# demox-labs/aleo

Measured on AMD Instinct MI355X. Metric: MSM G1 scalar-muls/sec (2^20 bases per GPU, BLS12-377, bit-exact), higher is better.
Workload: dtype u32

## Files before the change

### aleo_amd/_lib.py

```python
from __future__ import annotations
import ctypes, os

_HERE = os.path.dirname(os.path.abspath(__file__))
LIB_PATH = os.environ.get('ALEO_MI355X_LIB') or os.path.join(_HERE, 'lib', 'libaleo_mi355x.so')

EXPORTS = [
    'aleo_mi355x_init', 'aleo_mi355x_msm_g1', 'aleo_mi355x_bases_pin', 'aleo_mi355x_bases_unpin',
    'aleo_mi355x_bases_generate', 'aleo_mi355x_bases_from_scalars', 'aleo_mi355x_fr_lin_device', 'aleo_mi355x_msm_g1_device_sparse', 'aleo_mi355x_bases_precompute_range', 'aleo_mi355x_kzg_commit_segments_sparse_device', 'aleo_mi355x_fr_blind_rows_device', 'aleo_mi355x_ahp_sumcheck_operands_device', 'aleo_mi355x_varuna_prove', 'aleo_mi355x_varuna_index_build', 'aleo_mi355x_varuna_index_export', 'aleo_mi355x_varuna_index_vk', 'aleo_mi355x_varuna_index_free', 'aleo_mi355x_varuna_prove_indexed', 'aleo_mi355x_varuna_prove_batch_indexed', 'aleo_mi355x_varuna_last_timing', 'aleo_mi355x_fr_random_device', 'aleo_mi355x_fr_lincomb_device', 'aleo_mi355x_ahp_first_sumcheck_device', 'aleo_mi355x_ahp_matrix_sumcheck_device', 'aleo_mi355x_fr_powers_device', 'aleo_mi355x_fr_gather_mul_device', 'aleo_mi355x_fr_eval_batch_device', 'aleo_mi355x_bases_download', 'aleo_mi355x_bases_info', 'aleo_mi355x_bases_precompute',
    'aleo_mi355x_msm_g1_pinned', 'aleo_mi355x_msm_g1_device', 'aleo_mi355x_g1_sum', 'aleo_mi355x_msm_g2', 'aleo_mi355x_g2_sum', 'aleo_mi355x_bases_g2_pin', 'aleo_mi355x_bases_g2_unpin', 'aleo_mi355x_msm_g2_pinned', 'aleo_mi355x_ntt_fr',
    'aleo_mi355x_ntt_fr_device', 'aleo_mi355x_ntt_fr_batch_device', 'aleo_mi355x_ntt_fr_from_device', 'aleo_mi355x_fr_grid_scale_device', 'aleo_mi355x_kzg_commit', 'aleo_mi355x_kzg_commit_device', 'aleo_mi355x_kzg_commit_hiding',
    'aleo_mi355x_msm_g1_batch_device', 'aleo_mi355x_kzg_commit_batch_device', 'aleo_mi355x_kzg_commit_batch', 'aleo_mi355x_kzg_commit_segments', 'aleo_mi355x_kzg_commit_segments_device',
    'aleo_mi355x_fr_vec_op_device', 'aleo_mi355x_fr_batch_inverse_device', 'aleo_mi355x_fr_spmv_device', 'aleo_mi355x_fr_divide_by_linear_device', 'aleo_mi355x_kzg_open_device', 'aleo_mi355x_fq_mul',
    'aleo_mi355x_fr_mul', 'aleo_mi355x_selftest_madd28', 'aleo_mi355x_selftest_addquad', 'aleo_mi355x_selftest_f28_rows', 'aleo_mi355x_selftest_g2pair', 'aleo_mi355x_selftest_slice_order', 'aleo_mi355x_last_msm_timing', 'aleo_mi355x_strerror', 'aleo_mi355x_last_error',
    'aleo_mi355x_version',
    'aleo_mi355x_g1_compress', 'aleo_mi355x_g1_decompress', 'aleo_mi355x_fr_to_bytes', 'aleo_mi355x_fr_from_bytes',
    'aleo_mi355x_bech32m_encode', 'aleo_mi355x_bech32m_decode', 'aleo_mi355x_proof_to_bytes',
    'aleo_mi355x_poseidon_hash_fr', 'aleo_mi355x_fs_new', 'aleo_mi355x_fs_free', 'aleo_mi355x_fs_absorb_bytes', 'aleo_mi355x_fs_absorb_g1',
    'aleo_mi355x_fs_absorb_fr', 'aleo_mi355x_fs_squeeze_fr', 'aleo_mi355x_fr_random', 'aleo_mi355x_poseidon_parameters_fr',
    'aleo_mi355x_init_device', 'aleo_mi355x_device_count', 'aleo_mi355x_peer_info', 'aleo_mi355x_min_msm', 'aleo_mi355x_min_ntt', 'aleo_mi355x_kzg_commit_segments_sharded_device', 'aleo_mi355x_kzg_commit_batch_sharded_device', 'aleo_mi355x_bases_attach_shards', 'aleo_mi355x_bases_shard_transforms', 'aleo_mi355x_bases_pin_sharded', 'aleo_mi355x_bases_generate_sharded', 'aleo_mi355x_bases_unpin_sharded',
    'aleo_mi355x_bases_sharded_info', 'aleo_mi355x_msm_g1_sharded', 'aleo_mi355x_fr_transpose_device', 'aleo_mi355x_ntt_fr_sharded', 'aleo_mi355x_ntt_fr_sharded_device', 'aleo_mi355x_selftest_host_inverse', 'aleo_mi355x_varuna_prove_many',
    'aleo_mi355x_record_parse', 'aleo_mi355x_records_scan', 'aleo_mi355x_records_scan_host', 'aleo_mi355x_min_records',
    'aleo_mi355x_records_scan_many', 'aleo_mi355x_records_scan_many_host',
    'aleo_mi355x_records_parse_many', 'aleo_mi355x_records_parse_many_host', 'aleo_mi355x_records_scan_strings', 'aleo_mi355x_records_scan_strings_host',
    'aleo_mi355x_records_decrypt_fields', 'aleo_mi355x_records_decrypt_fields_host', 'aleo_mi355x_min_decrypt',
    'aleo_mi355x_record_fields', 'aleo_mi355x_record_plaintext', 'aleo_mi355x_record_decrypt',
    'aleo_mi355x_records_decrypt_strings', 'aleo_mi355x_records_decrypt_strings_host', 'aleo_mi355x_found_free', 'aleo_mi355x_found_count', 'aleo_mi355x_found_index',
    'aleo_mi355x_found_kind', 'aleo_mi355x_found_rvk', 'aleo_mi355x_found_offsets', 'aleo_mi355x_found_fields', 'aleo_mi355x_found_plain', 'aleo_mi355x_found_status',
    'aleo_mi355x_found_microcredits', 'aleo_mi355x_found_unparsed', 'aleo_mi355x_found_first_unparsed',
    'aleo_mi355x_records_decrypt_strings_many', 'aleo_mi355x_records_decrypt_strings_many_host',
    'aleo_mi355x_records_serial_numbers', 'aleo_mi355x_records_serial_numbers_host', 'aleo_mi355x_min_serials', 'aleo_mi355x_found_serial_numbers',
    'aleo_mi355x_record_commitment', 'aleo_mi355x_record_checksum', 'aleo_mi355x_account_from_private_key',
]


class AleoMi355xError(RuntimeError):
    status = None


class NotOwner(AleoMi355xError):
    status = 7


class UnsatisfiedAssignment(AleoMi355xError):
    status = 6


_LIB = None


def lib():
    global _LIB
    if _LIB is not None:
        return _LIB
    if not os.path.exists(LIB_PATH):
        raise AleoMi355xError(f'{LIB_PATH} not built: run `python -c "import __graft_entry__ as g; g.build()"` '
                              '(aleo_amd/csrc/build.sh).  There is no CPU fallback.')
    try:
        import torch
    except Exception:
        pass
    L = ctypes.CDLL(LIB_PATH)
    vp, sz, i32, u32, u64 = ctypes.c_void_p, ctypes.c_size_t, ctypes.c_int32, ctypes.c_uint32, ctypes.c_uint64
    sig = {
        'aleo_mi355x_init': ([i32], i32),
        'aleo_mi355x_init_device': ([i32], i32),
        'aleo_mi355x_device_count': ([ctypes.POINTER(i32), ctypes.POINTER(i32)], i32),
        'aleo_mi355x_peer_info': ([ctypes.POINTER(i32), ctypes.POINTER(i32)], i32),
        'aleo_mi355x_min_msm': ([], sz),
        'aleo_mi355x_min_ntt': ([], sz),
        'aleo_mi355x_kzg_commit_segments_sharded_device': ([vp, sz, u64, vp, sz, vp], i32),
        'aleo_mi355x_kzg_commit_batch_sharded_device': ([vp, u64, vp, vp, sz, vp], i32),
        'aleo_mi355x_bases_attach_shards': ([u64, u64, sz], i32),
        'aleo_mi355x_bases_shard_transforms': ([u64, sz], i32),
        'aleo_mi355x_bases_pin_sharded': ([vp, sz, sz, ctypes.POINTER(i32), sz, i32, ctypes.POINTER(u64)], i32),
        'aleo_mi355x_bases_generate_sharded': ([vp, u64, sz, ctypes.POINTER(i32), sz, i32, ctypes.POINTER(u64)], i32),
        'aleo_mi355x_bases_unpin_sharded': ([u64], i32),
        'aleo_mi355x_bases_sharded_info': ([u64, ctypes.POINTER(u64), i32], i32),
        'aleo_mi355x_msm_g1_sharded': ([vp, u64, vp, sz, vp], i32),
        'aleo_mi355x_fr_transpose_device': ([vp, vp, u64, u64, vp], i32),
        'aleo_mi355x_ntt_fr_sharded': ([vp, u32, i32, i32, ctypes.POINTER(i32), sz], i32),
        'aleo_mi355x_ntt_fr_sharded_device': ([vp, u32, i32, i32, ctypes.POINTER(i32), sz, vp], i32),
        'aleo_mi355x_selftest_host_inverse': ([u32, ctypes.c_uint64, ctypes.POINTER(u32), ctypes.POINTER(ctypes.c_double)], i32),
        'aleo_mi355x_msm_g1': ([vp, vp, sz, vp, sz], i32),
        'aleo_mi355x_bases_pin': ([vp, sz, sz, ctypes.POINTER(u64)], i32),
        'aleo_mi355x_bases_unpin': ([u64], i32),
        'aleo_mi355x_bases_generate': ([vp, u64, sz, ctypes.POINTER(u64)], i32),
        'aleo_mi355x_bases_from_scalars': ([vp, vp, sz, ctypes.POINTER(u64)], i32),
        'aleo_mi355x_fr_lin_device': ([vp, sz, vp, vp, vp, vp, vp, vp], i32),
        'aleo_mi355x_fr_powers_device': ([vp, sz, vp, vp, vp], i32),
        'aleo_mi355x_msm_g1_device_sparse': ([vp, u64, vp, sz, vp], i32),
        'aleo_mi355x_bases_precompute_range': ([u64, sz, sz, i32], i32),
        'aleo_mi355x_kzg_commit_segments_sparse_device': ([vp, sz, u64, vp, sz, vp], i32),
        'aleo_mi355x_fr_blind_rows_device': ([vp, vp, sz, sz, vp, vp], i32),
        'aleo_mi355x_ahp_sumcheck_operands_device': ([vp, vp, vp, sz, sz, sz, vp], i32),
        'aleo_mi355x_varuna_prove': ([vp, ctypes.POINTER(vp), sz, vp, vp, ctypes.POINTER(sz)], i32),
        'aleo_mi355x_varuna_index_build': ([ctypes.POINTER(u64), u64, u64, u64, u64, vp, sz, sz, sz, ctypes.c_uint32], i32),
        'aleo_mi355x_varuna_index_export': ([u64, vp], i32),
        'aleo_mi355x_varuna_index_vk': ([u64, vp, ctypes.POINTER(sz)], i32),
        'aleo_mi355x_varuna_index_free': ([u64], i32),
        'aleo_mi355x_varuna_prove_indexed': ([u64, ctypes.POINTER(vp), sz, vp, vp, ctypes.POINTER(sz)], i32),
        'aleo_mi355x_varuna_prove_batch_indexed': ([ctypes.POINTER(u64), sz, ctypes.POINTER(vp), ctypes.POINTER(sz), vp, vp, ctypes.POINTER(sz)], i32),
        'aleo_mi355x_varuna_last_timing': ([ctypes.POINTER(ctypes.c_double), i32], i32),
        'aleo_mi355x_varuna_prove_many': ([vp, sz], i32),
        'aleo_mi355x_fr_random_device': ([vp, sz, vp, u64, i32, vp], i32),
        'aleo_mi355x_fr_random': ([vp, sz, vp, u64], i32),
        'aleo_mi355x_poseidon_hash_fr': ([u32, vp, sz, vp, sz], i32),
        'aleo_mi355x_poseidon_parameters_fr': ([u32, vp, vp], i32),
        'aleo_mi355x_fs_new': ([ctypes.POINTER(u64)], i32),
        'aleo_mi355x_fs_free': ([u64], i32),
        'aleo_mi355x_fs_absorb_bytes': ([u64, vp, sz], i32),
        'aleo_mi355x_fs_absorb_g1': ([u64, vp, sz, sz], i32),
        'aleo_mi355x_fs_absorb_fr': ([u64, vp, sz], i32),
        'aleo_mi355x_fs_squeeze_fr': ([u64, vp, sz, i32], i32),
        'aleo_mi355x_fr_lincomb_device': ([vp, sz, vp, ctypes.POINTER(vp), ctypes.POINTER(sz), vp, sz, vp], i32),
        'aleo_mi355x_ahp_first_sumcheck_device': ([vp, sz, vp, vp, vp, vp, vp, vp, vp, vp], i32),
        'aleo_mi355x_ahp_matrix_sumcheck_device': ([vp, sz, ctypes.POINTER(vp), sz, ctypes.POINTER(vp), vp, vp], i32),
        'aleo_mi355x_fr_gather_mul_device': ([vp, sz, vp, vp, vp, vp, vp, vp], i32),
        'aleo_mi355x_fr_eval_batch_device': ([vp, ctypes.POINTER(vp), ctypes.POINTER(sz), vp, sz, vp], i32),
        'aleo_mi355x_bases_download': ([u64, sz, sz, vp], i32),
        'aleo_mi355x_bases_info': ([u64, ctypes.POINTER(u64), i32], i32),
        'aleo_mi355x_bases_precompute': ([u64], i32),
        'aleo_mi355x_msm_g1_pinned': ([vp, u64, vp, sz], i32),
        'aleo_mi355x_msm_g1_device': ([vp, u64, vp, sz, vp], i32),
        'aleo_mi355x_g1_sum': ([vp, vp, sz], i32),
        'aleo_mi355x_msm_g2': ([vp, vp, sz, vp, sz], i32),
        'aleo_mi355x_g2_sum': ([vp, vp, sz], i32),
        'aleo_mi355x_bases_g2_pin': ([vp, sz, sz, ctypes.POINTER(u64)], i32),
        'aleo_mi355x_bases_g2_unpin': ([u64], i32),
        'aleo_mi355x_msm_g2_pinned': ([vp, u64, vp, sz], i32),
        'aleo_mi355x_ntt_fr': ([vp, u32, i32, i32, i32], i32),
        'aleo_mi355x_ntt_fr_device': ([vp, u32, i32, i32, i32, vp], i32),
        'aleo_mi355x_ntt_fr_batch_device': ([vp, u32, sz, i32, i32, i32, vp], i32),
        'aleo_mi355x_ntt_fr_from_device': ([vp, vp, sz, sz, u32, sz, i32, i32, vp], i32),
        'aleo_mi355x_fr_grid_scale_device': ([vp, u32, u64, u64, u64, u64, u64, i32, i32, vp], i32),
        'aleo_mi355x_kzg_commit': ([vp, u64, vp, sz], i32),
        'aleo_mi355x_kzg_commit_device': ([vp, u64, vp, sz, vp], i32),
        'aleo_mi355x_kzg_commit_hiding': ([vp, u64, vp, sz, u64, vp, sz], i32),
        'aleo_mi355x_msm_g1_batch_device': ([vp, u64, vp, vp, sz, vp], i32),
        'aleo_mi355x_kzg_commit_batch_device': ([vp, u64, vp, vp, sz, vp], i32),
        'aleo_mi355x_kzg_commit_batch': ([vp, u64, vp, vp, sz], i32),
        'aleo_mi355x_kzg_commit_segments': ([vp, sz, u64, vp, sz], i32),
        'aleo_mi355x_kzg_commit_segments_device': ([vp, sz, u64, vp, sz, vp], i32),
        'aleo_mi355x_fr_vec_op_device': ([vp, vp, vp, sz, i32, vp], i32),
        'aleo_mi355x_fr_batch_inverse_device': ([vp, sz, vp], i32),
        'aleo_mi355x_fr_spmv_device': ([vp, vp, vp, vp, vp, sz, vp], i32),
        'aleo_mi355x_fr_divide_by_linear_device': ([vp, vp, vp, sz, vp, vp], i32),
        'aleo_mi355x_kzg_open_device': ([vp, vp, u64, vp, sz, vp, vp], i32),
        'aleo_mi355x_fq_mul': ([vp, vp, vp, sz], i32),
        'aleo_mi355x_fr_mul': ([vp, vp, vp, sz], i32),
        'aleo_mi355x_selftest_madd28': ([u32, u32, u64, ctypes.POINTER(u32)], i32),
        'aleo_mi355x_selftest_addquad': ([u32, u64, ctypes.POINTER(u32)], i32),
        'aleo_mi355x_selftest_f28_rows': ([vp, vp, u32, vp, vp, vp, vp, u32, vp, vp], i32),
        'aleo_mi355x_selftest_g2pair': ([vp, u32, u32, ctypes.POINTER(u32)], i32),
        'aleo_mi355x_selftest_slice_order': ([vp, u32, u32, i32, ctypes.POINTER(u32)], i32),
        'aleo_mi355x_last_msm_timing': ([ctypes.POINTER(ctypes.c_double), i32], i32),
        'aleo_mi355x_strerror': ([i32], ctypes.c_char_p),
        'aleo_mi355x_last_error': ([], ctypes.c_char_p),
        'aleo_mi355x_version': ([], ctypes.c_char_p),
        'aleo_mi355x_g1_compress': ([vp, vp, sz], i32),
        'aleo_mi355x_g1_decompress': ([vp, vp, sz, i32], i32),
        'aleo_mi355x_fr_to_bytes': ([vp, vp, sz], i32),
        'aleo_mi355x_fr_from_bytes': ([vp, vp, sz], i32),
        'aleo_mi355x_bech32m_encode': ([ctypes.c_char_p, sz, ctypes.c_char_p, vp, sz], i32),
        'aleo_mi355x_bech32m_decode': ([vp, ctypes.POINTER(sz), ctypes.c_char_p, sz, ctypes.c_char_p], i32),
        'aleo_mi355x_proof_to_bytes': ([vp, ctypes.POINTER(sz), vp], i32),
        'aleo_mi355x_record_parse': ([ctypes.c_char_p, ctypes.POINTER(i32), vp, vp], i32),
        'aleo_mi355x_records_scan': ([vp, vp, vp, vp, sz, vp, vp], i32),
        'aleo_mi355x_records_scan_host': ([vp, vp, vp, vp, sz, vp, vp], i32),
        'aleo_mi355x_min_records': ([], sz),
        'aleo_mi355x_records_scan_many': ([vp, vp, vp, vp, sz, vp, vp, sz], i32),
        'aleo_mi355x_records_scan_many_host': ([vp, vp, vp, vp, sz, vp, vp, sz], i32),
        'aleo_mi355x_records_parse_many': ([vp, vp, vp, vp, vp, sz], i32),
        'aleo_mi355x_records_parse_many_host': ([vp, vp, vp, vp, vp, sz], i32),
        'aleo_mi355x_records_scan_strings': ([vp, vp, vp, vp, vp, sz, vp, vp, sz], i32),
        'aleo_mi355x_records_scan_strings_host': ([vp, vp, vp, vp, vp, sz, vp, vp, sz], i32),
        'aleo_mi355x_records_decrypt_fields': ([vp, vp, vp, vp, vp, sz], i32),
        'aleo_mi355x_records_decrypt_fields_host': ([vp, vp, vp, vp, vp, sz], i32),
        'aleo_mi355x_min_decrypt': ([], sz),
        'aleo_mi355x_record_fields': ([ctypes.c_char_p, vp, sz, ctypes.POINTER(sz)], i32),
        'aleo_mi355x_record_plaintext': ([ctypes.c_char_p, vp, sz, vp, ctypes.c_char_p, ctypes.POINTER(sz)], i32),
        'aleo_mi355x_record_decrypt': ([ctypes.c_char_p, vp, vp, ctypes.c_char_p, ctypes.POINTER(sz)], i32),
        'aleo_mi355x_records_decrypt_strings': ([ctypes.POINTER(vp), vp, vp, sz, vp, vp], i32),
        'aleo_mi355x_records_decrypt_strings_host': ([ctypes.POINTER(vp), vp, vp, sz, vp, vp], i32),
        'aleo_mi355x_records_decrypt_strings_many': ([ctypes.POINTER(vp), vp, vp, sz, vp, vp, sz], i32),
        'aleo_mi355x_records_decrypt_strings_many_host': ([ctypes.POINTER(vp), vp, vp, sz, vp, vp, sz], i32),
        'aleo_mi355x_records_serial_numbers': ([vp, vp, vp, sz, vp], i32),
        'aleo_mi355x_records_serial_numbers_host': ([vp, vp, vp, sz, vp], i32),
        'aleo_mi355x_min_serials': ([], sz),
        'aleo_mi355x_found_serial_numbers': ([vp, vp, sz, vp, vp, vp], i32),
        'aleo_mi355x_record_commitment': ([vp, ctypes.c_char_p, vp, sz, ctypes.c_char_p, ctypes.c_char_p], i32),
        'aleo_mi355x_record_checksum': ([vp, ctypes.c_char_p], i32),
        'aleo_mi355x_account_from_private_key': ([ctypes.c_char_p, vp, vp, vp], i32),
        'aleo_mi355x_found_free': ([vp], None),
        **{'aleo_mi355x_found_' + name: ([vp], sz) for name in ('count', 'fields', 'unparsed', 'first_unparsed')},
        **{'aleo_mi355x_found_' + name: ([vp], vp) for name in ('index', 'kind', 'rvk', 'offsets', 'plain', 'status', 'microcredits')},
    }
    for name, (args, res) in sig.items():
        f = getattr(L, name); f.argtypes = args; f.restype = res
    _LIB = L
    return L


def check(status: int, what: str):
    if status != 0:
        L = lib()
        e = {UnsatisfiedAssignment.status: UnsatisfiedAssignment, NotOwner.status: NotOwner}.get(status, AleoMi355xError)(
            f'{what}: {L.aleo_mi355x_strerror(status).decode()} [{L.aleo_mi355x_last_error().decode()}]')
        e.status = status
        raise e


def seed32(seed=None):
    if seed is None: raw = os.urandom(32)
    elif isinstance(seed, (bytes, bytearray)):
        if len(seed) != 32: raise ValueError('a proof seed is 32 bytes')
        raw = bytes(seed)
    else: raw = int(seed).to_bytes(32, 'little')
    return (ctypes.c_uint8 * 32).from_buffer_copy(raw)
```

### aleo_amd/csrc/api.hip

```cpp
#include "entry.h"
#include "host_field.hpp"
#include <cstdlib>
#include <chrono>
#include <cstring>
#include <thread>

namespace aleo_mi355x {

thread_local MsmTiming g_last_msm;

static void jacobian_to_affine104(void* out104, const uint64_t* jac18) {
  uint8_t* o = (uint8_t*)out104; std::memset(o, 0, 104);
  bool inf = true; for (int i = 12; i < 18; ++i) if (jac18[i]) inf = false;
  if (inf) { o[96] = 1; host::HFq one = host::HFq::one(); std::memcpy(o + 48, one.l, 48); return; }
  std::memcpy(o, jac18, 96);
}

void jacobian_rows_to_affine104(void* out104, const uint64_t* jac18, size_t k) {
  for (size_t q = 0; q < k; ++q) jacobian_to_affine104((uint8_t*)out104 + 104 * q, jac18 + 18 * q);
}

template <class F> static int32_t enqueue_on_slot(void* stream, F&& f) {
  Slot sl; if (sl.rc) return sl.rc;
  hipStream_t s = nullptr; if (int32_t rcs = pick_stream(sl.c, stream, &s)) return rcs;
// ... 437 lines not shown
        for (size_t g = 0; g < G; ++g) { for (size_t i = 0; i < grp[g].size(); ++i) live[at[g][i]] = grp[g][i]; if (rcs[g] && !rc) { rc = rcs[g]; g_last_error = errs[g]; } }
        split_done = true;
      }
    }
    if (!split_done) rc = live.empty() ? ALEO_MI355X_OK : varuna_prove_many(sl.c, fb.pb, live);
    std::string first_error;
    for (size_t i = 0; i < live.size(); ++i) { requests[where[i]].status = live[i].status; if (live[i].status && first_error.empty()) first_error = live[i].error; }
    for (size_t p = 0; p < n_requests; ++p) if (rq[p].status && first_error.empty()) first_error = rq[p].error;
    if (!first_error.empty()) g_last_error = first_error;
    return rc;
  });
}

int32_t aleo_mi355x_varuna_last_timing(double* out_ms, int32_t cap) {
  int32_t n = cap < 8 ? cap : 8;
  for (int32_t i = 0; i < n; ++i) out_ms[i] = g_varuna_timing[i];
  return n;
}

int32_t aleo_mi355x_fr_random_device(void* d_dst, size_t n, const uint8_t* seed, uint64_t first_index, int32_t montgomery, void* stream) {
  return device_entry((!d_dst && n) || !seed, nullptr, stream, [&](Ctx* c, hipStream_t s) { return fr_random(c, d_dst, n, seed, first_index, montgomery, s); });
}

int32_t aleo_mi355x_fr_lincomb_device(void* d_dst, size_t n, const void* c0_mont, const void* const* d_terms, const size_t* lens, const void* coeffs_mont, size_t k, void* stream) {
  return device_entry((!d_dst && n) || (k && (!d_terms || !lens || !coeffs_mont)), nullptr, stream, [&](Ctx* c, hipStream_t s) { return fr_lincomb(c, d_dst, n, c0_mont, d_terms, lens, coeffs_mont, k, s); });
}

int32_t aleo_mi355x_ahp_first_sumcheck_device(void* d_dst, size_t n, const void* d_r, const void* d_za, const void* d_zb, const void* d_t, const void* d_z,
                                              const void* eta_b_mont, const void* eta_c_mont, void* stream) {
  return device_entry(n && (!d_dst || !d_r || !d_za || !d_zb || !d_t || !d_z || !eta_b_mont || !eta_c_mont), nullptr, stream, [&](Ctx* c, hipStream_t s) { return ahp_first_sumcheck(c, d_dst, n, d_r, d_za, d_zb, d_t, d_z, eta_b_mont, eta_c_mont, s); });
}

int32_t aleo_mi355x_ahp_matrix_sumcheck_device(void* d_dst, size_t n, const void* const* d_index, size_t index_stride, const void* const* d_f, const void* consts_mont, void* stream) {
  return device_entry(n && (!d_dst || !d_index || !d_f || !consts_mont || (d_index[0] && !d_f[0]) || (d_index[1] && !d_f[1]) || (d_index[2] && !d_f[2])), nullptr, stream, [&](Ctx* c, hipStream_t s) { return ahp_matrix_sumcheck(c, d_dst, n, d_index, index_stride, d_f, consts_mont, s); });
}

int32_t aleo_mi355x_fr_blind_rows_device(void* d_dst, const void* d_src, size_t n, size_t rows, const void* rho_mont, void* stream) {
  return device_entry(rows && n && (!d_dst || !d_src || !rho_mont), nullptr, stream, [&](Ctx* c, hipStream_t s) { return fr_blind_rows(c, d_dst, d_src, n, rows, rho_mont, s); });
}

int32_t aleo_mi355x_ahp_sumcheck_operands_device(void* d_dst, const void* d_witness_polys, const void* d_x_polys, size_t n, size_t n_x, size_t instances, void* stream) {
  return device_entry(instances && n && (!d_dst || !d_witness_polys || (!d_x_polys && n_x)), nullptr, stream, [&](Ctx* c, hipStream_t s) { return ahp_sumcheck_operands(c, d_dst, d_witness_polys, d_x_polys, n, n_x, instances, s); });
}

int32_t aleo_mi355x_fr_batch_inverse_device(void* d_inout, size_t n, void* stream) {
  return device_entry(!d_inout && n, nullptr, stream, [&](Ctx* c, hipStream_t s) { return fr_batch_inverse(c, d_inout, n, s); });
}

int32_t aleo_mi355x_fr_divide_by_linear_device(void* d_quotient, void* d_eval, const void* d_poly, size_t n, const void* z_mont, void* stream) {
  return guarded([&] {
    if ((!d_poly && n) || (!d_quotient && !d_eval)) return ALEO_MI355X_ERR_BAD_ARG;
    if (!z_mont || (d_quotient && d_quotient == d_poly)) return bad_arg("fr_divide_by_linear_device: null point, or quotient aliases the polynomial");
    return enqueue_on_slot(stream, [&](Ctx* c, hipStream_t s) { return fr_divide_by_linear(c, d_quotient, d_eval, d_poly, n, z_mont, s); });
  });
}

int32_t aleo_mi355x_kzg_open_device(void* out_affine104, void* out_eval_mont, uint64_t handle, const void* d_poly_mont, size_t n, const void* z_mont, void* stream) {
  return guarded([&] {
    if (!out_affine104 || !z_mont || (!d_poly_mont && n)) return ALEO_MI355X_ERR_BAD_ARG;
    Slot sl; if (sl.rc) return sl.rc;
    FoundBases fb(sl.d, handle); if (fb.rc) return fb.rc;
    hipStream_t s = nullptr; if (int32_t rcs = pick_stream(sl.c, stream, &s)) return rcs;
    int32_t rc; if ((rc = sl.c->ntt_stage.reserve((n ? n : 1) * 32 + 32))) return rc;
    char* q = sl.c->ntt_stage.as<char>(); char* ev = q + (n ? n : 1) * 32;
    if ((rc = fr_divide_by_linear(sl.c, q, ev, d_poly_mont, n, z_mont, s))) return rc;
    if (out_eval_mont) HIPCHK(hipMemcpyAsync(out_eval_mont, ev, 32, hipMemcpyDeviceToHost, s));
    uint64_t jac[18];
    if ((rc = msm_run1(sl.c, jac, fb.pb, q, n ? n - 1 : 0, true, s))) return rc;
    if (n <= 1) HIPCHK(hipStreamSynchronize(s));
    jacobian_to_affine104(out_affine104, jac);
    return ALEO_MI355X_OK;
  });
}

int32_t aleo_mi355x_fr_spmv_device(void* d_y, const void* d_row_ptr, const void* d_col_idx, const void* d_vals, const void* d_x, size_t rows, void* stream) {
  return device_entry((!d_y || !d_row_ptr) && rows, nullptr, stream, [&](Ctx* c, hipStream_t s) { return fr_spmv(c, d_y, d_row_ptr, d_col_idx, d_vals, d_x, rows, s); });
}

int32_t aleo_mi355x_ntt_fr(void* inout, uint32_t lg_n, int32_t order, int32_t direction, int32_t type) {
  return guarded([&] {
    if (!inout || lg_n > 30 || order < 0 || order > 3 || direction < 0 || direction > 1 || type < 0 || type > 1) return bad_arg("ntt_fr: bad argument");
    Slot sl; if (sl.rc) return sl.rc;
    size_t bytes = ((size_t)1 << lg_n) * 32;
    int32_t rc; if ((rc = sl.c->ntt_stage.reserve(bytes))) return rc;
    HIPCHK(hipMemcpyAsync(sl.c->ntt_stage.p, inout, bytes, hipMemcpyHostToDevice, sl.c->stream));
    if ((rc = ntt_run(sl.c, sl.c->ntt_stage.p, lg_n, 1, order, direction, type, sl.c->stream))) return rc;
    HIPCHK(hipMemcpyAsync(inout, sl.c->ntt_stage.p, bytes, hipMemcpyDeviceToHost, sl.c->stream));
    HIPCHK(hipStreamSynchronize(sl.c->stream));
    return ALEO_MI355X_OK;
  });
}

int32_t aleo_mi355x_ntt_fr_device(void* d_inout, uint32_t lg_n, int32_t order, int32_t direction, int32_t type, void* stream) {
  return device_entry(!d_inout || lg_n > 30 || order < 0 || order > 3 || direction < 0 || direction > 1 || type < 0 || type > 1, "ntt_fr_device: bad argument", stream, [&](Ctx* c, hipStream_t s) { return ntt_run(c, d_inout, lg_n, 1, order, direction, type, s); });
}

int32_t aleo_mi355x_ntt_fr_batch_device(void* d_inout, uint32_t lg_n, size_t batch, int32_t order, int32_t direction, int32_t type, void* stream) {
  return device_entry((!d_inout && batch) || lg_n > 30 || order < 0 || order > 3 || direction < 0 || direction > 1 || type < 0 || type > 1, "ntt_fr_batch_device: bad argument", stream, [&](Ctx* c, hipStream_t s) { return ntt_run(c, d_inout, lg_n, batch, order, direction, type, s); });
}

int32_t aleo_mi355x_ntt_fr_from_device(void* d_out, const void* d_src, size_t src_stride, size_t src_len, uint32_t lg_n, size_t batch, int32_t direction, int32_t type, void* stream) {
  return guarded([&] {
    if (((!d_out || !d_src) && batch) || lg_n > 30 || direction < 0 || direction > 1 || type < 0 || type > 1 || src_len > ((size_t)1 << lg_n) || src_stride >= (1ull << 32)) {
      g_last_error = "ntt_fr_from_device: bad argument"; return ALEO_MI355X_ERR_BAD_ARG;
    }
    if (batch) {
      const char* o0 = (const char*)d_out; const char* o1 = o0 + ((batch << lg_n) * 32);
      const char* s0 = (const char*)d_src; const char* s1 = s0 + ((batch - 1) * src_stride + src_len) * 32;
      if (src_len && o0 < s1 && s0 < o1) return bad_arg("ntt_fr_from_device: d_out overlaps d_src");
    }
    return enqueue_on_slot(stream, [&](Ctx* c, hipStream_t s) { return ntt_run_from(c, d_out, d_src, src_stride, src_len, lg_n, batch, direction, type, s); });
  });
}

int32_t aleo_mi355x_fr_grid_scale_device(void* d_data, uint32_t lg_n, uint64_t rows, uint64_t cols, uint64_t row0, uint64_t col0, uint64_t ld,
                                         int32_t mode, int32_t direction, void* stream) {
  return device_entry((!d_data && rows && cols) || lg_n == 0 || lg_n > 32 || mode < 0 || mode > 1 || direction < 0 || direction > 1, "fr_grid_scale_device: bad argument", stream, [&](Ctx* c, hipStream_t s) { return fr_grid_scale(c, d_data, lg_n, rows, cols, row0, col0, ld, mode, direction, s); });
}

int32_t aleo_mi355x_fr_transpose_device(void* d_dst, const void* d_src, uint64_t rows, uint64_t cols, void* stream) {
  return guarded([&] {
    if ((!d_dst || !d_src) && rows && cols) return bad_arg("fr_transpose_device: bad argument");
    if (d_dst == d_src && rows > 1 && cols > 1) return bad_arg("fr_transpose_device: in place is not supported");
    return enqueue_on_slot(stream, [&](Ctx* c, hipStream_t s) { return fr_transpose(c, d_dst, d_src, rows, cols, s); });
  });
}

int32_t aleo_mi355x_fq_mul(void* r, const void* a, const void* b, size_t n) {
  return guarded([&] { if ((!r || !a || !b) && n) return ALEO_MI355X_ERR_BAD_ARG; Slot sl; if (sl.rc) return sl.rc; return launch_fq_mul(sl.c, r, a, b, n); });
}
int32_t aleo_mi355x_fr_mul(void* r, const void* a, const void* b, size_t n) {
  return guarded([&] { if ((!r || !a || !b) && n) return ALEO_MI355X_ERR_BAD_ARG; Slot sl; if (sl.rc) return sl.rc; return launch_fr_mul(sl.c, r, a, b, n); });
}

int32_t aleo_mi355x_selftest_madd28(uint32_t lanes, uint32_t steps, uint64_t seed, uint32_t* failures) {
  return guarded([&] { if (!failures) return ALEO_MI355X_ERR_BAD_ARG; Slot sl; if (sl.rc) return sl.rc; return selftest_madd28(sl.c, lanes, steps, seed, failures); });
}
int32_t aleo_mi355x_selftest_addquad(uint32_t ops, uint64_t seed, uint32_t* failures) {
  return guarded([&] { if (!failures || !ops || ops > (1u << 22)) return ALEO_MI355X_ERR_BAD_ARG; Slot sl; if (sl.rc) return sl.rc; return selftest_addquad(sl.c, ops, seed, failures); });
}
int32_t aleo_mi355x_selftest_f28_rows(const void* a224, const void* b224, uint32_t n_add, void* out_pair224, void* out_quad224,
                                      const void* acc224, const void* pt112, uint32_t n_madd, void* out_acc224, uint8_t* ok_u8) {
  return guarded([&] {
    if (n_add > (1u << 20) || n_madd > (1u << 20)) return bad_arg("selftest_f28_rows: at most 2^20 rows of either kind");
    if ((n_add && (!a224 || !b224 || !out_pair224 || !out_quad224)) || (n_madd && (!acc224 || !pt112 || !out_acc224 || !ok_u8))) return bad_arg("selftest_f28_rows: bad argument");
    Slot sl; if (sl.rc) return sl.rc;
    return selftest_f28_rows(sl.c, a224, b224, n_add, out_pair224, out_quad224, acc224, pt112, n_madd, out_acc224, ok_u8);
  });
}

int32_t aleo_mi355x_selftest_slice_order(const uint32_t* hist, uint32_t n_buckets, uint32_t total_pairs, int32_t fused, uint32_t* violations) {
  return guarded([&] { if (!hist || !violations) return ALEO_MI355X_ERR_BAD_ARG; Slot sl; if (sl.rc) return sl.rc; return selftest_slice_order(sl.c, hist, n_buckets, total_pairs, fused != 0, violations); });
}
int32_t aleo_mi355x_selftest_g2pair(const void* affine192, uint32_t n_points, uint32_t n_pairs, uint32_t* failures2) {
  return guarded([&] { if (!affine192 || !failures2 || n_points < 3 || !n_pairs || n_pairs > (1u << 20)) return ALEO_MI355X_ERR_BAD_ARG; Slot sl; if (sl.rc) return sl.rc; return selftest_g2pair(sl.c, affine192, n_points, n_pairs, failures2); });
}

int32_t aleo_mi355x_last_msm_timing(double* out_ms, int32_t cap) {
  return guarded([&] {
    if (!out_ms || cap <= 0) return 0;
    const MsmTiming& t = g_last_msm;
    double v[7] = {t.total, t.sort, t.accum, t.reduce, t.host, t.accum_kernel, (double)t.accum_launches};
    int32_t k = cap < 7 ? cap : 7;
    for (int32_t i = 0; i < k; ++i) out_ms[i] = v[i];
    return k;
  }, 0);
}

const char* aleo_mi355x_strerror(int32_t status) {
  switch (status) {
    case ALEO_MI355X_OK: return "ok";
    case ALEO_MI355X_ERR_NO_DEVICE: return "no gfx950 device available";
    case ALEO_MI355X_ERR_BAD_ARG: return "bad argument";
    case ALEO_MI355X_ERR_HIP: return "HIP runtime error";
    case ALEO_MI355X_ERR_BAD_HANDLE: return "unknown handle";
    case ALEO_MI355X_ERR_OOM: return "out of device memory";
    case ALEO_MI355X_ERR_UNSATISFIED: return "assignment does not satisfy the circuit";
    case ALEO_MI355X_ERR_NOT_OWNER: return "the record's owner is not the given address";
    default: return "unknown status";
  }
}
static size_t env_size(const char* name, size_t dflt) { const char* e = std::getenv(name); if (!e || !*e) return dflt; char* end = nullptr; const unsigned long long v = std::strtoull(e, &end, 10); return end && *end == 0 ? (size_t)v : dflt; }
size_t aleo_mi355x_min_msm(void) { return env_size("ALEO_MI355X_MIN_MSM", (size_t)1 << 10); }
size_t aleo_mi355x_min_ntt(void) { return env_size("ALEO_MI355X_MIN_NTT", (size_t)1 << 12); }
int32_t aleo_mi355x_selftest_host_inverse(uint32_t count, uint64_t seed, uint32_t* failures, double* ns_per_inverse) {
  return guarded([&] {
    if (!failures) return bad_arg("selftest_host_inverse: bad argument");
    *failures = 0;
    inverse_selftest<6>(count, seed, failures, ns_per_inverse);
    inverse_selftest<4>(count, seed, failures, ns_per_inverse ? ns_per_inverse + 2 : nullptr);
    return ALEO_MI355X_OK;
  });
}
const char* aleo_mi355x_last_error(void) { return g_last_error.c_str(); }
const char* aleo_mi355x_version(void) { return "aleo_mi355x 0.4.0 (gfx950)"; }

}
```

### aleo_amd/csrc/ctx.h

```cpp
#pragma once
#include <hip/hip_runtime.h>
#include <atomic>
#include <condition_variable>
#include <cstdint>
#include <cstdio>
#include <map>
#include <memory>
#include <functional>
#include <mutex>
#include <string>
#include <vector>
#include "../../include/aleo_mi355x.h"

namespace aleo_mi355x {

extern thread_local std::string g_last_error;

#define HIPCHK(expr)                                                                                   \
  do {                                                                                                 \
    hipError_t e__ = (expr);                                                                           \
    if (e__ != hipSuccess) {                                                                           \
      char buf__[512];                                                                                 \
      snprintf(buf__, sizeof buf__, "%s failed: %s (%s:%d)", #expr, hipGetErrorString(e__), __FILE__, __LINE__); \
      g_last_error = buf__;                                                                            \
      return (e__ == hipErrorOutOfMemory) ? ALEO_MI355X_ERR_OOM : ALEO_MI355X_ERR_HIP;                 \
    }                                                                                                  \
  } while (0)

struct DevBuf {
  void* p = nullptr; size_t cap = 0;
  int32_t reserve(size_t bytes) {
    if (bytes <= cap) return ALEO_MI355X_OK;
    if (p) { (void)hipFree(p); p = nullptr; cap = 0; }
    size_t want = bytes + bytes / 8;
    HIPCHK(hipMalloc(&p, want));
    cap = want; return ALEO_MI355X_OK;
  }
  template <class T> T* as() const { return (T*)p; }
};

struct DevTmp {
  void* p = nullptr;
  DevTmp() = default; DevTmp(const DevTmp&) = delete; DevTmp& operator=(const DevTmp&) = delete;
  ~DevTmp() { if (p) (void)hipFree(p); }
  int32_t alloc(size_t bytes) { HIPCHK(hipMalloc(&p, bytes ? bytes : 1)); return ALEO_MI355X_OK; }
  void* release() { void* q = p; p = nullptr; return q; }
};

#ifndef ALEO_ROW28
#define ALEO_ROW28 128
#endif
static constexpr size_t ROW28 = ALEO_ROW28;
static_assert(ROW28 == 112 || ROW28 == 128, "row stride of the 28-bit tables");

struct PinnedBases {
  void* d_xy = nullptr;
  void* d_xy28 = nullptr;
  uint8_t* d_inf = nullptr;
  struct PreTable { void* d = nullptr; int c = 0; size_t cover = 0, min_n = 0; };
  PreTable tab[3];
  PreTable range; size_t range_off = 0;
  bool tabled = false;
  uint64_t shards = 0; size_t shard_min = 0;
  size_t shard_ntt_min = (size_t)1 << 24;
  size_t n = 0;
};

struct PinnedOwner {
  PinnedBases pb; bool building = false;
  ~PinnedOwner() { if (pb.d_xy) (void)hipFree(pb.d_xy); if (pb.d_xy28) (void)hipFree(pb.d_xy28); if (pb.d_inf) (void)hipFree(pb.d_inf); for (auto& t : pb.tab) if (t.d) (void)hipFree(t.d); if (pb.range.d) (void)hipFree(pb.range.d); }
};

struct PinnedG2 {
  void* d_xy = nullptr; uint8_t* d_inf = nullptr; void* d_rows28 = nullptr; size_t n = 0;
  ~PinnedG2() { if (d_xy) (void)hipFree(d_xy); if (d_inf) (void)hipFree(d_inf); if (d_rows28) (void)hipFree(d_rows28); }
};

struct SrsCacheEntry {
  const void* host_ptr = nullptr; size_t n = 0, stride = 0; uint64_t handle = 0, last_use = 0; uint32_t hits = 0;
  std::vector<std::pair<size_t, uint64_t>> samples;
};

struct MsmTiming { double total = 0, sort = 0, accum = 0, reduce = 0, host = 0, accum_kernel = 0; int accum_launches = 1; };

struct NttTables;

struct Device;

struct Ctx {
  Device* dev = nullptr;
  int device = -1;
  hipStream_t stream = nullptr;
  std::mutex mu;
  hipEvent_t ev[8] = {};
  uint32_t meta_seq = 0;
  size_t hist_zero_max = 0;
  size_t hist_clean = 0; hipStream_t hist_clean_stream = nullptr; void* hist_clean_ptr = nullptr;
  DevBuf hist, scan_local, scan_blk, sorted, part_cnt, part_items, partial, task_g, meta, vbuf, scalars_stage, out_stage;
  void* h_pinned = nullptr; size_t h_pinned_cap = 0;
  std::function<int32_t()> tail_hook;
  DevBuf prover_ws; void* prover_pin = nullptr; size_t prover_pin_cap = 0;
  MsmTiming last_msm;
  DevBuf cold_raw, cold_xy, cold_xy28, cold_flags;
  DevBuf ntt_tmp, ntt_stage;
  DevBuf records_k; bool records_k_ready = false;
  hipEvent_t scratch_ev = nullptr; bool scratch_busy = false; hipStream_t scratch_stream = nullptr;
  hipStream_t side = nullptr;
  hipStream_t hi = nullptr;
  hipStream_t aux = nullptr;
  hipEvent_t ev_hop = nullptr;
};

int32_t scratch_acquire(Ctx* c, DevBuf& b, size_t bytes, hipStream_t s);
int32_t scratch_release(Ctx* c, hipStream_t s);

static constexpr int MAX_SLOTS = 8;

struct Barrier {
  std::mutex mu; std::condition_variable cv; size_t n, waiting = 0, phase = 0;
  explicit Barrier(size_t n_) : n(n_) {}
  void wait() {
    std::unique_lock<std::mutex> lk(mu); const size_t ph = phase;
    if (++waiting >= n) { waiting = 0; ++phase; cv.notify_all(); } else cv.wait(lk, [&] { return phase != ph; });
  }
  void drop() {
    std::lock_guard<std::mutex> lk(mu);
    if (n) --n;
    if (n && waiting >= n) { waiting = 0; ++phase; cv.notify_all(); }
  }
};

struct ShardWs { hipStream_t st = nullptr; DevBuf a, b; };

struct Device {
  int device = -1;
  int n_slots = 4;
  std::mutex mu;
  std::map<uint64_t, std::shared_ptr<PinnedOwner>> bases; uint64_t next_handle = 1;
  std::vector<SrsCacheEntry> srs_cache; uint64_t srs_clock = 0;
  std::map<uint64_t, std::shared_ptr<PinnedG2>> g2_bases;
  std::map<uint64_t, NttTables*> ntt_tables;
  std::map<uint64_t, std::shared_ptr<struct VarunaIndexOwner>> varuna; uint64_t next_varuna = 1;
  std::atomic<int> ntt_attr_mask{0};
  Ctx slots[MAX_SLOTS];
  std::vector<std::unique_ptr<ShardWs>> shard_ws;
  DevBuf shard_home;
  hipStream_t hi_pool[MAX_SLOTS] = {}; int hi_made = 0;
  Ctx helpers[MAX_SLOTS];
};
struct HelperSet { std::vector<Ctx*> ctx; std::vector<std::unique_lock<std::mutex>> locks; };
int32_t acquire_helpers(Device* d, int want, HelperSet& hs);

extern thread_local MsmTiming g_last_msm;
void host_parallel_for(size_t n, const std::function<void(size_t)>& f);
void host_trace_mark(const char* label);
#define HT(label) do { if (::aleo_mi355x::g_host_trace_on) ::aleo_mi355x::host_trace_mark(label); } while (0)
extern bool g_host_trace_on;
int32_t ensure_host_pinned(Ctx* c, size_t bytes);

struct MsmSeg { const void* d_ptr = nullptr; size_t len = 0, off = 0; uint32_t out = 0; };
struct MsmJob { const MsmSeg* segs = nullptr; uint32_t nseg = 0, k = 0; bool mont = false; bool sparse = false; bool fire_tail = false; size_t tier_n = 0; bool lean = false; };
int32_t msm_run(Ctx* c, uint64_t* out_jac18, const PinnedBases& pb, const MsmJob& job, hipStream_t s);
inline int32_t msm_run1(Ctx* c, uint64_t* out_jac18, const PinnedBases& pb, const void* d_scalars, size_t n, bool mont, hipStream_t s, bool sparse = false) {
  MsmSeg g; g.d_ptr = d_scalars; g.len = n;
  MsmJob j; j.segs = &g; j.nseg = 1; j.k = 1; j.mont = mont; j.sparse = sparse; return msm_run(c, out_jac18, pb, j, s);
}
int32_t msm_batch(Ctx* c, uint64_t* out_jac18, const PinnedBases& pb, const MsmJob& job, hipStream_t s);
int32_t msm_run1_split(Ctx* c, uint64_t* out_jac18, const PinnedBases& pb, const void* d_scalars, size_t n, bool mont, hipStream_t s, bool sparse, const void* host_src, bool may_merge = true);
int32_t selftest_madd28(Ctx* c, uint32_t lanes, uint32_t steps, uint64_t seed, uint32_t* failures);
int32_t selftest_addquad(Ctx* c, uint32_t ops, uint64_t seed, uint32_t* failures);
int32_t selftest_f28_rows(Ctx* c, const void* a224, const void* b224, uint32_t n_add, void* out_pair224, void* out_quad224,
                          const void* acc224, const void* pt112, uint32_t n_madd, void* out_acc224, uint8_t* ok_u8);
int32_t selftest_slice_order(Ctx* c, const uint32_t* h_hist, uint32_t M, uint32_t pairs, bool fused, uint32_t* violations);
int32_t generate_multiples(Ctx* c, const void* base104, uint64_t first, size_t n, PinnedBases* out);
int32_t generate_from_scalars(Ctx* c, const void* base104, const void* scalars32, size_t n, PinnedBases* out);
int32_t msm_precompute(Ctx* c, PinnedBases* pb);
int32_t msm_precompute_range(Ctx* c, PinnedBases* pb, size_t off, size_t n, int window_bits);
int32_t unpack_affine104(Ctx* c, const void* d_rows104, void* d_xy96, void* d_flags, size_t n, hipStream_t s);
int32_t rows_to28_into(const void* d_xy96, void* d_dst, size_t n, hipStream_t s);
int32_t make_rows28(Ctx* c, PinnedBases* pb);
int32_t commit_sharded(Ctx* c, uint64_t sharded_handle, const MsmSeg* segs, uint32_t nseg, uint32_t k, bool mont, uint64_t* out_jac18, hipStream_t s, bool s_drain);
int32_t ntt_sharded_device(Ctx* c, void* d_inout, uint32_t lg_n, int32_t direction, int32_t type, const int* devices, size_t n_devices, hipStream_t s);
int32_t sharded_devices(uint64_t sharded_handle, std::vector<int>* out);
int32_t msm_g2_run(Ctx* c, uint64_t* out_jac36, const void* d_xy, const uint8_t* d_inf, const void* d_scalars, size_t n, hipStream_t s, const void* d_rows28 = nullptr);
int32_t g2_rows_to28(const void* d_xy192, void* d_dst224, size_t n, hipStream_t s);
int32_t g2_sum_host(uint64_t* out36, const uint64_t* pts36, size_t count);
int32_t selftest_g2pair(Ctx* c, const void* aff192_host, uint32_t n, uint32_t npairs, uint32_t* failures2);
int32_t g2_unpack200(Ctx* c, const void* d_rows200, void* d_xy192, void* d_flags, uint32_t* d_count, size_t n, hipStream_t s);
int32_t launch_fq_mul(Ctx* c, void* r, const void* a, const void* b, size_t n);
int32_t launch_fr_mul(Ctx* c, void* r, const void* a, const void* b, size_t n);
int32_t fr_lin(Ctx* c, void* d_dst, size_t n, const void* c0, const void* c1, const void* d_a, const void* c2, const void* d_b, hipStream_t s);
int32_t fr_powers(Ctx* c, void* d_dst, size_t n, const void* first, const void* ratio, hipStream_t s);
int32_t fr_gather_mul(Ctx* c, void* d_dst, size_t n, const void* d_scale, const void* d_t1, const void* d_idx1, const void* d_t2, const void* d_idx2, hipStream_t s);
int32_t fr_gather_mul3(Ctx* c, void* const* d_dst, const size_t* n, const void* const* d_scale, const void* d_t1, const void* const* d_idx1, const void* d_t2, const void* const* d_idx2, uint32_t count, hipStream_t s);
int32_t fr_eval_batch(Ctx* c, void* d_out, const void* const* d_polys, const size_t* lens, const void* z_mont, size_t k, hipStream_t s);
int32_t fr_random(Ctx* c, void* d_dst, size_t n, const uint8_t* seed32, uint64_t first, int32_t mont, hipStream_t s);
int32_t fr_lincomb(Ctx* c, void* d_dst, size_t n, const void* c0, const void* const* d_terms, const size_t* lens, const void* coeffs, size_t k, hipStream_t s);
int32_t fr_add_tiled(Ctx* c, void* d_dst, size_t n, const void* d_src, size_t n_src, hipStream_t s);
int32_t ahp_first_sumcheck(Ctx* c, void* d_dst, size_t n, const void* d_r, const void* d_a, const void* d_b, const void* d_t, const void* d_z, const void* eta_b, const void* eta_c, hipStream_t s);
int32_t ahp_matrix_sumcheck(Ctx* c, void* d_dst, size_t n, const void* const* d_index, size_t index_stride_elems, const void* const* d_f, const void* consts, hipStream_t s);
int32_t fr_blind_rows(Ctx* c, void* d_dst, const void* d_src, size_t n, size_t rows, const void* rho_mont, hipStream_t s);
int32_t ahp_sumcheck_operands(Ctx* c, void* d_dst, const void* d_wit, const void* d_xp, size_t n, size_t n_x, size_t instances, hipStream_t s);
int32_t fr_scatter_to_mont(Ctx* c, void* d_dst, const void* d_src, const void* d_pos, size_t n, void* d_flag, hipStream_t s);
int32_t fr_vec_op(Ctx* c, void* d_dst, const void* d_a, const void* d_b, size_t n, int32_t op, hipStream_t s);
int32_t fr_batch_inverse(Ctx* c, void* d_inout, size_t n, hipStream_t s);
int32_t fr_divide_by_linear(Ctx* c, void* d_q, void* d_eval, const void* d_p, size_t n, const void* z_mont32, hipStream_t s);
int32_t index_expand_rows(Ctx* c, const uint32_t* d_row_ptr, const uint32_t* d_col, const uint32_t* d_positions, size_t rows, uint32_t* d_k_row, uint32_t* d_k_col, uint32_t* d_cpos, uint32_t* d_count_plus1, hipStream_t s);
int32_t index_scan_inclusive(Ctx* c, uint32_t* d_a, size_t n, hipStream_t s);
int32_t index_transpose_rows(Ctx* c, const uint32_t* d_row_ptr, const uint32_t* d_cpos, const void* d_val, size_t rows, uint32_t row_base, uint32_t* d_cursor, uint32_t* d_tcol, void* d_tval, hipStream_t s);
int32_t fr_spmv(Ctx* c, void* d_y, const void* d_row_ptr, const void* d_col, const void* d_vals, const void* d_x, size_t rows, hipStream_t s, size_t max_row = 0);
int32_t fr_divide_by_linear_many(Ctx* c, void* const* d_q, void* const* d_eval, const void* const* d_p, const size_t* n, const void* const* z_mont32, size_t count, hipStream_t s);
int32_t fr_scale_rows(Ctx* c, void* d_dst, const void* d_src, size_t n, size_t rows, const void* consts_mont, hipStream_t s);
int32_t fr_split_quotient(Ctx* c, void* d_hq, void* d_rq, const void* d_q, const void* d_mask, size_t n, void* host_sum_devptr, hipStream_t s);
int32_t fr_sub_mul(Ctx* c, void* d_dst, const void* d_a, const void* d_b, const void* d_m, size_t n, hipStream_t s);
int32_t fr_pick(Ctx* c, void* dst_devptr, const void* const* d_src, size_t count, hipStream_t s);
int32_t varuna_prove(Ctx* c, const PinnedBases& pb, const aleo_mi355x_varuna_index& ix, const void* const* assignments, size_t k, const uint8_t* seed32, uint8_t* out, size_t* out_len);
struct ProveRequest { std::vector<const aleo_mi355x_varuna_index*> ixs; const void* const* assignments = nullptr; const size_t* ks = nullptr; const uint8_t* seed32 = nullptr;
                      uint8_t* out = nullptr; size_t* out_len = nullptr; int32_t status = 0; std::string error; };
int32_t varuna_prove_many(Ctx* c, const PinnedBases& pb, std::vector<ProveRequest>& requests, int workers = 0);
int32_t varuna_prove_batch(Ctx* c, const PinnedBases& pb, const aleo_mi355x_varuna_index* const* ixs, size_t m, const void* const* assignments, const size_t* ks,
                           const uint8_t* seed32, uint8_t* out, size_t* out_len);
extern thread_local double g_varuna_timing[8];
struct VarunaIndexOwner;
int32_t varuna_index_build(Ctx* c, const PinnedBases& pb, std::shared_ptr<PinnedOwner> key, uint64_t key_handle, uint64_t max_degree, uint64_t gamma_offset,
                           uint64_t lagrange_offset, const aleo_mi355x_r1cs_matrix* abc, size_t n_constraints, size_t n_public, size_t n_private, uint32_t domain_flags, VarunaIndexOwner** out);
void varuna_index_delete(VarunaIndexOwner* o);
const aleo_mi355x_varuna_index* varuna_index_view(const VarunaIndexOwner* o);
const std::vector<uint8_t>& varuna_index_vk(const VarunaIndexOwner* o);
void jacobian_rows_to_affine104(void* out104, const uint64_t* jac18, size_t k);
int32_t ntt_run(Ctx* c, void* d_inout, uint32_t lg_n, size_t batch, int32_t order, int32_t direction, int32_t type, hipStream_t s);
int32_t ntt_run_from(Ctx* c, void* d_out, const void* d_src, size_t src_stride_elems, size_t src_len, uint32_t lg_n, size_t batch, int32_t direction, int32_t type, hipStream_t s);

int32_t fr_transpose(Ctx* c, void* d_dst, const void* d_src, uint64_t rows, uint64_t cols, hipStream_t s);
int32_t fr_grid_scale(Ctx* c, void* d_data, uint32_t lg_n, uint64_t rows, uint64_t cols, uint64_t row0, uint64_t col0, uint64_t ld, int32_t mode,
                      int32_t direction, hipStream_t s);

}
```

### aleo_amd/csrc/msm.hip

```cpp
#include "ec.h"
#include "fp28.h"
#include "host_field.hpp"
#include "msm_chain.h"
#include <chrono>

namespace aleo_mi355x {

__device__ __forceinline__ XYZZ xyzz28_to_xyzz(const XYZZ28& a) {
  XYZZ r; r.X = f28_to_fq(a.X); r.Y = f28_to_fq(a.Y); r.ZZ = f28_to_fq(a.ZZ); r.ZZZ = f28_to_fq(a.ZZZ); return r;
}
__device__ __noinline__ void slice_slow_path28(const char* bases, const uint32_t* run, uint32_t j, uint32_t j1, const XYZZ28* acc28, XYZZ* acc_out, bool* inf_out) {
  XYZZ acc = xyzz28_to_xyzz(*acc28); bool inf = false;
  for (; j < j1; ++j) {
    uint32_t e = run[j];
    F28 x, y; load_affine28(bases + (size_t)(e & 0x7fffffffu) * ROW28, x, y);
    AffinePt p; p.x = Fq::reduce(f28_to_fq(x)); p.y = Fq::reduce(f28_to_fq(y));
    if (e >> 31) p.y = fq_neg_canonical(p.y);
    xyzz_madd(acc, inf, p.x, p.y);
  }
  *acc_out = acc; *inf_out = inf;
}

__device__ __forceinline__ const char* chain_sum(const FrontChain& ch, uint32_t g) {
  for (uint32_t i = 0; i < ch.n; ++i) if (ch.v[i].hist[g]) return ch.v[i].partial + (size_t)scan_at(ch.v[i].scan_local, ch.v[i].scan_blk, g).y * 224u;
// ... 175 lines not shown
  uint32_t base = j * S;
  if (base) {
    XYZZ r = xyzz_infinity();
    for (int bit = 31 - __clz(base); bit >= 0; --bit) {
      xyzz_double_ni(&r);
      if ((base >> bit) & 1) xyzz_add_ni(&r, &run);
    }
    xyzz_add_ni(&acc, &r);
  }
  store_xyzz(V + (size_t)t * 192, acc);
}

__global__ void __launch_bounds__(256) k_seg_tree_pass(char* __restrict__ V, uint32_t seg_len, uint32_t nseg, uint32_t L) {
  const uint32_t half = (L + 1) >> 1, pairs = L - half;
  const uint32_t op = (blockIdx.x * 256 + threadIdx.x) >> 1;
  if (op >= pairs * nseg) return;
  const uint32_t seg = op / pairs, i = op % pairs;
  char* pa = V + ((size_t)seg * seg_len + i) * 192;
  xyzz_add_pair(pa, pa + (size_t)half * 192, pa);
}

static constexpr uint32_t PB28 = 224, PW28 = 56;
template <uint32_t LANES>
__global__ void __launch_bounds__(256) k_masked_pairs(const char* __restrict__ Vrun, uint32_t lgN, uint32_t nsets, char* __restrict__ V, uint32_t v_set_stride) {
  const uint32_t seg_len = 1u << (lgN - 2);
  const uint32_t op = (blockIdx.x * 256 + threadIdx.x) >> lg_lanes(LANES);
  if (op >= seg_len * lgN * nsets) return;
  const uint32_t q = op / (seg_len * lgN), r = op % (seg_len * lgN), l = r / seg_len, k = r % seg_len;
  auto ins = [&](uint32_t x) { return ((x >> l) << (l + 1)) | (1u << l) | (x & ((1u << l) - 1u)); };
  const char* run = Vrun + ((size_t)q << lgN) * PB28;
  pt28_add<LANES>(run + (size_t)ins(2 * k) * PB28, run + (size_t)ins(2 * k + 1) * PB28, V + ((size_t)q * v_set_stride + (1u << lgN) + r) * PB28);
}
static constexpr uint32_t FOLD = 256;
template <uint32_t LANES>
__global__ void __launch_bounds__(128 * LANES) k_seg_fold(const char* __restrict__ in, uint32_t in_stride, uint32_t L, uint32_t nseg,
                                                          char* __restrict__ out, uint32_t out_stride) {
  __shared__ __attribute__((aligned(16))) uint32_t lds[2][(FOLD / 2) * PW28];
  const uint32_t bps = (L + FOLD - 1) / FOLD, seg = blockIdx.x / bps, blk = blockIdx.x % bps, pr = threadIdx.x >> lg_lanes(LANES);
  if (seg >= nseg) return;
  {
    const uint32_t e0 = blk * FOLD + 2 * pr;
    const char* src = in + ((size_t)seg * in_stride + e0) * PB28;
    char* dst = (char*)(lds[0] + pr * PW28);
    if (e0 + 1 < L) pt28_add<LANES>(src, src + PB28, dst);
    else if (e0 < L) grp_copy<LANES, PB28>(src, dst);
    else grp_zero<LANES, PB28>(dst);
  }
  uint32_t cur = 0;
  for (uint32_t n = FOLD / 2; n > 1; n >>= 1) {
    __syncthreads();
    if (pr < (n >> 1)) pt28_add<LANES>((const char*)(lds[cur] + (2 * pr) * PW28), (const char*)(lds[cur] + (2 * pr + 1) * PW28), (char*)(lds[cur ^ 1] + pr * PW28));
    cur ^= 1;
  }
  __syncthreads();
  if (pr == 0) grp_copy<LANES, PB28>((const char*)lds[cur], out + ((size_t)seg * out_stride + blk) * PB28);
}
template <uint32_t LANES>
__global__ void __launch_bounds__(256) k_seg_pair_pass(const char* __restrict__ in, uint32_t in_stride, uint32_t L, uint32_t nseg,
                                                       char* __restrict__ out, uint32_t out_stride) {
  const uint32_t half = (L + 1) >> 1;
  const uint32_t op = (blockIdx.x * 256 + threadIdx.x) >> lg_lanes(LANES);
  if (op >= half * nseg) return;
  const uint32_t seg = op / half, i = op % half;
  const char* src = in + ((size_t)seg * in_stride + 2 * i) * PB28;
  char* dst = out + ((size_t)seg * out_stride + i) * PB28;
  if (2 * i + 1 < L) pt28_add<LANES>(src, src + PB28, dst); else grp_copy<LANES, PB28>(src, dst);
}
template <uint32_t LANES>
__global__ void __launch_bounds__(256) k_prog_pass(const char* __restrict__ node, uint32_t node_set_stride, const char* __restrict__ A, uint32_t a_set_stride,
                                                   const char* __restrict__ T, uint32_t t_set_stride, uint32_t nT, uint32_t L, uint32_t nsets,
                                                   char* __restrict__ out, uint32_t out_set_stride) {
  const uint32_t half = L >> 1, per_set = (2 + nT) * half;
  const uint32_t op = (blockIdx.x * 256 + threadIdx.x) >> lg_lanes(LANES);
  if (op >= per_set * nsets) return;
  const uint32_t q = op / per_set, r = op % per_set, g = r / half, i = r % half;
  const char* src = g == 0 ? node + ((size_t)q * node_set_stride + 2 * i) * PB28
                  : g == 1 ? A + ((size_t)q * a_set_stride + 2 * i) * PB28
                           : T + ((size_t)q * t_set_stride + (size_t)(g - 2) * L + 2 * i) * PB28;
  char* dst = out + ((size_t)q * out_set_stride + (size_t)g * half + i) * PB28;
  pt28_add<LANES>(src, src + PB28, dst);
  if (g == 0) grp_copy<LANES, PB28>(src + PB28, out + ((size_t)q * out_set_stride + (size_t)(2 + nT) * half + i) * PB28);
}
__global__ void __launch_bounds__(256) k_prog_pass2(const char* __restrict__ node, uint32_t node_set_stride, const char* __restrict__ A, uint32_t a_set_stride,
                                                    const char* __restrict__ T, uint32_t t_set_stride, uint32_t nT, uint32_t L, uint32_t nsets,
                                                    char* __restrict__ out, uint32_t out_set_stride) {
  __shared__ __attribute__((aligned(16))) uint32_t lds[(2 * 32 + 1) * PW28];
  char* zero = (char*)(lds + 64 * PW28);
  if (threadIdx.x < 4) grp_zero<4, PB28>(zero);
  __syncthreads();
  const uint32_t quarter = L >> 2, per_set = (2 + nT) * quarter;
  const uint32_t oct = threadIdx.x >> 3, y = (threadIdx.x >> 2) & 1u, op = blockIdx.x * 32 + oct;
  if (op >= per_set * nsets) return;
  const uint32_t q = op / per_set, r = op % per_set, g = r / quarter, i = r % quarter;
  const char* src = g == 0 ? node + ((size_t)q * node_set_stride + 4 * i) * PB28
                  : g == 1 ? A + ((size_t)q * a_set_stride + 4 * i) * PB28
                           : T + ((size_t)q * t_set_stride + (size_t)(g - 2) * L + 4 * i) * PB28;
  char* slot = (char*)(lds + (2 * oct) * PW28);
  pt28_add<4>(src + (size_t)(2 * y) * PB28, src + (size_t)(2 * y + 1) * PB28, slot + y * PB28);
  pair_fence();
  char* base = out + (size_t)q * out_set_stride * PB28;
  const bool born = y && g == 0;
  const char* pa = y ? (born ? src + PB28 : zero) : slot;
  const char* pb = y ? (born ? src + 3 * PB28 : zero) : slot + PB28;
  char* dst = y ? (born ? base + ((size_t)(2 + nT) * quarter + i) * PB28 : zero) : base + ((size_t)g * quarter + i) * PB28;
  pt28_add<4>(pa, pb, dst);
  if (born) grp_copy<4, PB28>(slot + PB28, base + ((size_t)(3 + nT) * quarter + i) * PB28);
}
template <uint32_t LANES>
__global__ void __launch_bounds__(128 * LANES) k_prog_final(const char* __restrict__ in, uint32_t in_set_stride, uint32_t L, uint32_t nT, uint32_t lgL, uint32_t nsets,
                                                            char* __restrict__ out) {
  __shared__ __attribute__((aligned(16))) uint32_t lds[2][(FOLD / 2) * PW28];
  const uint32_t per_set = 1 + nT + lgL, q = blockIdx.x / per_set, o = blockIdx.x % per_set, pr = threadIdx.x >> lg_lanes(LANES);
  if (q >= nsets) return;
  const char* set = in + (size_t)q * in_set_stride * PB28;
  {
    char* dst = (char*)(lds[0] + pr * PW28);
    if (o <= nT) {
      const char* seg = set + (size_t)(o == 0 ? 1 : 1 + o) * L * PB28; const uint32_t e0 = 2 * pr;
      if (e0 + 1 < L) pt28_add<LANES>(seg + (size_t)e0 * PB28, seg + (size_t)(e0 + 1) * PB28, dst);
      else if (e0 < L) grp_copy<LANES, PB28>(seg + (size_t)e0 * PB28, dst);
      else grp_zero<LANES, PB28>(dst);
    } else {
      const uint32_t b = o - 1 - nT;
      auto ins = [&](uint32_t x) { return ((x >> b) << (b + 1)) | (1u << b) | (x & ((1u << b) - 1u)); };
      if (L >= 4 && 4 * pr + 3 < L) pt28_add<LANES>(set + (size_t)ins(2 * pr) * PB28, set + (size_t)ins(2 * pr + 1) * PB28, dst);
      else if (L == 2 && pr == 0) grp_copy<LANES, PB28>(set + PB28, dst);
      else grp_zero<LANES, PB28>(dst);
    }
  }
  uint32_t cur = 0;
  for (uint32_t n = FOLD / 2; n > 1; n >>= 1) {
    __syncthreads();
    if (pr < (n >> 1)) pt28_add<LANES>((const char*)(lds[cur] + (2 * pr) * PW28), (const char*)(lds[cur] + (2 * pr + 1) * PW28), (char*)(lds[cur ^ 1] + pr * PW28));
    cur ^= 1;
  }
  __syncthreads();
  if (pr == 0) grp_copy<LANES, PB28>((const char*)lds[cur], out + ((size_t)q * per_set + o) * PB28);
}
__global__ void k_gather_strided(const char* __restrict__ V, uint32_t stride, uint32_t count, char* __restrict__ out) {
  uint32_t t = blockIdx.x * blockDim.x + threadIdx.x;
  if (t >= count * 14) return;
  uint32_t w = t / 14, q = t % 14;
  ((uint4*)out)[t] = ((const uint4*)(V + (size_t)w * stride * PB28))[q];
}

__global__ void k_gather_windows(const char* __restrict__ V, uint32_t seg_len, uint32_t W, char* __restrict__ out) {
  uint32_t t = blockIdx.x * blockDim.x + threadIdx.x;
  if (t >= W * 12) return;
  uint32_t w = t / 12, q = t % 12;
  ((uint4*)out)[t] = ((const uint4*)(V + (size_t)w * seg_len * 192))[q];
}

int32_t msm_front_sort(Ctx* c, const PinnedBases& pb, const MsmJob& job, hipStream_t s, Front& f) {
  const uint32_t K = f.K = job.k;
  size_t n = 0, pts = 0; SegArgs segs{};
  if (K > MAX_SETS || job.nseg > MAX_SEGS) { g_last_error = "msm: too many sets / segments in one call"; return ALEO_MI355X_ERR_BAD_ARG; }
  for (uint32_t q = 0; q < job.nseg; ++q) {
    const MsmSeg& g = job.segs[q];
    if (g.len == 0) continue;
    if (g.out >= K || g.off + g.len >= (1ull << 31)) { g_last_error = "msm: segment out of range"; return ALEO_MI355X_ERR_BAD_ARG; }
    const uint32_t i = segs.nseg++;
    segs.ptr[i] = (const char*)g.d_ptr; segs.n[i] = (uint32_t)g.len; segs.off[i] = (uint32_t)g.off; segs.set[i] = (uint8_t)g.out;
    n = g.off + g.len > n ? g.off + g.len : n; pts += g.len;
  }
  if (n == 0) { f.empty = true; return ALEO_MI355X_OK; }
  if (job.tier_n > n && job.tier_n <= pb.n) n = job.tier_n;
  if (n > pb.n) { g_last_error = "msm: a segment reaches past the pinned bases"; return ALEO_MI355X_ERR_BAD_ARG; }
  const PinnedBases::PreTable* T = nullptr;
  const uint8_t* d_inf = pb.d_inf;
  bool ranged = job.sparse && pb.range.d != nullptr;
  for (uint32_t i = 0; ranged && i < segs.nseg; ++i) ranged = segs.off[i] >= pb.range_off && (size_t)segs.off[i] + segs.n[i] <= pb.range_off + pb.range.cover;
  if (ranged) {
    T = &pb.range; n = 0;
    for (uint32_t i = 0; i < segs.nseg; ++i) { segs.off[i] -= (uint32_t)pb.range_off; n = (size_t)segs.off[i] + segs.n[i] > n ? (size_t)segs.off[i] + segs.n[i] : n; }
    if (d_inf) d_inf += pb.range_off;
  } else T = msm_tier(pb, n);
  const bool pre = f.pre = T != nullptr;
  if (K > 1 && (!pre || K > (ranged ? msm_range_sets(pb) : msm_max_sets(pb, n)))) { g_last_error = "msm: internal: batch without a table tier (or too many sets)"; return ALEO_MI355X_ERR_BAD_ARG; }
  MsmPlan& P = f.P; P = make_plan(pre ? n : pts, pre ? T->c : 0);
  if (pre) { P.W = K; P.M = K * P.B; }
  if (!pre && !pb.d_xy28) { g_last_error = "msm: pinned set without 28-bit rows"; return ALEO_MI355X_ERR_HIP; }
  f.bases = (const char*)(pre ? T->d : pb.d_xy28);
  const uint32_t cpw = f.cpw = P.B / P.S, nchunks = f.nchunks = cpw * P.W;
  uint32_t lgN = 0; while ((1u << lgN) < cpw) ++lgN;
  f.lgN = lgN;
  const bool masked = f.masked = pre && lgN >= 2 && (1u << lgN) == cpw;
  if (pre && !masked) { g_last_error = "msm: internal: table path without masked reduction"; return ALEO_MI355X_ERR_HIP; }
  int32_t rc;
  const uint32_t tseg = f.tseg = cpw / 4, fseg = f.fseg = lgN + 4, nseg = f.nseg = K * fseg, setw = f.setw = fseg * tseg;
  constexpr uint32_t SUM_TREE_MIN_C = 13;
  f.prog = masked && P.c >= SUM_TREE_MIN_C && cpw > FOLD;
  f.out_pts = f.prog ? 1 + lgN : fseg;
  f.vpoints = masked ? (size_t)K * setw + nchunks + (nseg + 1) + (size_t)nseg * (tseg / 2 + tseg / 4 + 2) + 3 * (size_t)nchunks + 64 : (size_t)nchunks + P.W;
  if ((rc = ensure_host_pinned(c, 64 + (size_t)(masked ? nseg : P.W) * 224 + ASIDE_MAX * 228))) return rc;
  SortPhase& sp = f.sp;
  if ((rc = msm_sort_phase(c, segs, pts, job.mont, d_inf, (uint32_t)(pre ? T->cover : pb.n), P, pre, s, &sp, f.lean))) return rc;
  const uint32_t M = sp.M;
  if ((rc = c->partial.reserve(sp.slices_max * (pre ? 224 : 192)))) return rc;
  if ((rc = c->vbuf.reserve(f.vpoints * 224))) return rc;
  return ALEO_MI355X_OK;
}

int32_t msm_front_accum(Ctx* c, hipStream_t s, Front& f, const FrontChain* seed, hipEvent_t after) {
  const SortPhase& sp = f.sp; const uint32_t M = sp.M; const char* bases = f.bases;
  char* partial = c->partial.as<char>();
  if (after) HIPCHK(hipStreamWaitEvent(s, after, 0));
  if (!f.lean) HIPCHK(hipEventRecord(c->ev[6], s));
  const bool seeded = f.pre && seed && seed->n;
  auto* const kern = seeded ? k_accum28<true, true> : f.pre ? k_accum28<true, false> : k_accum28<false, false>;
  hipLaunchKernelGGL(kern, dim3(sp.slice_blocks), dim3(256), 0, s, bases, sp.sorted, sp.hist, sp.scan_local, sp.scan_blk, sp.total_pairs, M, sp.meta, sp.order, sp.task_g, partial, seeded ? *seed : FrontChain{});
  if (!f.lean) HIPCHK(hipEventRecord(c->ev[5], s));
  HIPCHK(hipGetLastError());
  return ALEO_MI355X_OK;
}

int32_t msm_front_finish(Ctx* c, hipStream_t s, Front& f, bool allow_aside) {
  int32_t rc;
  const SortPhase& sp = f.sp; SliceMeta& sm = f.sm; const uint32_t M = sp.M; const bool pre = f.pre;
  uint32_t* heavy = sp.heavy; uint32_t* meta = sp.meta; uint2* scan_local = sp.scan_local; uint2* scan_blk = sp.scan_blk;
  char* partial = c->partial.as<char>();
  if ((rc = msm_wait_meta(c, sp, s, &sm))) return rc;
  const bool aside = f.aside = allow_aside && f.masked && sm.n_super >= 1 && sm.n_super <= ASIDE_MAX && !sm.super_overflow && sm.max_m >= 64;
  uint32_t* h_aside = (uint32_t*)((char*)c->h_pinned + 64 + (size_t)f.nseg * 224);
  if (aside) {
    if (f.lean) HIPCHK(hipEventRecord(c->ev[5], s));
    HIPCHK(hipStreamWaitEvent(c->side, c->ev[5], 0));
    for (uint32_t pass = 0, L = sm.max_m - 1; L > 1; ++pass, L = (L + 1) >> 1) {
      const uint64_t ops = (uint64_t)sm.n_super * (L >> 1);
      launch_grp(grp_lanes(ops), k_tree_pass<true, 4>, k_tree_pass<true, 2>, ops, c->side, partial, heavy, 0u, 0u, sp.super_list, sm.n_super, L >> 1, scan_local, scan_blk, M, meta, pass, 1u);
    }
    uint32_t* dst = nullptr;
    HIPCHK(hipHostGetDevicePointer((void**)&dst, h_aside, 0));
    hipLaunchKernelGGL(k_gather_super, dim3((sm.n_super * 57 + 255) / 256), dim3(256), 0, c->side, partial, sp.super_list, sm.n_super, scan_local, scan_blk, dst);
    HIPCHK(hipEventRecord(c->ev[4], c->side));
  }
  const bool rest_ok = pre && !sm.super_overflow && (aside || sm.n_super == 0) && sm.n_heavy && sm.max_common > 2 && sm.max_common <= 8;
  if (sm.NT) {
    for (uint32_t pass = 0, L = sm.max_m, Lcm = sm.max_common; L > 1; ++pass, L = (L + 1) >> 1, Lcm = (Lcm + 1) >> 1) {
      if (rest_ok && pass == 1) {
        hipLaunchKernelGGL(k_tree_rest<4>, dim3((uint32_t)((4ull * sm.n_heavy + 255) / 256)), dim3(256), 0, s, partial, heavy, sm.n_heavy, scan_local, scan_blk, M, meta);
        break;
      }
      const uint32_t Lc = sm.super_overflow ? L : Lcm;
      const uint32_t len_a = (sm.n_heavy && Lc > 1) ? sm.n_heavy : 0, pairs_a = len_a ? Lc >> 1 : 0;
      const uint32_t len_b = aside ? 0 : sm.n_super, pairs_b = len_b ? L >> 1 : 0;
      const uint64_t ops = (uint64_t)len_a * pairs_a + (uint64_t)len_b * pairs_b;
      const uint32_t lanes = pre ? grp_lanes(ops) : 2u;
      const uint64_t threads = lanes * ops;
      if (!threads) continue;
      if (threads >= (1ull << 32)) { (void)hipStreamSynchronize(s); g_last_error = "msm: slice tree too wide"; return ALEO_MI355X_ERR_HIP; }
      launch_grp(lanes, k_tree_pass<true, 4>, pre ? k_tree_pass<true, 2> : k_tree_pass<false, 2>, ops, s, partial, heavy, len_a, pairs_a, sp.super_list, len_b, pairs_b, scan_local, scan_blk, M, meta, pass, 0u);
    }
  }
  if (!f.lean) HIPCHK(hipEventRecord(c->ev[2], s));
  return ALEO_MI355X_OK;
}

int32_t msm_reduce_queue(Ctx* c, Front& f, hipStream_t s, const FrontChain& older) {
  const MsmPlan& P = f.P; const SortPhase& sp = f.sp;
  const uint32_t K = f.K, cpw = f.cpw, nchunks = f.nchunks, lgN = f.lgN, tseg = f.tseg, nseg = f.nseg, setw = f.setw;
  uint32_t* hist = sp.hist; uint2* scan_local = sp.scan_local; uint2* scan_blk = sp.scan_blk;
  char* partial = c->partial.as<char>(); char* V = c->vbuf.as<char>(); char* h_win = (char*)c->h_pinned + 64;
  char* Vrun = V + (size_t)K * setw * PB28; char* Tout = Vrun + (size_t)nchunks * PB28;
  const uint32_t lanes = grp_lanes(2 * (uint64_t)nchunks), per_block = lanes == 4 ? 32u : CHUNK_QUADS;
  auto* const chunks = lanes == 4 ? k_bucket_chunks<true, 4> : k_bucket_chunks<true, 2>;
  hipLaunchKernelGGL(chunks, dim3((nchunks + per_block - 1) / per_block), dim3(256), 0, s, partial, hist, scan_local, scan_blk, P.B, P.S, nchunks, V, setw, Vrun, older);
  if (f.prog) {
    char* G0 = Tout; char* G1 = G0 + (size_t)K * (3 * (cpw / 2)) * PB28;
    const char* node = Vrun; uint32_t node_ss = cpw; const char* A = V; uint32_t a_ss = setw; const char* T = Vrun; uint32_t t_ss = 0, nT = 0, L = cpw;
    char* dstbuf = G0;
    while (L > FOLD) {
      const uint32_t half = L >> 1, out_ss = (3 + nT) * half; const uint64_t ops = (uint64_t)(2 + nT) * half * K;
      if ((L >> 2) >= FOLD && grp_lanes(ops) == 4) {
        const uint32_t quarter = L >> 2, out2 = (4 + nT) * quarter; const uint64_t octs = (uint64_t)(2 + nT) * quarter * K;
        hipLaunchKernelGGL(k_prog_pass2, dim3((uint32_t)((octs + 31) / 32)), dim3(256), 0, s, node, node_ss, A, a_ss, T, t_ss, nT, L, K, dstbuf, out2);
        node = dstbuf; node_ss = out2; A = dstbuf + (size_t)quarter * PB28; a_ss = out2; T = dstbuf + (size_t)2 * quarter * PB28; t_ss = out2; nT += 2; L = quarter;
        dstbuf = dstbuf == G0 ? G1 : G0;
        continue;
      }
      launch_grp(grp_lanes(ops), k_prog_pass<4>, k_prog_pass<2>, ops, s, node, node_ss, A, a_ss, T, t_ss, nT, L, K, dstbuf, out_ss);
      node = dstbuf; node_ss = out_ss; A = dstbuf + (size_t)half * PB28; a_ss = out_ss; T = dstbuf + (size_t)2 * half * PB28; t_ss = out_ss; ++nT; L = half;
      dstbuf = dstbuf == G0 ? G1 : G0;
    }
    uint32_t lgL = 0; while ((1u << lgL) < L) ++lgL;
    char* dst = nullptr;
    HIPCHK(hipHostGetDevicePointer((void**)&dst, h_win, 0));
    hipLaunchKernelGGL(k_prog_final<4>, dim3(K * (1 + nT + lgL)), dim3(512), 0, s, node, node_ss, L, nT, lgL, K, dst);
  } else {
    const uint64_t mops = (uint64_t)tseg * lgN * K;
    launch_grp(grp_lanes(mops), k_masked_pairs<4>, k_masked_pairs<2>, mops, s, Vrun, lgN, K, V, setw);
    char* F1 = Tout + (size_t)(nseg + 1) * PB28; char* F2 = F1 + (size_t)nseg * (tseg / 2 + 1) * PB28;
    const char* cur = V; uint32_t L = tseg, stride = tseg;
    while (L > FOLD) {
      char* dst = (cur == F1) ? F2 : F1; uint32_t half = (L + 1) >> 1;
      const uint64_t ops = (uint64_t)half * nseg;
      launch_grp(grp_lanes(ops), k_seg_pair_pass<4>, k_seg_pair_pass<2>, ops, s, cur, stride, L, nseg, dst, half);
      cur = dst; stride = half; L = half;
    }
    if (L > 1) {
      char* dst = nullptr;
      HIPCHK(hipHostGetDevicePointer((void**)&dst, h_win, 0));
      hipLaunchKernelGGL(k_seg_fold<4>, dim3(nseg), dim3(512), 0, s, cur, stride, L, nseg, dst, 1u);
    } else {
      hipLaunchKernelGGL(k_gather_strided, dim3((nseg * 14 + 255) / 256), dim3(256), 0, s, cur, stride, nseg, Tout);
      HIPCHK(hipMemcpyAsync(h_win, Tout, (size_t)nseg * PB28, hipMemcpyDeviceToHost, s));
    }
  }
  HIPCHK(hipEventRecord(c->ev[3], s));
  if (f.lean && older.n == 0 && !f.aside) {
    if (sp.zero_bytes > c->hist_zero_max) c->hist_zero_max = sp.zero_bytes;
    const size_t z = c->hist_zero_max <= c->hist.cap && (void*)sp.hist == c->hist.p ? c->hist_zero_max : sp.zero_bytes;
    HIPCHK(hipMemsetAsync(sp.hist, 0, z, s)); c->hist_clean = z; c->hist_clean_stream = s; c->hist_clean_ptr = (void*)sp.hist;
  }
  return ALEO_MI355X_OK;
}

static int32_t phase_times(Ctx* c, const Front& f, std::chrono::steady_clock::time_point t_host0) {
  const double host_ms = std::chrono::duration<double, std::milli>(std::chrono::steady_clock::now() - t_host0).count();
  float ms; MsmTiming tm;
  if (f.lean) { tm.host = host_ms; tm.total = host_ms; c->last_msm = tm; g_last_msm = tm; return ALEO_MI355X_OK; }
  HIPCHK(hipEventElapsedTime(&ms, c->ev[0], c->ev[1])); tm.sort = ms;
  HIPCHK(hipEventElapsedTime(&ms, c->ev[1], c->ev[2])); tm.accum = ms;
  HIPCHK(hipEventElapsedTime(&ms, c->ev[2], c->ev[3])); tm.reduce = ms;
  HIPCHK(hipEventElapsedTime(&ms, c->ev[6], c->ev[5])); tm.accum_kernel = ms;
  tm.host = host_ms; tm.total = tm.sort + tm.accum + tm.reduce + tm.host;
  c->last_msm = tm; g_last_msm = tm;
  return ALEO_MI355X_OK;
}

int32_t msm_collect(Ctx* c, uint64_t* out_jac18, Front& f, hipStream_t s, bool fire_tail, TailWait wait) {
  using namespace host;
  const MsmPlan& P = f.P; const SliceMeta& sm = f.sm; const uint32_t K = f.K, lgN = f.lgN, out_pts = f.out_pts; const bool prog = f.prog, aside = f.aside;
  const uint32_t* h_aside = (const uint32_t*)((char*)c->h_pinned + 64 + (size_t)f.nseg * 224);
  const char* h_win = (const char*)c->h_pinned + 64;
  if (fire_tail && c->tail_hook) {
    std::function<int32_t()> hook = std::move(c->tail_hook); c->tail_hook = nullptr;
    HT("msm: reduction queued");
    const int32_t hrc = hook();
    HT("msm: hook queued");
    HIPCHK(hipEventSynchronize(c->ev[3]));
    if (hrc) { (void)hipStreamSynchronize(s); return hrc; }
  } else if (wait == TailWait::event) HIPCHK(hipEventSynchronize(c->ev[3]));
  else HIPCHK(hipStreamSynchronize(s));
  if (aside) HIPCHK(hipEventSynchronize(c->ev[4]));
  HIPCHK(hipGetLastError());
  HT("msm: result arrived");
  const auto t_host0 = std::chrono::steady_clock::now();
  HXYZZ totals[MAX_SETS];
  auto horner = [&](size_t q) {
// ... 128 lines not shown
```

### aleo_amd/csrc/msm_chain.h

```cpp
#pragma once
#include "msm_common.h"

namespace aleo_mi355x {
#pragma GCC visibility push(hidden)
struct FrontView { const char* partial; const uint32_t* hist; const uint2* scan_local; const uint2* scan_blk; };
struct FrontChain { FrontView v[3]; uint32_t n = 0; };
struct Front {
  MsmPlan P{}; SortPhase sp; SliceMeta sm;
  uint32_t K = 0, cpw = 0, nchunks = 0, lgN = 0, tseg = 0, fseg = 0, nseg = 0, setw = 0; size_t vpoints = 0;
  uint32_t out_pts = 0;
  bool pre = false, masked = false, prog = false, aside = false, empty = false, lean = false; const char* bases = nullptr;
};
struct StreamDrainGuard {
  std::vector<hipStream_t> streams; bool armed = true;
  ~StreamDrainGuard() { if (!armed) return; const std::string keep = g_last_error; for (hipStream_t st : streams) if (st) (void)hipStreamSynchronize(st); g_last_error = keep; }
  void add(hipStream_t st) { streams.push_back(st); }
  void dismiss() { armed = false; }
};
int32_t msm_front_sort(Ctx* c, const PinnedBases& pb, const MsmJob& job, hipStream_t s, Front& f);
int32_t msm_front_accum(Ctx* c, hipStream_t s, Front& f, const FrontChain* seed, hipEvent_t after);
int32_t msm_front_finish(Ctx* c, hipStream_t s, Front& f, bool allow_aside);
int32_t msm_reduce_queue(Ctx* c, Front& f, hipStream_t s, const FrontChain& older);
enum class TailWait { stream, event };
int32_t msm_collect(Ctx* c, uint64_t* out_jac18, Front& f, hipStream_t s, bool fire_tail, TailWait wait);
int32_t msm_back(Ctx* c, uint64_t* out_jac18, Front& f, hipStream_t s, bool fire_tail, const FrontChain& older);
#pragma GCC visibility pop
}
```

### aleo_amd/csrc/msm_common.h

```cpp
#pragma once
#include "ctx.h"

namespace aleo_mi355x {

static constexpr uint32_t SCAN_TILE = 2048;
static constexpr uint32_t SCALAR_BITS = 254;
static constexpr uint32_t MAX_SETS = 32;
static constexpr uint32_t MAX_SEGS = 64;
static constexpr uint32_t SUPER_CAP = 4096;
static constexpr uint32_t MAX_SLICE = 512;

struct MsmPlan { uint32_t c, W, B, M, S; };
__host__ __device__ constexpr int win_count(int c) { return ((int)SCALAR_BITS + c - 1) / c; }
__host__ __device__ constexpr int win_full(int c) { return win_count(c) - (win_count(c) * c - (int)SCALAR_BITS); }
__host__ __device__ constexpr int win_width(int c, int w) { return w < win_full(c) ? c : c - 1; }
__host__ __device__ constexpr int win_offset(int c, int w) { return w <= win_full(c) ? w * c : win_full(c) * c + (w - win_full(c)) * (c - 1); }
MsmPlan make_plan(size_t n, int pre_c);
__attribute__((visibility("hidden"))) const PinnedBases::PreTable* msm_tier(const PinnedBases& pb, size_t n);
__attribute__((visibility("hidden"))) uint32_t msm_range_sets(const PinnedBases& pb);
uint32_t msm_max_sets(const PinnedBases& pb, size_t n);
struct SegArgs { const char* ptr[MAX_SEGS]; uint32_t n[MAX_SEGS], off[MAX_SEGS], col0[MAX_SEGS]; uint8_t set[MAX_SEGS]; uint32_t nseg = 0, ncol = 0, tile = 2048; };

struct SliceRule { uint32_t single, split; };
__host__ __device__ __forceinline__ SliceRule pick_rule(const uint32_t* total_pairs, uint32_t M) {
  const uint32_t pairs = total_pairs[0], mean = pairs / M, fill_shift = total_pairs[1];
  const uint32_t fill_min = pairs < (1u << 18) ? 4u : 8u;
  uint32_t by_mean = 32u; while (by_mean < 2u * mean && by_mean < 512u) by_mean <<= 1;
  uint32_t fill = (pairs + (1u << fill_shift) - 1) >> fill_shift;
  fill = fill < fill_min ? fill_min : (fill > 256u ? 256u : fill);
  SliceRule r; r.single = by_mean; r.split = by_mean >> 1;
  if (by_mean >= 2u * fill) { r.single = fill; r.split = fill; }
  return r;
}
__host__ __device__ __forceinline__ uint32_t slices_of(uint32_t cnt, SliceRule r) { return cnt <= r.single ? (cnt ? 1u : 0u) : (cnt + r.split - 1) / r.split; }
__device__ __forceinline__ uint2 scan_at(const uint2* local, const uint2* blk, uint32_t g) {
  uint2 a = local[g], b = blk[g / SCAN_TILE]; return make_uint2(a.x + b.x, a.y + b.y);
}
__host__ __device__ __forceinline__ uint32_t slice_len(uint32_t cnt, uint32_t m, uint32_t k) {
  return (uint32_t)(((uint64_t)(k + 1) * cnt) / m) - (uint32_t)(((uint64_t)k * cnt) / m);
}

struct SortPhase {
  MsmPlan P; uint32_t M = 0, digitsW = 0, slice_blocks = 0; size_t slices_max = 0, pairs_max = 0;
  uint32_t *hist = nullptr, *heavy = nullptr, *meta = nullptr; uint2 *scan_local = nullptr, *scan_blk = nullptr;
  uint32_t *sorted = nullptr, *task_g = nullptr, *order = nullptr; const uint32_t* total_pairs = nullptr; const uint32_t* super_list = nullptr;
  uint32_t meta_seq = 0;
  size_t zero_bytes = 0;
};
struct SliceMeta { uint32_t NT = 0, max_m = 0, n_heavy = 0, n_super = 0, max_common = 0; bool super_overflow = false; };
int32_t msm_sort_phase(Ctx* c, SegArgs& segs, size_t pts, bool mont, const uint8_t* d_inf, uint32_t row_stride,
                       const MsmPlan& P, bool pre, hipStream_t s, SortPhase* out, bool lean = false);
int32_t msm_wait_meta(Ctx* c, const SortPhase& sp, hipStream_t s, SliceMeta* m);

}
```

### aleo_amd/csrc/msm_request.hip

```cpp
#include "host_field.hpp"
#include "msm_chain.h"
#include <cstring>
#include <thread>

namespace aleo_mi355x {

static void identity_results(uint64_t* out_jac18, size_t k, const uint32_t* where = nullptr) {
  for (size_t q = 0; q < k; ++q) host::hstore_jacobian_normalized(out_jac18 + 18 * (size_t)(where ? where[q] : q), host::HXYZZ::infinity());
}

int32_t msm_run(Ctx* c, uint64_t* out_jac18, const PinnedBases& pb, const MsmJob& job, hipStream_t s) {
  if (job.k == 0) return ALEO_MI355X_OK;
  Front f; int32_t rc;
  f.lean = job.lean;
  if ((rc = msm_front_sort(c, pb, job, s, f))) return rc;
  if (f.empty) { identity_results(out_jac18, job.k); return ALEO_MI355X_OK; }
  if ((rc = msm_front_accum(c, s, f, nullptr, nullptr))) return rc;
  if ((rc = msm_front_finish(c, s, f, true))) return rc;
  return msm_back(c, out_jac18, f, s, job.fire_tail, FrontChain{});
}

static int32_t msm_run_chunked(Ctx* c, HelperSet& hs, uint64_t* out_jac18, const PinnedBases& pb, size_t n, bool mont, hipStream_t s, const void* host_src) {
  const uint32_t Q = 1 + (uint32_t)hs.ctx.size();
  static const uint32_t share[4][3] = {{0, 0, 0}, {0, 0, 0}, {37, 63, 0}, {18, 30, 52}};
  Ctx* cx[3] = {c, Q > 1 ? hs.ctx[0] : nullptr, Q > 2 ? hs.ctx[1] : nullptr}; hipStream_t st[3] = {s, Q > 1 ? hs.ctx[0]->hi : nullptr, Q > 2 ? hs.ctx[1]->hi : nullptr};
  StreamDrainGuard guard; for (uint32_t k = 0; k < Q; ++k) { guard.add(st[k]); guard.add(cx[k]->side); }
  size_t lo[4] = {0, 0, 0, 0};
  for (uint32_t k = 0, acc = 0; k < Q; ++k) { acc += share[Q][k]; lo[k + 1] = k + 1 == Q ? n : (((size_t)((double)n * acc / 100.0)) + 255) & ~(size_t)255; if (lo[k + 1] > n) lo[k + 1] = n; }
  Front f[3]; MsmSeg seg[3]; int32_t rc;
  auto view = [&](uint32_t k) { return FrontView{cx[k]->partial.as<char>(), f[k].sp.hist, f[k].sp.scan_local, f[k].sp.scan_blk}; };
  auto chain_before = [&](uint32_t k) { FrontChain ch; for (uint32_t i = k; i-- > 0;) ch.v[ch.n++] = view(i); return ch; };
  for (uint32_t k = 0; k < Q; ++k) {
    MsmJob j; j.mont = mont; j.tier_n = n; j.k = 1;
    const size_t len = lo[k + 1] - lo[k];
    if ((rc = cx[k]->scalars_stage.reserve((len ? len : 1) * 32))) return rc;
    if (hipMemcpyAsync(cx[k]->scalars_stage.p, (const char*)host_src + lo[k] * 32, len * 32, hipMemcpyHostToDevice, st[k]) != hipSuccess) { g_last_error = "msm: upload of a chunk failed"; return ALEO_MI355X_ERR_HIP; }
    seg[k].d_ptr = cx[k]->scalars_stage.p; seg[k].len = len; seg[k].off = lo[k];
    j.segs = &seg[k]; j.nseg = 1;
    if ((rc = msm_front_sort(cx[k], pb, j, st[k], f[k]))) return rc;
    if (f[k].empty || !f[k].masked || f[k].P.c != f[0].P.c || f[k].sp.M != f[0].sp.M) { g_last_error = "msm: internal: chunks without a shared table window"; return ALEO_MI355X_ERR_HIP; }
    if (k) { if ((rc = msm_front_finish(cx[k - 1], st[k - 1], f[k - 1], false))) return rc; }
    const FrontChain seed = chain_before(k);
    if ((rc = msm_front_accum(cx[k], st[k], f[k], &seed, k ? cx[k - 1]->ev[2] : nullptr))) return rc;
  }
  if ((rc = msm_front_finish(cx[Q - 1], st[Q - 1], f[Q - 1], false))) return rc;
  if ((rc = msm_back(cx[Q - 1], out_jac18, f[Q - 1], st[Q - 1], false, chain_before(Q - 1)))) return rc;
  HIPCHK(hipStreamSynchronize(s));
  MsmTiming tm = cx[Q - 1]->last_msm; float ms = 0, kern = 0;
  for (uint32_t k = 0; k < Q; ++k) { HIPCHK(hipEventElapsedTime(&ms, cx[k]->ev[6], cx[k]->ev[5])); kern += ms; }
  tm.accum_kernel = kern / Q; tm.accum_launches = (int)Q;
  HIPCHK(hipEventElapsedTime(&ms, c->ev[0], c->ev[1])); tm.sort = ms;
  HIPCHK(hipEventElapsedTime(&ms, c->ev[1], cx[Q - 1]->ev[2])); tm.accum = ms;
  tm.total = tm.sort + tm.accum + tm.reduce + tm.host;
  c->last_msm = tm; g_last_msm = tm;
  guard.dismiss();
  return ALEO_MI355X_OK;
}

namespace {
struct Chain { std::vector<MsmSeg> segs; std::vector<uint32_t> results; size_t points = 0; bool sparse = false, fire_tail = false; };
void scatter_results(uint64_t* out_jac18, const Chain& ch, const uint64_t* res) {
  for (size_t q = 0; q < ch.results.size(); ++q) std::memcpy(out_jac18 + 18 * (size_t)ch.results[q], res + 18 * q, 144);
}
}
static int32_t run_chains_pipelined(Ctx* c, const std::vector<Ctx*>& helpers, uint64_t* out_jac18, const PinnedBases& pb, std::vector<Chain>& chains, bool mont, hipStream_t s) {
  auto SS = [&](Ctx* x) { return x->aux; };
  const size_t n = chains.size(), R = 1 + helpers.size();
  std::vector<Ctx*> cx(R); std::vector<hipStream_t> acc_st(R);
  cx[0] = c; acc_st[0] = s; for (size_t k = 1; k < R; ++k) { cx[k] = helpers[k - 1]; acc_st[k] = helpers[k - 1]->stream; }
  StreamDrainGuard guard; for (size_t k = 0; k < R; ++k) { guard.add(SS(cx[k])); guard.add(acc_st[k]); guard.add(cx[k]->side); }
  std::vector<Front> f(n); std::vector<MsmJob> job(n); std::vector<char> live(n, 0);
  HIPCHK(hipEventRecord(c->ev[4], s));
  for (size_t k = 0; k < R; ++k) { HIPCHK(hipStreamWaitEvent(SS(cx[k]), c->ev[4], 0)); if (k) HIPCHK(hipStreamWaitEvent(acc_st[k], c->ev[4], 0)); }
  int32_t rc;
  auto sort_of = [&](size_t i) -> int32_t {
    Chain& ch = chains[i]; MsmJob& g = job[i];
    g.segs = ch.segs.data(); g.nseg = (uint32_t)ch.segs.size(); g.k = (uint32_t)ch.results.size(); g.mont = mont; g.sparse = ch.sparse; g.fire_tail = false;
    Ctx* cc = cx[i % R];
    const int32_t r = msm_front_sort(cc, pb, g, SS(cc), f[i]);
    if (r) return r;
    if (f[i].empty) { identity_results(out_jac18, ch.results.size(), ch.results.data()); return ALEO_MI355X_OK; }
    if (!f[i].masked) { g_last_error = "msm: internal: a pipelined chain without a table tier"; return ALEO_MI355X_ERR_HIP; }
    live[i] = 1;
    HIPCHK(hipEventRecord(cc->ev_hop, SS(cc)));
    return ALEO_MI355X_OK;
  };
  auto collect = [&](size_t i) -> int32_t {
    if (!live[i]) return ALEO_MI355X_OK;
    uint64_t res[MAX_SETS * 18]; Ctx* cc = cx[i % R];
    const int32_t r = msm_collect(cc, res, f[i], SS(cc), false, TailWait::event);
    if (r) return r;
    scatter_results(out_jac18, chains[i], res);
    live[i] = 0;
    return ALEO_MI355X_OK;
  };
  if ((rc = sort_of(0))) return rc;
  hipEvent_t prev_accum = nullptr; size_t collected = 0;
  for (size_t i = 0; i < n; ++i) {
    Ctx* cc = cx[i % R]; hipStream_t as = acc_st[i % R];
    if (live[i]) {
      HIPCHK(hipStreamWaitEvent(as, cc->ev_hop, 0));
      if ((rc = msm_front_accum(cc, as, f[i], nullptr, prev_accum))) return rc;
      prev_accum = cc->ev[5];
    }
    if (i + 1 < n) {
      for (; collected + R <= i + 1; ++collected) if ((rc = collect(collected))) return rc;
      if (live[i]) HIPCHK(hipStreamWaitEvent(SS(cx[(i + 1) % R]), cc->ev[6], 0));
      if ((rc = sort_of(i + 1))) return rc;
    }
    if (live[i]) {
      HIPCHK(hipStreamWaitEvent(SS(cc), cc->ev[5], 0));
      if ((rc = msm_front_finish(cc, SS(cc), f[i], true))) return rc;
      if ((rc = msm_reduce_queue(cc, f[i], SS(cc), FrontChain{}))) return rc;
    }
  }
  for (; collected < n; ++collected) if ((rc = collect(collected))) return rc;
  return ALEO_MI355X_OK;
}
static int32_t run_chains(Ctx* c, uint64_t* out_jac18, const PinnedBases& pb, std::vector<Chain>& chains, bool mont, hipStream_t s, bool lean = false) {
  bool lean_now = false;
  auto run_one = [&](Ctx* cc, Chain& ch, hipStream_t st) -> int32_t {
    uint64_t res[MAX_SETS * 18];
    MsmJob g; g.segs = ch.segs.data(); g.nseg = (uint32_t)ch.segs.size(); g.k = (uint32_t)ch.results.size(); g.mont = mont; g.sparse = ch.sparse; g.fire_tail = ch.fire_tail; g.lean = lean_now;
    const int32_t rc = msm_run(cc, res, pb, g, st);
    if (rc) return rc;
    scatter_results(out_jac18, ch, res);
    return ALEO_MI355X_OK;
  };
  size_t total = 0; for (auto& ch : chains) total += ch.points;
  HelperSet hs;
  if (chains.size() >= 2 && total >= ((size_t)1 << 20) && c->dev) { const int32_t rc = acquire_helpers(c->dev, chains.size() >= 3 ? 2 : 1, hs); if (rc) return rc; }
  if (hs.ctx.empty()) { lean_now = lean; for (auto& ch : chains) { const int32_t rc = run_one(c, ch, s); if (rc) return rc; } return ALEO_MI355X_OK; }
  Ctx* h = hs.ctx[0];
  bool all_tiered = true;
  for (auto& ch : chains) {
    size_t reach = 0; for (auto& g : ch.segs) if (g.len) reach = g.off + g.len > reach ? g.off + g.len : reach;
    bool t_ok = reach == 0;
    if (reach && msm_tier(pb, reach)) t_ok = ch.results.size() <= 1 || ch.results.size() <= msm_max_sets(pb, reach);
    all_tiered = all_tiered && t_ok && ch.results.size() <= MAX_SETS;
  }
  if (all_tiered) return run_chains_pipelined(c, hs.ctx, out_jac18, pb, chains, mont, s);
  HIPCHK(hipEventRecord(c->ev[4], s));
  HIPCHK(hipStreamWaitEvent(h->stream, c->ev[4], 0));
  std::atomic<size_t> next{0}; int32_t rc_h = ALEO_MI355X_OK; std::string err_h; MsmTiming tm_h{};
  std::thread helper([&] {
    if (hipSetDevice(c->device) != hipSuccess) { rc_h = ALEO_MI355X_ERR_HIP; err_h = "hipSetDevice failed"; return; }
    try {
      for (size_t i; (i = next.fetch_add(1)) < chains.size();) { const int32_t rc = run_one(h, chains[i], h->stream); if (rc) { rc_h = rc; err_h = g_last_error; return; } }
    } catch (...) { rc_h = ALEO_MI355X_ERR_HIP; err_h = "msm: exception on the helper thread"; }
    tm_h = h->last_msm;
  });
  int32_t rc_m = ALEO_MI355X_OK;
  try { for (size_t i; !rc_m && (i = next.fetch_add(1)) < chains.size();) rc_m = run_one(c, chains[i], s); }
  catch (...) { rc_m = ALEO_MI355X_ERR_HIP; g_last_error = "msm: exception on the calling thread"; next.store(chains.size()); }
  helper.join();
  (void)hipStreamSynchronize(h->stream);
  if (rc_m) return rc_m;
  if (rc_h) { g_last_error = err_h; return rc_h; }
  return ALEO_MI355X_OK;
}

static constexpr uint32_t MERGE_MIN_LG = 19, CHUNKS3_MIN_LG = 21;
int32_t msm_run1_split(Ctx* c, uint64_t* out_jac18, const PinnedBases& pb, const void* d_scalars, size_t n, bool mont, hipStream_t s, bool sparse, const void* host_src, bool may_merge) {
  const bool tiered = msm_tier(pb, n) != nullptr;
  HelperSet hs;
  if (host_src && may_merge && !sparse && tiered && n >= ((size_t)1 << MERGE_MIN_LG) && c->dev) { const int32_t rc = acquire_helpers(c->dev, n >= ((size_t)1 << CHUNKS3_MIN_LG) ? 2 : 1, hs); if (rc) return rc; }
  if (!hs.ctx.empty()) return msm_run_chunked(c, hs, out_jac18, pb, n, mont, s, host_src);
  if (host_src) {
    const int32_t rc = c->scalars_stage.reserve((n ? n : 1) * 32); if (rc) return rc;
    if (n) HIPCHK(hipMemcpyAsync(c->scalars_stage.p, host_src, n * 32, hipMemcpyHostToDevice, s));
    d_scalars = c->scalars_stage.p;
  }
  return msm_run1(c, out_jac18, pb, d_scalars, n, mont, s, sparse);
}

static int32_t cut_chains(const MsmJob& job, const std::vector<uint32_t>& ids, const std::vector<size_t>& points, const std::vector<uint32_t>& nsegs, size_t cap, bool sparse, std::vector<Chain>& chains) {
  for (size_t pos = 0; pos < ids.size();) {
    size_t take = 0, pts = 0, sg = 0;
    while (pos + take < ids.size() && take < cap && (take == 0 || (pts + points[ids[pos + take]] <= ((size_t)1 << 26) && sg + nsegs[ids[pos + take]] <= MAX_SEGS))) {
      pts += points[ids[pos + take]]; sg += nsegs[ids[pos + take]]; ++take;
    }
    if (sg > MAX_SEGS) { g_last_error = "msm: one result with more than 64 segments"; return ALEO_MI355X_ERR_BAD_ARG; }
    chains.emplace_back(); Chain& ch = chains.back(); ch.segs.reserve(sg); ch.points = pts; ch.sparse = sparse; ch.fire_tail = take == job.k;
    for (size_t i = 0; i < take; ++i) ch.results.push_back(ids[pos + i]);
    for (uint32_t q = 0; q < job.nseg; ++q) {
      const MsmSeg& g = job.segs[q];
      if (!g.len) continue;
      for (size_t i = 0; i < take; ++i) if (ch.results[i] == g.out) { MsmSeg h = g; h.out = (uint32_t)i; ch.segs.push_back(h); break; }
    }
    pos += take;
  }
  return ALEO_MI355X_OK;
}

int32_t msm_batch(Ctx* c, uint64_t* out_jac18, const PinnedBases& pb, const MsmJob& job, hipStream_t s) {
  const uint32_t K = job.k;
  auto tier_of = [&](size_t n) { const PinnedBases::PreTable* t = msm_tier(pb, n); return t ? (int)(t - pb.tab) : -1; };
  std::vector<size_t> reach(K, 0), points(K, 0); std::vector<uint32_t> nsegs(K, 0);
  for (uint32_t q = 0; q < job.nseg; ++q) {
    const MsmSeg& g = job.segs[q];
    if (g.out >= K) { g_last_error = "msm: segment names a result that does not exist"; return ALEO_MI355X_ERR_BAD_ARG; }
    if (!g.len) continue;
    reach[g.out] = g.off + g.len > reach[g.out] ? g.off + g.len : reach[g.out]; points[g.out] += g.len; nsegs[g.out]++;
  }
  if (job.sparse && pb.range.d) {
    bool inside = true;
    for (uint32_t q = 0; q < job.nseg && inside; ++q) { const MsmSeg& g = job.segs[q]; if (g.len) inside = g.off >= pb.range_off && g.off + g.len <= pb.range_off + pb.range.cover; }
    if (inside) {
      std::vector<uint32_t> all(K); for (uint32_t q = 0; q < K; ++q) all[q] = q;
      std::vector<Chain> chains;
      if (const int32_t rc = cut_chains(job, all, points, nsegs, msm_range_sets(pb), true, chains)) return rc;
      return run_chains(c, out_jac18, pb, chains, job.mont, s, job.lean);
    }
  }
  {
    size_t far = 0, pts = 0, sg = 0;
    for (uint32_t q = 0; q < K; ++q) { far = reach[q] > far ? reach[q] : far; pts += points[q]; sg += nsegs[q]; }
    if (K > 1 && K <= MAX_SETS && tier_of(far) >= 0 && K <= msm_max_sets(pb, far) && pts <= ((size_t)1 << 21) && sg <= MAX_SEGS) {
      bool split = false;
      for (uint32_t q = 0; q < K; ++q) if (points[q] && tier_of(reach[q]) != tier_of(far)) split = true;
      if (split) {
        std::vector<MsmSeg> segs; segs.reserve(sg);
        for (uint32_t q = 0; q < job.nseg; ++q) if (job.segs[q].len) segs.push_back(job.segs[q]);
        MsmJob g; g.segs = segs.data(); g.nseg = (uint32_t)segs.size(); g.k = K; g.mont = job.mont; g.fire_tail = true; g.lean = job.lean;
        return msm_run(c, out_jac18, pb, g, s);
      }
    }
  }
  std::vector<uint32_t> todo; todo.reserve(K); std::vector<Chain> chains;
  for (int t = -1; t < 3; ++t) {
    todo.clear();
    for (uint32_t q = 0; q < K; ++q) if (tier_of(reach[q]) == t) todo.push_back(q);
    if (todo.empty()) continue;
    const size_t cap = t < 0 ? 1 : msm_max_sets(pb, reach[todo[0]]);
    if (const int32_t rc = cut_chains(job, todo, points, nsegs, cap, false, chains)) return rc;
  }
  return run_chains(c, out_jac18, pb, chains, job.mont, s, job.lean);
}

}
```

### aleo_amd/csrc/msm_sort.hip

```cpp
#include <algorithm>
#include "ec.h"
#include "msm_common.h"

namespace aleo_mi355x {

MsmPlan make_plan(size_t n, int pre_c) {
  MsmPlan p;
  if (pre_c) {
    p.c = (uint32_t)pre_c; p.W = 1; p.B = 1u << (pre_c - 1); p.M = p.B; p.S = pre_c >= 20 ? 16 : 4;
    return p;
  }
  uint32_t lg = 0; while (((size_t)1 << (lg + 1)) <= n) ++lg;
  int c = (int)lg - 4; if (c < 2) c = 2; if (c > 16) c = 16;
  p.c = (uint32_t)c; p.W = (SCALAR_BITS + p.c - 1) / p.c; p.B = 1u << (p.c - 1); p.M = p.W * p.B;
  p.S = p.B >= 8 ? 8 : p.B;
  return p;
}

template <bool MONT> __device__ __forceinline__ void load_scalar(const void* scalars, uint32_t i, uint32_t (&s)[8]) {
  const uint4* p = (const uint4*)scalars + 2 * (size_t)i;
  uint4 a = p[0], b = p[1];
  s[0] = a.x; s[1] = a.y; s[2] = a.z; s[3] = a.w; s[4] = b.x; s[5] = b.y; s[6] = b.z; s[7] = b.w;
  if constexpr (MONT) {
    Fr f; for (int k = 0; k < 8; ++k) f.v[k] = s[k];
    f = Fr::from_mont(f);
    for (int k = 0; k < 8; ++k) s[k] = f.v[k];
  }
}
template <int C, int W_IDX> __device__ __forceinline__ uint32_t window_raw(const uint32_t (&s)[8]) {
  constexpr int bit = win_offset(C, W_IDX), width = win_width(C, W_IDX), limb = bit >> 5, off = bit & 31;
  uint32_t v = 0;
  if constexpr (limb < 8) {
    v = s[limb] >> off;
    if constexpr (off + width > 32 && limb + 1 < 8) v |= s[limb + 1] << (32 - off);
  }
  return v & ((1u << width) - 1u);
}

template <int C, int W_IDX, class F> __device__ __forceinline__ void for_each_digit(const uint32_t (&s)[8], uint32_t carry, F&& f) {
  constexpr int W = win_count(C);
  if constexpr (W_IDX < W) {
    constexpr int width = win_width(C, W_IDX);
    constexpr uint32_t B = 1u << (width - 1);
    uint32_t d = window_raw<C, W_IDX>(s) + carry;
    uint32_t neg = d > B ? 1u : 0u;
    uint32_t mag = neg ? (1u << width) - d : d;
    if (mag) f((uint32_t)W_IDX, mag - 1u, neg);
    for_each_digit<C, W_IDX + 1>(s, neg, f);
  }
}

static constexpr uint32_t PART_TILE = 2048;
static constexpr uint32_t MAX_COARSE = 2048;
static constexpr uint32_t MAX_COARSE_ALL = 4096;

template <int C, bool PRE> struct SortGeom {
  static constexpr uint32_t W = (SCALAR_BITS + C - 1) / C, B = 1u << (C - 1);
  static constexpr uint32_t LB = (C - 1) < 8 ? (C - 1) : 8;
  static constexpr uint32_t CB = B >> LB, NCB = PRE ? CB : W * CB;
  static_assert(NCB <= MAX_COARSE, "coarse bin table too small");
  __device__ static uint32_t bin(uint32_t w, uint32_t b) { return PRE ? (b >> LB) : w * CB + (b >> LB); }
};

#ifdef ALEO_NO_XCD_TILE
__device__ __forceinline__ uint32_t xcd_tile(uint32_t b, uint32_t) { return b; }
#else
__device__ __forceinline__ uint32_t xcd_tile(uint32_t b, uint32_t g) { return (g & 7u) ? b : (b & 7u) * (g >> 3) + (b >> 3); }
#endif
template <int C, bool MONT, bool PRE>
__global__ void __launch_bounds__(256) k_part_count(SegArgs segs, const uint8_t* inf, uint32_t* __restrict__ cnt) {
  using Gm = SortGeom<C, PRE>;
  __shared__ uint32_t h[MAX_COARSE];
  const uint32_t bx = xcd_tile(blockIdx.x, gridDim.x);
  const uint32_t n = segs.n[blockIdx.y], base = bx * segs.tile;
  if (base >= n) return;
  for (uint32_t i = threadIdx.x; i < Gm::NCB; i += 256) h[i] = 0;
  __syncthreads();
  const char* scalars = segs.ptr[blockIdx.y]; const uint32_t off = segs.off[blockIdx.y], nblk = segs.ncol;
  cnt += (size_t)segs.set[blockIdx.y] * Gm::NCB * nblk + segs.col0[blockIdx.y];
  for (uint32_t q = 0; q < segs.tile / 256; ++q) {
    uint32_t i = base + q * 256 + threadIdx.x;
    if (i < n && !(inf && inf[off + i])) {
      uint32_t s[8]; load_scalar<MONT>(scalars, i, s);
      for_each_digit<C, 0>(s, 0u, [&](uint32_t w, uint32_t b, uint32_t) { atomicAdd(&h[Gm::bin(w, b)], 1u); });
    }
  }
  __syncthreads();
  for (uint32_t i = threadIdx.x; i < Gm::NCB; i += 256) cnt[(size_t)i * nblk + bx] = h[i];
}

__global__ void __launch_bounds__(256) k_scan32_tiles(const uint32_t* __restrict__ in, uint32_t len, uint32_t* __restrict__ local, uint32_t* __restrict__ tile_tot) {
  __shared__ uint32_t wsum[4];
  uint32_t base = blockIdx.x * SCAN_TILE + threadIdx.x * 8;
  uint32_t c[8], pre[8], run = 0;
#pragma unroll
  for (int k = 0; k < 8; ++k) c[k] = (base + k < len) ? in[base + k] : 0u;
#pragma unroll
  for (int k = 0; k < 8; ++k) { pre[k] = run; run += c[k]; }
  uint32_t inc = run; int lane = threadIdx.x & 63, wv = threadIdx.x >> 6;
#pragma unroll
  for (int d = 1; d < 64; d <<= 1) { uint32_t o = __shfl_up(inc, d); if (lane >= d) inc += o; }
  if (lane == 63) wsum[wv] = inc;
  __syncthreads();
  uint32_t woff = 0; for (int k = 0; k < wv; ++k) woff += wsum[k];
  uint32_t excl = woff + inc - run;
#pragma unroll
  for (int k = 0; k < 8; ++k) if (base + k < len) local[base + k] = excl + pre[k];
  if (threadIdx.x == 255) tile_tot[blockIdx.x] = woff + inc;
}
__global__ void __launch_bounds__(256) k_scan32_top(const uint32_t* __restrict__ tile_tot, uint32_t ntiles, uint32_t* __restrict__ blk, uint32_t aux) {
  __shared__ uint32_t sh[256]; __shared__ uint32_t carry;
  if (threadIdx.x == 0) carry = 0;
  __syncthreads();
  for (uint32_t b0 = 0; b0 < ntiles; b0 += 256) {
    uint32_t i = b0 + threadIdx.x, v = i < ntiles ? tile_tot[i] : 0u;
    sh[threadIdx.x] = v; __syncthreads();
    for (int d = 1; d < 256; d <<= 1) {
      uint32_t o = threadIdx.x >= (uint32_t)d ? sh[threadIdx.x - d] : 0u;
      __syncthreads(); sh[threadIdx.x] += o; __syncthreads();
    }
    uint32_t inc = sh[threadIdx.x], cr = carry;
    if (i < ntiles) blk[i] = cr + inc - v;
    __syncthreads();
    if (threadIdx.x == 255) carry = cr + inc;
    __syncthreads();
  }
  if (threadIdx.x == 0) { blk[ntiles] = carry; blk[ntiles + 1] = aux; }
}
__device__ __forceinline__ uint32_t scan32_at(const uint32_t* local, const uint32_t* blk, size_t i) { return local[i] + blk[i / SCAN_TILE]; }

template <int C, bool MONT, bool PRE>
__global__ void __launch_bounds__(256) k_part_scatter(SegArgs segs, const uint8_t* inf, uint32_t row_stride,
                                                      const uint32_t* __restrict__ off_local, const uint32_t* __restrict__ off_blk, uint2* __restrict__ items) {
  using Gm = SortGeom<C, PRE>;
  __shared__ uint32_t cur[MAX_COARSE];
  const uint32_t bx = xcd_tile(blockIdx.x, gridDim.x);
  const uint32_t n = segs.n[blockIdx.y], base = bx * segs.tile;
  if (base >= n) return;
  const char* scalars = segs.ptr[blockIdx.y]; const uint32_t off = segs.off[blockIdx.y], nblk = segs.ncol;
  const size_t row0 = (size_t)segs.set[blockIdx.y] * Gm::NCB; const uint32_t col = segs.col0[blockIdx.y] + bx;
  for (uint32_t i = threadIdx.x; i < Gm::NCB; i += 256) cur[i] = scan32_at(off_local, off_blk, (row0 + i) * nblk + col);
  __syncthreads();
  for (uint32_t q = 0; q < segs.tile / 256; ++q) {
    uint32_t i = base + q * 256 + threadIdx.x;
    if (i < n && !(inf && inf[off + i])) {
      uint32_t s[8]; load_scalar<MONT>(scalars, i, s);
      for_each_digit<C, 0>(s, 0u, [&](uint32_t w, uint32_t b, uint32_t neg) {
        uint32_t pos = atomicAdd(&cur[Gm::bin(w, b)], 1u);
        items[pos] = make_uint2((PRE ? w * row_stride + off + i : off + i) | (neg << 31), b & ((1u << Gm::LB) - 1u));
      });
    }
  }
}

static constexpr uint32_t BIN_PART = 4096;

__global__ void __launch_bounds__(256) k_bin_parts(const uint32_t* __restrict__ off_local, const uint32_t* __restrict__ off_blk, uint32_t nblk, uint32_t ncb,
                                                   uint32_t cnt_tiles, uint32_t* __restrict__ part_start) {
  __shared__ uint32_t wsum[4];
  const uint32_t tid = threadIdx.x; const int lane = tid & 63, wv = tid >> 6;
  constexpr int PER = MAX_COARSE_ALL / 256;
  uint32_t pre[PER], run = 0;
#pragma unroll
  for (int k = 0; k < PER; ++k) {
    const uint32_t bin = tid * PER + k; pre[k] = run;
    if (bin < ncb) {
      const uint32_t st = scan32_at(off_local, off_blk, (size_t)bin * nblk);
      const uint32_t en = (bin + 1 < ncb) ? scan32_at(off_local, off_blk, (size_t)(bin + 1) * nblk) : off_blk[cnt_tiles];
      run += (en - st + BIN_PART - 1) / BIN_PART;
    }
  }
  uint32_t inc = run;
#pragma unroll
  for (int d = 1; d < 64; d <<= 1) { uint32_t o = __shfl_up(inc, d); if (lane >= d) inc += o; }
  if (lane == 63) wsum[wv] = inc;
  __syncthreads();
  uint32_t woff = 0; for (int k = 0; k < wv; ++k) woff += wsum[k];
  const uint32_t excl = woff + inc - run;
#pragma unroll
  for (int k = 0; k < PER; ++k) if (tid * PER + k < ncb) part_start[tid * PER + k] = excl + pre[k];
  if (tid == 255) part_start[ncb] = woff + inc;
}

struct BinPart { uint32_t bin, bstart, lo, hi; bool live; };
__device__ __forceinline__ BinPart locate_part(const uint32_t* __restrict__ off_local, const uint32_t* __restrict__ off_blk, uint32_t nblk, uint32_t ncb,
                                               uint32_t cnt_tiles, const uint32_t* __restrict__ part_start) {
  BinPart r; r.live = blockIdx.x < part_start[ncb];
  if (!r.live) return r;
  uint32_t lo = 0, hi = ncb;
  while (hi - lo > 1) { uint32_t mid = (lo + hi) >> 1; if (part_start[mid] <= blockIdx.x) lo = mid; else hi = mid; }
  r.bin = lo;
  r.bstart = scan32_at(off_local, off_blk, (size_t)lo * nblk);
  const uint32_t bend = (lo + 1 < ncb) ? scan32_at(off_local, off_blk, (size_t)(lo + 1) * nblk) : off_blk[cnt_tiles];
  r.lo = r.bstart + (blockIdx.x - part_start[lo]) * BIN_PART;
  r.hi = r.lo + BIN_PART < bend ? r.lo + BIN_PART : bend;
  return r;
}

__device__ __forceinline__ uint32_t lds_rank(uint32_t* h, uint32_t key, bool valid, int lane) {
  const uint64_t vm = __ballot(valid);
  if (!vm) return 0u;
  const int first = __ffsll((unsigned long long)vm) - 1;
  const uint32_t k0 = __shfl(key, first);
  const bool grp = valid && key == k0;
  const uint64_t same = __ballot(grp);
  uint32_t base = 0;
  if (lane == first) base = atomicAdd(&h[k0], (uint32_t)__popcll(same));
  base = __shfl(base, first);
  if (grp) return base + (uint32_t)__popcll(same & ((1ull << lane) - 1ull));
  return valid ? atomicAdd(&h[key], 1u) : 0u;
}

__device__ __forceinline__ uint32_t block_excl_scan(uint32_t v, uint32_t* wsum, int lane, int wv) {
  uint32_t inc = v;
#pragma unroll
  for (int d = 1; d < 64; d <<= 1) { uint32_t o = __shfl_up(inc, d); if (lane >= d) inc += o; }
  __syncthreads();
  if (lane == 63) wsum[wv] = inc;
  __syncthreads();
  uint32_t woff = 0; for (int k = 0; k < wv; ++k) woff += wsum[k];
  return woff + inc - v;
}

__global__ void __launch_bounds__(256) k_bin_hist(const uint2* __restrict__ items, const uint32_t* __restrict__ off_local, const uint32_t* __restrict__ off_blk,
                                                  uint32_t nblk, uint32_t ncb, uint32_t cnt_tiles, uint32_t LB, const uint32_t* __restrict__ part_start,
                                                  uint32_t* __restrict__ hist) {
  __shared__ uint32_t h[256];
  const uint32_t tid = threadIdx.x; const int lane = tid & 63;
  const BinPart P = locate_part(off_local, off_blk, nblk, ncb, cnt_tiles, part_start);
  if (!P.live) return;
  h[tid] = 0;
  __syncthreads();
// ... 112 lines not shown
    __syncthreads();
    if (threadIdx.x == 255) { carry.x = cr.x + inc.x; carry.y = cr.y + inc.y; }
    __syncthreads();
  }
  if (threadIdx.x == 0) {
    meta[0] = carry.y; meta[2] = carry.x;
    if (host_meta) {
      host_meta[0] = carry.y; host_meta[2] = carry.x;
      for (int i : {1, 3, 4, 5, 6, 7}) host_meta[i] = meta[i];
      __threadfence_system();
      host_meta[8] = seq;
    }
  }
}

static constexpr uint32_t FUSED_TILES = 512;
static constexpr uint32_t ORDER_BATCH = 2048;
static constexpr uint32_t STRETCH_CAP = 8192;
template <bool FUSED>
__global__ void __launch_bounds__(256) k_slice_order(const uint32_t* __restrict__ hist, const uint2* __restrict__ scan_local, uint2* scan_blk, const uint2* __restrict__ tile_tot,
                                                     uint32_t ntiles, const uint32_t* __restrict__ total_pairs, uint32_t M, uint32_t* meta, uint32_t* __restrict__ task_g,
                                                     const uint32_t* __restrict__ len_count, uint32_t* __restrict__ len_cursor, uint32_t* __restrict__ order,
                                                     volatile uint32_t* host_meta, uint32_t seq) {
  __shared__ uint2 sblk[FUSED ? FUSED_TILES : 1]; __shared__ uint2 wtot2[4];
  __shared__ uint32_t s_total, s_tile[2], s_loc[2], wtot[4];
  __shared__ __attribute__((aligned(16))) uint32_t mark[ORDER_BATCH];
  __shared__ uint32_t h[MAX_SLICE + 1], base[MAX_SLICE + 1], len_start[MAX_SLICE + 2];
  const uint32_t tid = threadIdx.x; const int lane = tid & 63, wv = tid >> 6;
  uint32_t total;
  if constexpr (FUSED) {
    const uint2 v0 = 2 * tid < ntiles ? tile_tot[2 * tid] : make_uint2(0u, 0u), v1 = 2 * tid + 1 < ntiles ? tile_tot[2 * tid + 1] : make_uint2(0u, 0u);
    uint2 inc = make_uint2(v0.x + v1.x, v0.y + v1.y);
#pragma unroll
    for (int d = 1; d < 64; d <<= 1) { const uint32_t ox = __shfl_up(inc.x, d), oy = __shfl_up(inc.y, d); if (lane >= d) { inc.x += ox; inc.y += oy; } }
    if (lane == 63) wtot2[wv] = inc;
    __syncthreads();
    uint2 off = make_uint2(0u, 0u); for (int k = 0; k < wv; ++k) { off.x += wtot2[k].x; off.y += wtot2[k].y; }
    const uint2 excl = make_uint2(off.x + inc.x - v0.x - v1.x, off.y + inc.y - v0.y - v1.y);
    if (2 * tid < FUSED_TILES) sblk[2 * tid] = excl;
    if (2 * tid + 1 < FUSED_TILES) sblk[2 * tid + 1] = make_uint2(excl.x + v0.x, excl.y + v0.y);
    if (tid == 255) s_total = off.y + inc.y;
    if (blockIdx.x == 0) {
      if (2 * tid < ntiles) scan_blk[2 * tid] = excl;
      if (2 * tid + 1 < ntiles) scan_blk[2 * tid + 1] = make_uint2(excl.x + v0.x, excl.y + v0.y);
      if (tid == 255) {
        const uint32_t slices = off.y + inc.y, pairs = off.x + inc.x;
        meta[0] = slices; meta[2] = pairs;
        if (host_meta) {
          host_meta[0] = slices; host_meta[2] = pairs;
          for (int i : {1, 3, 4, 5, 6, 7}) host_meta[i] = meta[i];
          __threadfence_system();
          host_meta[8] = seq;
        }
      }
    }
    __syncthreads();
    total = s_total;
  } else {
    total = meta[0];
  }
  const uint32_t s0 = blockIdx.x * ORDER_BATCH;
  if (s0 >= total) return;
  const uint32_t s1 = (total - s0 < ORDER_BATCH ? total : s0 + ORDER_BATCH) - 1;
  auto blk_y = [&](uint32_t T) -> uint32_t { if constexpr (FUSED) return sblk[T].y; else return scan_blk[T].y; };
  auto first_slice = [&](uint32_t g) -> uint32_t { return scan_local[g].y + blk_y(g / SCAN_TILE); };

  {
    constexpr uint32_t PER = (MAX_SLICE + 1 + 255) / 256;
    uint32_t cnt[PER], tot = 0;
#pragma unroll
    for (uint32_t k = 0; k < PER; ++k) { const uint32_t l = PER * tid + k; cnt[k] = l <= MAX_SLICE ? len_count[l] : 0u; tot += cnt[k]; }
    uint32_t inc = tot;
#pragma unroll
    for (int d = 1; d < 64; d <<= 1) { const uint32_t o = __shfl_down(inc, d); if (lane + d < 64) inc += o; }
    if (lane == 0) wtot[wv] = inc;
    __syncthreads();
    uint32_t run = inc - tot; for (int k = wv + 1; k < 4; ++k) run += wtot[k];
#pragma unroll
    for (uint32_t k = PER; k-- > 0;) { const uint32_t l = PER * tid + k; if (l <= MAX_SLICE) len_start[l] = run; run += cnt[k]; }
  }
  for (uint32_t i = tid; i <= MAX_SLICE; i += 256) h[i] = 0;
  for (uint32_t i = tid; i < ORDER_BATCH; i += 256) mark[i] = 0;

  for (uint32_t T = tid; T < ntiles; T += 256) {
    const uint32_t y = blk_y(T), yn = T + 1 < ntiles ? blk_y(T + 1) : 0xffffffffu;
    if (y <= s0 && yn > s0) s_tile[0] = T;
    if (y <= s1 && yn > s1) s_tile[1] = T;
  }
  __syncthreads();
#pragma unroll
  for (int j = 0; j < 2; ++j) {
    const uint32_t s = j ? s1 : s0, T = s_tile[j], by = blk_y(T), e0 = T * SCAN_TILE + tid * 8;
    uint32_t v[9];
#pragma unroll
    for (int k = 0; k < 9; ++k) v[k] = (e0 + k < M && tid * 8 + k < SCAN_TILE) ? scan_local[e0 + k].y + by : 0xffffffffu;
#pragma unroll
    for (int k = 0; k < 8; ++k) if (v[k] <= s && v[k + 1] > s) s_loc[j] = e0 + k;
  }
  __syncthreads();
  const uint32_t g_lo = s_loc[0], g_hi = s_loc[1];
  const bool walk = g_hi - g_lo < STRETCH_CAP;
  uint32_t gq[8];
  if (walk) {
#pragma unroll 4
    for (uint32_t g = g_lo + tid; g <= g_hi; g += 256)
      if (hist[g]) { const uint32_t slot = g == g_lo ? 0u : first_slice(g) - s0; if (slot < ORDER_BATCH) mark[slot] = g + 1u; }
    __syncthreads();
    const uint4 m0 = ((const uint4*)mark)[2 * tid], m1 = ((const uint4*)mark)[2 * tid + 1];
    gq[0] = m0.x; gq[1] = m0.y; gq[2] = m0.z; gq[3] = m0.w; gq[4] = m1.x; gq[5] = m1.y; gq[6] = m1.z; gq[7] = m1.w;
#pragma unroll
    for (int k = 1; k < 8; ++k) gq[k] = gq[k] > gq[k - 1] ? gq[k] : gq[k - 1];
    uint32_t inc = gq[7];
#pragma unroll
    for (int d = 1; d < 64; d <<= 1) { const uint32_t o = __shfl_up(inc, d); if (lane >= d && o > inc) inc = o; }
    if (lane == 63) wtot[wv] = inc;
    uint32_t before = __shfl_up(inc, 1); if (lane == 0) before = 0;
    __syncthreads();
    for (int k = 0; k < wv; ++k) before = wtot[k] > before ? wtot[k] : before;
#pragma unroll
    for (int k = 0; k < 8; ++k) gq[k] = (gq[k] > before ? gq[k] : before) - 1u;
  } else {
#pragma unroll
    for (int k = 0; k < 8; ++k) {
      const uint32_t sid = s0 + tid * 8 + k;
      uint32_t lo = g_lo, hi = g_hi;
      if (sid <= s1) while (lo < hi) { const uint32_t mid = (lo + hi + 1) >> 1; if (first_slice(mid) <= sid) lo = mid; else hi = mid - 1; }
      gq[k] = lo;
    }
  }
  const SliceRule rule = pick_rule(total_pairs, M);
  uint32_t len[8], rank[8];
#pragma unroll
  for (int k = 0; k < 8; ++k) {
    const uint32_t sid = s0 + tid * 8 + k; len[k] = 0;
    if (sid <= s1) { const uint32_t g = gq[k], cnt = hist[g]; len[k] = slice_len(cnt, slices_of(cnt, rule), sid - first_slice(g)); }
  }
  if (s0 + tid * 8 + 7 <= s1) {
    uint4* dst = (uint4*)(task_g + s0 + tid * 8);
    dst[0] = make_uint4(gq[0], gq[1], gq[2], gq[3]); dst[1] = make_uint4(gq[4], gq[5], gq[6], gq[7]);
  } else {
#pragma unroll
    for (int k = 0; k < 8; ++k) if (s0 + tid * 8 + k <= s1) task_g[s0 + tid * 8 + k] = gq[k];
  }
#pragma unroll
  for (int k = 0; k < 8; ++k) rank[k] = lds_rank(h, len[k], s0 + tid * 8 + k <= s1, lane);
  __syncthreads();
  for (uint32_t i = tid; i <= MAX_SLICE; i += 256)
    if (h[i]) base[i] = len_start[i] + atomicAdd(&len_cursor[i], h[i]);
  __syncthreads();
#pragma unroll
  for (int k = 0; k < 8; ++k) if (s0 + tid * 8 + k <= s1) order[base[len[k]] + rank[k]] = s0 + tid * 8 + k;
}

struct SortArgs { SegArgs segs; const uint8_t* inf; uint32_t nblk_x, row_stride; uint32_t* cnt; uint32_t* off_local; uint32_t* off_blk; uint2* items; };
template <int C, bool MONT, bool PRE> static void launch_sort_c(const SortArgs& a, int phase, hipStream_t s) {
  if (phase == 0) hipLaunchKernelGGL((k_part_count<C, MONT, PRE>), dim3(a.nblk_x, a.segs.nseg), dim3(256), 0, s, a.segs, a.inf, a.cnt);
  else hipLaunchKernelGGL((k_part_scatter<C, MONT, PRE>), dim3(a.nblk_x, a.segs.nseg), dim3(256), 0, s, a.segs, a.inf, a.row_stride, a.off_local, a.off_blk, a.items);
}
template <bool MONT> static void launch_sort(int c, bool pre, const SortArgs& a, int phase, hipStream_t s) {
#define CASE(C, PRE) case C: launch_sort_c<C, MONT, PRE>(a, phase, s); break;
  if (pre) switch (c) { CASE(13, true) CASE(16, true) CASE(17, true) CASE(20, true) }
  else switch (c) {
    CASE(2, false) CASE(3, false) CASE(4, false) CASE(5, false) CASE(6, false) CASE(7, false) CASE(8, false) CASE(9, false) CASE(10, false) CASE(11, false) CASE(12, false)
    CASE(13, false) CASE(14, false) CASE(15, false) CASE(16, false)
  }
#undef CASE
}

static constexpr uint32_t FILL_SHIFT = 17;

static size_t slice_bound(size_t pairs_max, size_t M) {
  const size_t nonempty = M < pairs_max ? M : pairs_max;
  const size_t fill_cap = ((size_t)9 << FILL_SHIFT) >> 3;
  const size_t by_rule = M + fill_cap + pairs_max / 256;
  const size_t by_min = pairs_max / 4;
  return nonempty + (by_min < by_rule ? by_min : by_rule) + 1;
}

const PinnedBases::PreTable* msm_tier(const PinnedBases& pb, size_t n) { for (const auto& t : pb.tab) if (t.d && n >= t.min_n && n <= t.cover) return &t; return nullptr; }
static uint32_t sets_of_window(int c) {
  const uint32_t B = 1u << (c - 1), LB = 8, cb = B >> LB, cap = MAX_COARSE_ALL / (cb ? cb : 1);
  return cap < MAX_SETS ? (cap ? cap : 1) : MAX_SETS;
}
uint32_t msm_max_sets(const PinnedBases& pb, size_t n) { const PinnedBases::PreTable* t = msm_tier(pb, n); return t ? sets_of_window(t->c) : 1; }
uint32_t msm_range_sets(const PinnedBases& pb) { return sets_of_window(pb.range.c); }

static int32_t launch_slice_stage(const SortPhase& sp, uint2* tile_tot, const uint32_t* total_pairs, uint32_t* host_meta, bool fuse_top, hipEvent_t ev, hipStream_t s) {
  const uint32_t M = sp.M, ntiles = (M + SCAN_TILE - 1) / SCAN_TILE;
  uint32_t* len_count = sp.meta + 16; uint32_t* len_cursor = len_count + MAX_SLICE + 1;
  hipLaunchKernelGGL(k_scan_tiles, dim3(ntiles), dim3(256), 0, s, sp.hist, M, total_pairs, sp.scan_local, tile_tot, sp.meta, sp.heavy, len_count);
  if (!fuse_top) hipLaunchKernelGGL(k_scan_top, dim3(1), dim3(256), 0, s, tile_tot, ntiles, sp.scan_blk, sp.meta, (volatile uint32_t*)host_meta, sp.meta_seq);
  HIPCHK(hipGetLastError());
  if (ev) HIPCHK(hipEventRecord(ev, s));
  const uint32_t blocks = (uint32_t)((sp.slices_max + ORDER_BATCH - 1) / ORDER_BATCH);
  hipLaunchKernelGGL(fuse_top ? k_slice_order<true> : k_slice_order<false>, dim3(blocks), dim3(256), 0, s, sp.hist, sp.scan_local, sp.scan_blk, (const uint2*)tile_tot, ntiles,
                     total_pairs, M, sp.meta, sp.task_g, len_count, len_cursor, sp.order, fuse_top ? (volatile uint32_t*)host_meta : nullptr, fuse_top ? sp.meta_seq : 0u);
  HIPCHK(hipGetLastError());
  return ALEO_MI355X_OK;
}

int32_t msm_sort_phase(Ctx* c, SegArgs& segs, size_t pts, bool mont, const uint8_t* d_inf, uint32_t row_stride,
                       const MsmPlan& P, bool pre, hipStream_t s, SortPhase* out, bool lean) {
  SortPhase& sp = *out; sp.P = P;
  uint32_t width[MAX_SETS] = {}, nblk_x = 0;
  segs.tile = pts >= ((size_t)1 << 22) ? 8192u : (pts >= ((size_t)1 << 21) ? 4096u : PART_TILE);
  for (uint32_t q = 0; q < segs.nseg; ++q) {
    const uint32_t nb = (segs.n[q] + segs.tile - 1) / segs.tile, st = pre ? segs.set[q] : 0;
    segs.col0[q] = width[st]; width[st] += nb; nblk_x = nb > nblk_x ? nb : nblk_x;
  }
  uint32_t nblk = 1; for (uint32_t w : width) nblk = w > nblk ? w : nblk;
  segs.ncol = nblk;
  sp.digitsW = (SCALAR_BITS + P.c - 1) / P.c;
  const uint32_t M = sp.M = P.M, ntiles = (M + SCAN_TILE - 1) / SCAN_TILE;
  const size_t pairs_max = sp.pairs_max = pts * (size_t)sp.digitsW;
  if (pairs_max >= (1ull << 32)) { g_last_error = "msm: n * windows exceeds 2^32 (shard the MSM across GPUs)"; return ALEO_MI355X_ERR_BAD_ARG; }
  const size_t slices_max = sp.slices_max = slice_bound(pairs_max, M);
  sp.slice_blocks = (uint32_t)((slices_max + 255) / 256);
  int32_t rc;
  const size_t hist_words = 3 * (size_t)M + 2048 + SUPER_CAP;
  if ((rc = c->scan_local.reserve((size_t)M * 8))) return rc;
  if ((rc = c->scan_blk.reserve(2 * (size_t)ntiles * 8 + 64))) return rc;
  if ((rc = c->sorted.reserve(pairs_max * 4))) return rc;
  const uint32_t LB = (P.c - 1) < 8 ? (P.c - 1) : 8, ncb = P.W * (P.B >> LB);
  const size_t cnt_len = (size_t)ncb * nblk;
  if (ncb > MAX_COARSE_ALL || cnt_len >= (1ull << 32)) { g_last_error = "msm: partition table too large"; return ALEO_MI355X_ERR_BAD_ARG; }
  const uint32_t cnt_tiles = (uint32_t)((cnt_len + SCAN_TILE - 1) / SCAN_TILE);
  if ((rc = c->hist.reserve((hist_words + cnt_len) * 4))) return rc;
  if ((rc = c->part_cnt.reserve((cnt_len + 2 * (size_t)cnt_tiles + 16 + MAX_COARSE_ALL) * 4))) return rc;
  if ((rc = c->part_items.reserve(pairs_max * 8))) return rc;
  if ((rc = c->task_g.reserve(2 * slices_max * 4))) return rc;
  if ((rc = ensure_host_pinned(c, 64))) return rc;

  uint32_t* hist = sp.hist = c->hist.as<uint32_t>(); uint32_t* heavy = sp.heavy = hist + M; uint32_t* meta = sp.meta = heavy + M;
  sp.super_list = heavy + M + 2048;
  uint32_t* bin_cursor = hist + 2 * (size_t)M + 2048 + SUPER_CAP;
  uint2* scan_local = sp.scan_local = c->scan_local.as<uint2>();
  uint2* tile_tot = c->scan_blk.as<uint2>(); uint2* scan_blk = sp.scan_blk = tile_tot + ntiles;
  uint32_t* sorted = sp.sorted = c->sorted.as<uint32_t>(); uint32_t* task_g = sp.task_g = c->task_g.as<uint32_t>(); uint32_t* order = sp.order = task_g + slices_max;

  if (!lean) HIPCHK(hipEventRecord(c->ev[0], s));
  sp.zero_bytes = (hist_words + cnt_len) * 4;
  const bool cleared_ahead = c->hist_clean >= sp.zero_bytes && c->hist_clean_stream == s && c->hist_clean_ptr == (void*)hist;
  c->hist_clean = 0;
  if (!cleared_ahead) HIPCHK(hipMemsetAsync(hist, 0, sp.zero_bytes, s));
  SortArgs sa;
  sa.segs = segs; sa.nblk_x = nblk_x ? nblk_x : 1;
  sa.inf = d_inf; sa.row_stride = row_stride;
  sa.cnt = hist + hist_words; sa.off_local = c->part_cnt.as<uint32_t>();
  uint32_t* cnt_tile_tot = sa.off_local + cnt_len; sa.off_blk = cnt_tile_tot + cnt_tiles;
  sa.items = c->part_items.as<uint2>();
  const uint32_t* total_pairs = sp.total_pairs = sa.off_blk + cnt_tiles;
  uint32_t* part_start = sa.off_blk + cnt_tiles + 4;
  const uint32_t nparts_max = ncb + (uint32_t)(pairs_max / BIN_PART) + 1;
  if (mont) launch_sort<true>(P.c, pre, sa, 0, s); else launch_sort<false>(P.c, pre, sa, 0, s);
  hipLaunchKernelGGL(k_scan32_tiles, dim3(cnt_tiles), dim3(256), 0, s, sa.cnt, (uint32_t)cnt_len, sa.off_local, cnt_tile_tot);
  hipLaunchKernelGGL(k_scan32_top, dim3(1), dim3(256), 0, s, cnt_tile_tot, cnt_tiles, sa.off_blk, FILL_SHIFT);
  if (mont) launch_sort<true>(P.c, pre, sa, 1, s); else launch_sort<false>(P.c, pre, sa, 1, s);
  hipLaunchKernelGGL(k_bin_parts, dim3(1), dim3(256), 0, s, sa.off_local, sa.off_blk, nblk, ncb, cnt_tiles, part_start);
  hipLaunchKernelGGL(k_bin_hist, dim3(nparts_max), dim3(256), 0, s, sa.items, sa.off_local, sa.off_blk, nblk, ncb, cnt_tiles, LB, part_start, hist);
  hipLaunchKernelGGL(k_bin_scatter, dim3(nparts_max), dim3(256), 0, s, sa.items, sa.off_local, sa.off_blk, nblk, ncb, cnt_tiles, LB, part_start, hist, bin_cursor, sorted);
  uint32_t* host_meta = nullptr;
  HIPCHK(hipHostGetDevicePointer((void**)&host_meta, c->h_pinned, 0));
  sp.meta_seq = ++c->meta_seq;
  const bool fuse_top = lean && ntiles <= FUSED_TILES;
  if ((rc = launch_slice_stage(sp, tile_tot, total_pairs, host_meta, fuse_top, lean ? nullptr : c->ev[1], s))) return rc;
  HIPCHK(hipGetLastError());
  return ALEO_MI355X_OK;
}

int32_t msm_wait_meta(Ctx* c, const SortPhase& sp, hipStream_t s, SliceMeta* m) {
  const volatile uint32_t* h_meta = (const volatile uint32_t*)c->h_pinned;
  for (uint64_t spins = 0; h_meta[8] != sp.meta_seq; ++spins) {
    __builtin_ia32_pause();
    if ((spins & 0xfff) == 0xfff) {
      const hipError_t q = hipStreamQuery(s);
      if (q == hipErrorNotReady) continue;
      if (q == hipSuccess && h_meta[8] == sp.meta_seq) break;
      if (q == hipSuccess) { (void)hipStreamSynchronize(s); if (h_meta[8] == sp.meta_seq) break; }
      g_last_error = std::string("msm: the slice metadata never arrived (") + hipGetErrorString(q) + ")"; return ALEO_MI355X_ERR_HIP;
    }
  }
  std::atomic_thread_fence(std::memory_order_acquire);
  m->NT = h_meta[0]; m->max_m = h_meta[1]; m->n_heavy = h_meta[3];
  m->max_common = h_meta[6] < 16u ? h_meta[6] : 16u;
  m->n_super = h_meta[5] < SUPER_CAP ? h_meta[5] : SUPER_CAP;
  m->super_overflow = h_meta[5] > SUPER_CAP;
  if (m->NT > sp.slices_max) {
    (void)hipStreamSynchronize(s); g_last_error = "msm: internal slice count overflow"; return ALEO_MI355X_ERR_HIP;
  }
  return ALEO_MI355X_OK;
}

int32_t selftest_slice_order(Ctx* c, const uint32_t* h_hist, uint32_t M, uint32_t pairs, bool fused, uint32_t* violations) {
  const uint32_t ntiles = (M + SCAN_TILE - 1) / SCAN_TILE;
  uint64_t sum = 0; for (uint32_t g = 0; g < M; ++g) sum += h_hist[g];
  if (!M || M > (1u << 20) || sum >= (1ull << 31) || (fused && ntiles > FUSED_TILES)) { g_last_error = "selftest_slice_order: bad argument"; return ALEO_MI355X_ERR_BAD_ARG; }
  SortPhase sp; sp.M = M; sp.pairs_max = sum > pairs ? (size_t)sum : pairs; sp.slices_max = slice_bound(sp.pairs_max, M);
  const size_t hist_words = 3 * (size_t)M + 2048 + SUPER_CAP;
  int32_t rc;
  if ((rc = c->hist.reserve(hist_words * 4))) return rc;
  if ((rc = c->scan_local.reserve((size_t)M * 8))) return rc;
  if ((rc = c->scan_blk.reserve(2 * (size_t)ntiles * 8 + 64))) return rc;
  if ((rc = c->task_g.reserve(2 * sp.slices_max * 4))) return rc;
  if ((rc = c->part_cnt.reserve(16))) return rc;
  if ((rc = ensure_host_pinned(c, 64))) return rc;
  const uint32_t tp[2] = {pairs, FILL_SHIFT};
  const SliceRule rule = pick_rule(tp, M);
  std::vector<uint32_t> first(M + 1), len_want(MAX_SLICE + 1, 0);
  uint32_t NT = 0, max_m = 0, max_common = 0, n_common = 0, n_super = 0;
  for (uint32_t g = 0; g < M; ++g) {
    const uint32_t cnt = h_hist[g], m = slices_of(cnt, rule);
    first[g] = NT; NT += m; max_m = m > max_m ? m : max_m;
    if (m > 16) ++n_super; else if (m > 1) { ++n_common; max_common = m > max_common ? m : max_common; }
    for (uint32_t k = 0; k < m; ++k) { const uint32_t l = slice_len(cnt, m, k); if (l <= MAX_SLICE) ++len_want[l]; }
  }
  first[M] = NT;
  if (pairs < sum || NT > sp.slices_max) { g_last_error = "selftest_slice_order: total_pairs below the histogram's sum"; return ALEO_MI355X_ERR_BAD_ARG; }
  hipStream_t s = c->stream;
  sp.hist = c->hist.as<uint32_t>(); sp.heavy = sp.hist + M; sp.meta = sp.heavy + M; sp.super_list = sp.heavy + M + 2048;
  sp.scan_local = c->scan_local.as<uint2>(); uint2* tile_tot = c->scan_blk.as<uint2>(); sp.scan_blk = tile_tot + ntiles;
  sp.task_g = c->task_g.as<uint32_t>(); sp.order = sp.task_g + sp.slices_max;
  uint32_t* total_pairs = c->part_cnt.as<uint32_t>();
  c->hist_clean = 0;
  HIPCHK(hipMemsetAsync(sp.hist, 0, hist_words * 4, s));
  HIPCHK(hipMemcpyAsync(sp.hist, h_hist, (size_t)M * 4, hipMemcpyHostToDevice, s));
  HIPCHK(hipMemcpyAsync(total_pairs, tp, 8, hipMemcpyHostToDevice, s));
  uint32_t* host_meta = nullptr;
  HIPCHK(hipHostGetDevicePointer((void**)&host_meta, c->h_pinned, 0));
  sp.meta_seq = ++c->meta_seq;
  if ((rc = launch_slice_stage(sp, tile_tot, total_pairs, host_meta, fused, nullptr, s))) return rc;
  HIPCHK(hipStreamSynchronize(s));

  uint32_t bad = 0;
  uint32_t meta[8 + 8 + MAX_SLICE + 1];
  HIPCHK(hipMemcpy(meta, sp.meta, sizeof meta, hipMemcpyDeviceToHost));
  const uint32_t over = n_super > SUPER_CAP ? n_super - SUPER_CAP : 0;
  const uint32_t want[7] = {NT, max_m, (uint32_t)sum, n_common + over, 0u, n_super, max_common};
  const volatile uint32_t* hm = (const volatile uint32_t*)c->h_pinned;
  for (int i = 0; i < 7; ++i) { bad += meta[i] != want[i]; bad += hm[i] != want[i]; }
  bad += hm[8] != sp.meta_seq;
  for (uint32_t l = 0; l <= MAX_SLICE; ++l) bad += meta[16 + l] != len_want[l];
  if (meta[3] == want[3] && meta[5] == want[5]) {
    const uint32_t ns = n_super < SUPER_CAP ? n_super : SUPER_CAP;
    std::vector<uint32_t> lc(want[3]), ls(ns), seen(M, 0);
    if (!lc.empty()) HIPCHK(hipMemcpy(lc.data(), sp.heavy, lc.size() * 4, hipMemcpyDeviceToHost));
    if (!ls.empty()) HIPCHK(hipMemcpy(ls.data(), sp.super_list, ls.size() * 4, hipMemcpyDeviceToHost));
    uint32_t long_in_common = 0;
    for (uint32_t g : lc) { if (g >= M) { ++bad; continue; } const uint32_t m = slices_of(h_hist[g], rule); bad += m <= 1; long_in_common += m > 16; bad += seen[g]++ != 0; }
    for (uint32_t g : ls) { if (g >= M) { ++bad; continue; } bad += slices_of(h_hist[g], rule) <= 16; bad += seen[g]++ != 0; }
    bad += long_in_common != over;
  }
  if (meta[0] == NT && NT) {
    std::vector<uint32_t> task(NT), ord(NT), hit(NT, 0);
    HIPCHK(hipMemcpy(task.data(), sp.task_g, (size_t)NT * 4, hipMemcpyDeviceToHost));
    HIPCHK(hipMemcpy(ord.data(), sp.order, (size_t)NT * 4, hipMemcpyDeviceToHost));
    for (uint32_t sid = 0; sid < NT; ++sid) { const uint32_t g = task[sid]; bad += !(g < M && first[g] <= sid && sid < first[g + 1]); }
    uint32_t prev = 0xffffffffu;
    for (uint32_t t = 0; t < NT; ++t) {
      const uint32_t sid = ord[t];
      if (sid >= NT || hit[sid]++) { ++bad; continue; }
      uint32_t g = (uint32_t)(std::upper_bound(first.begin(), first.begin() + M, sid) - first.begin()) - 1;
      const uint32_t cnt = h_hist[g], l = slice_len(cnt, slices_of(cnt, rule), sid - first[g]);
      bad += l > prev; prev = l;
    }
  }
  *violations = bad;
  return ALEO_MI355X_OK;
}


}
```

### include/aleo_mi355x.h

```cpp
#ifndef ALEO_MI355X_H
#define ALEO_MI355X_H

#include <stddef.h>
#include <stdint.h>

#ifdef __cplusplus
extern "C" {
#endif

#define ALEO_MI355X_OK 0
#define ALEO_MI355X_ERR_NO_DEVICE 1
#define ALEO_MI355X_ERR_BAD_ARG 2
#define ALEO_MI355X_ERR_HIP 3
#define ALEO_MI355X_ERR_BAD_HANDLE 4
#define ALEO_MI355X_ERR_OOM 5
#define ALEO_MI355X_ERR_UNSATISFIED 6
#define ALEO_MI355X_ERR_NOT_OWNER 7

#define ALEO_NTT_ORDER_NN 0
#define ALEO_NTT_ORDER_NR 1
#define ALEO_NTT_ORDER_RN 2
#define ALEO_NTT_ORDER_RR 3
#define ALEO_NTT_FORWARD 0
#define ALEO_NTT_INVERSE 1
#define ALEO_NTT_STANDARD 0
#define ALEO_NTT_COSET 1


int32_t aleo_mi355x_init(int32_t n_devices);
int32_t aleo_mi355x_init_device(int32_t device);
int32_t aleo_mi355x_device_count(int32_t* visible, int32_t* initialised);
int32_t aleo_mi355x_peer_info(int32_t* enabled_pairs, int32_t* refused_pairs);

int32_t aleo_mi355x_msm_g1(void* out_jacobian, const void* bases, size_t base_stride, const void* scalars, size_t n);

int32_t aleo_mi355x_bases_pin(const void* bases, size_t base_stride, size_t n, uint64_t* handle);
int32_t aleo_mi355x_bases_unpin(uint64_t handle);
int32_t aleo_mi355x_bases_generate(const void* base_affine104, uint64_t first_multiple, size_t n, uint64_t* handle);
int32_t aleo_mi355x_bases_from_scalars(const void* base_affine104, const void* scalars, size_t n, uint64_t* handle);
int32_t aleo_mi355x_bases_precompute(uint64_t handle);
int32_t aleo_mi355x_bases_precompute_range(uint64_t handle, size_t offset, size_t n, int32_t window_bits);
int32_t aleo_mi355x_bases_info(uint64_t handle, uint64_t* out, int32_t cap);
int32_t aleo_mi355x_bases_download(uint64_t handle, size_t offset, size_t n, void* out_affine104);
int32_t aleo_mi355x_msm_g1_pinned(void* out_jacobian, uint64_t handle, const void* scalars, size_t n);
int32_t aleo_mi355x_msm_g1_device(void* out_jacobian, uint64_t handle, const void* d_scalars, size_t n, void* stream);
int32_t aleo_mi355x_msm_g1_device_sparse(void* out_jacobian, uint64_t handle, const void* d_scalars, size_t n, void* stream);
int32_t aleo_mi355x_g1_sum(void* out_jacobian, const void* jacobian_points, size_t count);
int32_t aleo_mi355x_bases_pin_sharded(const void* bases, size_t base_stride, size_t n, const int32_t* devices, size_t n_devices, int32_t precompute, uint64_t* handle);
int32_t aleo_mi355x_bases_generate_sharded(const void* base_affine104, uint64_t first_multiple, size_t n, const int32_t* devices, size_t n_devices, int32_t precompute, uint64_t* handle);
int32_t aleo_mi355x_bases_unpin_sharded(uint64_t handle);
int32_t aleo_mi355x_bases_sharded_info(uint64_t handle, uint64_t* out, int32_t cap);
int32_t aleo_mi355x_msm_g1_sharded(void* out_jacobian, uint64_t handle, const void* scalars, size_t n, void* partials_out);

int32_t aleo_mi355x_msm_g2(void* out_jacobian288, const void* bases, size_t base_stride, const void* scalars, size_t n);
int32_t aleo_mi355x_g2_sum(void* out_jacobian288, const void* jacobian_points288, size_t count);
int32_t aleo_mi355x_bases_g2_pin(const void* bases, size_t base_stride, size_t n, uint64_t* handle);
int32_t aleo_mi355x_bases_g2_unpin(uint64_t handle);
int32_t aleo_mi355x_msm_g2_pinned(void* out_jacobian288, uint64_t handle, const void* scalars, size_t n);

int32_t aleo_mi355x_ntt_fr(void* inout, uint32_t lg_n, int32_t order, int32_t direction, int32_t type);
int32_t aleo_mi355x_ntt_fr_device(void* d_inout, uint32_t lg_n, int32_t order, int32_t direction, int32_t type, void* stream);
int32_t aleo_mi355x_ntt_fr_batch_device(void* d_inout, uint32_t lg_n, size_t batch, int32_t order, int32_t direction, int32_t type, void* stream);
int32_t aleo_mi355x_ntt_fr_from_device(void* d_out, const void* d_src, size_t src_stride, size_t src_len, uint32_t lg_n, size_t batch, int32_t direction, int32_t type, void* stream);
int32_t aleo_mi355x_fr_grid_scale_device(void* d_data, uint32_t lg_n, uint64_t rows, uint64_t cols, uint64_t row0, uint64_t col0, uint64_t ld,
                                         int32_t mode, int32_t direction, void* stream);
int32_t aleo_mi355x_fr_transpose_device(void* d_dst, const void* d_src, uint64_t rows, uint64_t cols, void* stream);
int32_t aleo_mi355x_ntt_fr_sharded(void* inout, uint32_t lg_n, int32_t direction, int32_t type, const int32_t* devices, size_t n_devices);
int32_t aleo_mi355x_ntt_fr_sharded_device(void* d_inout, uint32_t lg_n, int32_t direction, int32_t type, const int32_t* devices, size_t n_devices, void* stream);

int32_t aleo_mi355x_kzg_commit(void* out_affine104, uint64_t handle, const void* coeffs_mont, size_t n);
int32_t aleo_mi355x_kzg_commit_device(void* out_affine104, uint64_t handle, const void* d_coeffs_mont, size_t n, void* stream);

int32_t aleo_mi355x_msm_g1_batch_device(void* out_jacobian, uint64_t handle, const void* const* d_scalars, const size_t* lens, size_t k, void* stream);
int32_t aleo_mi355x_kzg_commit_batch_device(void* out_affine104, uint64_t handle, const void* const* d_coeffs_mont, const size_t* lens, size_t k, void* stream);
int32_t aleo_mi355x_kzg_commit_batch(void* out_affine104, uint64_t handle, const void* const* coeffs_mont, const size_t* lens, size_t k);

typedef struct { const void* scalars; size_t len; size_t base_offset; uint32_t output; } aleo_mi355x_commit_segment;
int32_t aleo_mi355x_kzg_commit_segments(void* out_affine104, size_t n_outputs, uint64_t handle, const aleo_mi355x_commit_segment* segments, size_t n_segments);
int32_t aleo_mi355x_kzg_commit_segments_device(void* out_affine104, size_t n_outputs, uint64_t handle, const aleo_mi355x_commit_segment* segments, size_t n_segments, void* stream);
int32_t aleo_mi355x_kzg_commit_segments_sparse_device(void* out_affine104, size_t n_outputs, uint64_t handle, const aleo_mi355x_commit_segment* segments, size_t n_segments, void* stream);
int32_t aleo_mi355x_kzg_commit_segments_sharded_device(void* out_affine104, size_t n_outputs, uint64_t sharded_handle, const aleo_mi355x_commit_segment* segments, size_t n_segments, void* stream);
int32_t aleo_mi355x_kzg_commit_batch_sharded_device(void* out_affine104, uint64_t sharded_handle, const void* const* d_coeffs_mont, const size_t* lens, size_t k, void* stream);
int32_t aleo_mi355x_bases_attach_shards(uint64_t handle, uint64_t sharded_handle, size_t min_points);
int32_t aleo_mi355x_bases_shard_transforms(uint64_t handle, size_t min_elements);

int32_t aleo_mi355x_kzg_commit_hiding(void* out_affine104, uint64_t h_powers, const void* coeffs_mont, size_t n,
                                      uint64_t h_gamma_powers, const void* blinding_mont, size_t m);

#define ALEO_FR_OP_MUL 0
#define ALEO_FR_OP_ADD 1
#define ALEO_FR_OP_SUB 2
int32_t aleo_mi355x_fr_vec_op_device(void* d_dst, const void* d_a, const void* d_b, size_t n, int32_t op, void* stream);
int32_t aleo_mi355x_fr_batch_inverse_device(void* d_inout, size_t n, void* stream);
int32_t aleo_mi355x_fr_lin_device(void* d_dst, size_t n, const void* c0_mont, const void* c1_mont, const void* d_a, const void* c2_mont, const void* d_b, void* stream);
int32_t aleo_mi355x_fr_powers_device(void* d_dst, size_t n, const void* first_mont, const void* ratio_mont, void* stream);
int32_t aleo_mi355x_fr_gather_mul_device(void* d_dst, size_t n, const void* d_scale, const void* d_table1, const void* d_idx1, const void* d_table2, const void* d_idx2, void* stream);
int32_t aleo_mi355x_fr_eval_batch_device(void* d_out, const void* const* d_polys, const size_t* lens, const void* z_mont, size_t k, void* stream);
int32_t aleo_mi355x_fr_random_device(void* d_dst, size_t n, const uint8_t seed[32], uint64_t first_index, int32_t montgomery, void* stream);
int32_t aleo_mi355x_fr_random(void* out, size_t n, const uint8_t seed[32], uint64_t first_index);
int32_t aleo_mi355x_fr_lincomb_device(void* d_dst, size_t n, const void* c0_mont, const void* const* d_terms, const size_t* lens, const void* coeffs_mont, size_t k, void* stream);
int32_t aleo_mi355x_fr_blind_rows_device(void* d_dst, const void* d_src, size_t n, size_t rows, const void* rho_mont, void* stream);
int32_t aleo_mi355x_ahp_sumcheck_operands_device(void* d_dst, const void* d_witness_polys, const void* d_x_polys, size_t n, size_t n_x, size_t instances, void* stream);
int32_t aleo_mi355x_ahp_first_sumcheck_device(void* d_dst, size_t n, const void* d_r, const void* d_za, const void* d_zb, const void* d_t, const void* d_z,
                                              const void* eta_b_mont, const void* eta_c_mont, void* stream);
int32_t aleo_mi355x_ahp_matrix_sumcheck_device(void* d_dst, size_t n, const void* const* d_index, size_t index_stride, const void* const* d_f, const void* consts_mont, void* stream);
int32_t aleo_mi355x_fr_divide_by_linear_device(void* d_quotient, void* d_eval, const void* d_poly, size_t n, const void* z_mont, void* stream);
int32_t aleo_mi355x_kzg_open_device(void* out_affine104, void* out_eval_mont, uint64_t handle, const void* d_poly_mont, size_t n, const void* z_mont, void* stream);
int32_t aleo_mi355x_fr_spmv_device(void* d_y, const void* d_row_ptr, const void* d_col_idx, const void* d_vals, const void* d_x, size_t rows, void* stream);

int32_t aleo_mi355x_g1_compress(void* out48, const void* affine104, size_t n);
int32_t aleo_mi355x_g1_decompress(void* out_affine104, const void* in48, size_t n, int32_t check_subgroup);
int32_t aleo_mi355x_fr_to_bytes(void* out32, const void* fr_mont, size_t n);
int32_t aleo_mi355x_fr_from_bytes(void* out_fr_mont, const void* in32, size_t n);
int32_t aleo_mi355x_bech32m_encode(char* out, size_t cap, const char* hrp, const void* data, size_t len);
int32_t aleo_mi355x_bech32m_decode(void* out, size_t* len, char* hrp_out, size_t hrp_cap, const char* s);
typedef struct {
  const uint64_t* batch_sizes; size_t n_circuits;
  const void* witness_commitments;
  const void* mask_poly;
  const void* g_1; const void* h_1;
  const void* g_abc;
  const void* h_2;
  const void* evaluations; size_t n_evaluations;
  const void* sums;
  const void* opening_points; const void* opening_random_v; const uint8_t* opening_has_v; size_t n_openings;
} aleo_mi355x_proof_parts;
int32_t aleo_mi355x_proof_to_bytes(void* out, size_t* len, const aleo_mi355x_proof_parts* parts);

typedef struct {
  uint64_t n_h, n_k_a, n_k_b, n_k_c, n_x, n_public, n_vars;
  uint64_t committer_key, max_degree, gamma_offset, lagrange_offset;
  const uint32_t* positions;
  const void* positions_device;
  const void *a_row_ptr, *a_col, *a_val, *b_row_ptr, *b_col, *b_val, *t_row_ptr, *t_col, *t_val;
  const void *vx_inv, *k_evals, *k_idx, *k_polys, *k2_evals;
  const void* vk_bytes; size_t vk_len;
  const void* vk_affine;
  uint64_t max_row[3];
} aleo_mi355x_varuna_index;
typedef struct { const uint32_t* row_ptr; const uint32_t* col; const void* val; } aleo_mi355x_r1cs_matrix;
int32_t aleo_mi355x_varuna_index_build(uint64_t* index_handle, uint64_t committer_key, uint64_t max_degree, uint64_t gamma_offset, uint64_t lagrange_offset,
                                       const aleo_mi355x_r1cs_matrix abc[3], size_t n_constraints, size_t n_public, size_t n_private, uint32_t domain_flags);
int32_t aleo_mi355x_varuna_index_export(uint64_t index_handle, aleo_mi355x_varuna_index* out);
int32_t aleo_mi355x_varuna_index_vk(uint64_t index_handle, void* out, size_t* len);
int32_t aleo_mi355x_varuna_index_free(uint64_t index_handle);
int32_t aleo_mi355x_varuna_prove_indexed(uint64_t index_handle, const void* const* assignments, size_t n_instances, const uint8_t seed[32], void* out_proof, size_t* len);
int32_t aleo_mi355x_varuna_prove(const aleo_mi355x_varuna_index* index, const void* const* assignments, size_t n_instances, const uint8_t seed[32], void* out_proof, size_t* len);
int32_t aleo_mi355x_varuna_prove_batch_indexed(const uint64_t* index_handles, size_t n_circuits, const void* const* assignments, const size_t* n_instances, const uint8_t seed[32],
                                               void* out_proof, size_t* len);
typedef struct {
  const uint64_t* index_handles; size_t n_circuits; const void* const* assignments; const size_t* n_instances; const uint8_t* seed;
  void* out_proof; size_t len; int32_t status;
} aleo_mi355x_prove_request;
int32_t aleo_mi355x_varuna_prove_many(aleo_mi355x_prove_request* requests, size_t n_requests);
int32_t aleo_mi355x_varuna_last_timing(double* out_ms, int32_t cap);

int32_t aleo_mi355x_poseidon_hash_fr(uint32_t rate, const void* inputs, size_t n_inputs, void* out, size_t n_out);
int32_t aleo_mi355x_poseidon_parameters_fr(uint32_t rate, void* ark_out, void* mds_out);
int32_t aleo_mi355x_fs_new(uint64_t* sponge);
int32_t aleo_mi355x_fs_free(uint64_t sponge);
int32_t aleo_mi355x_fs_absorb_bytes(uint64_t sponge, const void* data, size_t len);
int32_t aleo_mi355x_fs_absorb_g1(uint64_t sponge, const void* affine, size_t stride, size_t count);
int32_t aleo_mi355x_fs_absorb_fr(uint64_t sponge, const void* fr_canonical, size_t count);
int32_t aleo_mi355x_fs_squeeze_fr(uint64_t sponge, void* out_canonical, size_t count, int32_t short_);

int32_t aleo_mi355x_fq_mul(void* r, const void* a, const void* b, size_t n);
int32_t aleo_mi355x_fr_mul(void* r, const void* a, const void* b, size_t n);

int32_t aleo_mi355x_selftest_madd28(uint32_t lanes, uint32_t steps, uint64_t seed, uint32_t* failures);
int32_t aleo_mi355x_selftest_addquad(uint32_t ops, uint64_t seed, uint32_t* failures);
int32_t aleo_mi355x_selftest_f28_rows(const void* a224, const void* b224, uint32_t n_add, void* out_pair224, void* out_quad224,
                                      const void* acc224, const void* pt112, uint32_t n_madd, void* out_acc224, uint8_t* ok_u8);

int32_t aleo_mi355x_selftest_slice_order(const uint32_t* hist, uint32_t n_buckets, uint32_t total_pairs, int32_t fused, uint32_t* violations);

int32_t aleo_mi355x_selftest_g2pair(const void* affine192, uint32_t n_points, uint32_t n_pairs, uint32_t* failures2);

int32_t aleo_mi355x_selftest_host_inverse(uint32_t count, uint64_t seed, uint32_t* failures, double* ns_per_inverse);

int32_t aleo_mi355x_last_msm_timing(double* out_ms, int32_t cap);

size_t aleo_mi355x_min_msm(void);
size_t aleo_mi355x_min_ntt(void);

int32_t aleo_mi355x_record_parse(const char* record1, int32_t* owner_kind, void* owner32, void* nonce32);
int32_t aleo_mi355x_records_scan(uint8_t* flags, void* rvk_out, const void* owner_c0, const void* nonce_x, size_t n, const void* view_key32, const void* address_x32);
int32_t aleo_mi355x_records_scan_host(uint8_t* flags, void* rvk_out, const void* owner_c0, const void* nonce_x, size_t n, const void* view_key32, const void* address_x32);
size_t aleo_mi355x_min_records(void);

int32_t aleo_mi355x_records_scan_many(uint8_t* flags, void* rvk_out, const void* owner_c0, const void* nonce_x, size_t n, const void* view_keys32, const void* address_xs32, size_t n_keys);
int32_t aleo_mi355x_records_scan_many_host(uint8_t* flags, void* rvk_out, const void* owner_c0, const void* nonce_x, size_t n, const void* view_keys32, const void* address_xs32, size_t n_keys);
int32_t aleo_mi355x_records_parse_many(int8_t* kinds, void* owner32, void* nonce32, const char* text, const uint64_t* offsets, size_t n);
int32_t aleo_mi355x_records_parse_many_host(int8_t* kinds, void* owner32, void* nonce32, const char* text, const uint64_t* offsets, size_t n);
int32_t aleo_mi355x_records_scan_strings(uint8_t* flags, int8_t* kinds, void* rvk_out, const char* text, const uint64_t* offsets, size_t n,
                                         const void* view_keys32, const void* address_xs32, size_t n_keys);
int32_t aleo_mi355x_records_scan_strings_host(uint8_t* flags, int8_t* kinds, void* rvk_out, const char* text, const uint64_t* offsets, size_t n,
                                              const void* view_keys32, const void* address_xs32, size_t n_keys);
int32_t aleo_mi355x_records_decrypt_fields(void* plain_out, uint8_t* flags, const void* rvk, const uint32_t* offsets, const void* fields, size_t n);
int32_t aleo_mi355x_records_decrypt_fields_host(void* plain_out, uint8_t* flags, const void* rvk, const uint32_t* offsets, const void* fields, size_t n);
size_t aleo_mi355x_min_decrypt(void);
int32_t aleo_mi355x_record_fields(const char* record1, void* fields_out, size_t cap, size_t* n_fields_out);
int32_t aleo_mi355x_record_plaintext(const char* record1, const void* plain_fields, size_t n_fields, const void* address_x32, char* out, size_t* out_len);
int32_t aleo_mi355x_record_decrypt(const char* record1, const void* view_key32, const void* address_x32, char* out, size_t* out_len);
typedef struct aleo_mi355x_found aleo_mi355x_found;
int32_t aleo_mi355x_records_decrypt_strings(aleo_mi355x_found** out, const char* text, const uint64_t* offsets, size_t n, const void* view_key32, const void* address_x32);
int32_t aleo_mi355x_records_decrypt_strings_host(aleo_mi355x_found** out, const char* text, const uint64_t* offsets, size_t n, const void* view_key32, const void* address_x32);
void aleo_mi355x_found_free(aleo_mi355x_found* found);
size_t aleo_mi355x_found_count(const aleo_mi355x_found* found);
const uint32_t* aleo_mi355x_found_index(const aleo_mi355x_found* found);
const int8_t* aleo_mi355x_found_kind(const aleo_mi355x_found* found);
const uint8_t* aleo_mi355x_found_rvk(const aleo_mi355x_found* found);
const uint32_t* aleo_mi355x_found_offsets(const aleo_mi355x_found* found);
size_t aleo_mi355x_found_fields(const aleo_mi355x_found* found);
const uint8_t* aleo_mi355x_found_plain(const aleo_mi355x_found* found);
const uint8_t* aleo_mi355x_found_status(const aleo_mi355x_found* found);
const uint64_t* aleo_mi355x_found_microcredits(const aleo_mi355x_found* found);
size_t aleo_mi355x_found_unparsed(const aleo_mi355x_found* found);
size_t aleo_mi355x_found_first_unparsed(const aleo_mi355x_found* found);
int32_t aleo_mi355x_records_decrypt_strings_many(aleo_mi355x_found** out, const char* text, const uint64_t* offsets, size_t n, const void* view_keys32, const void* address_xs32, size_t n_keys);
int32_t aleo_mi355x_records_decrypt_strings_many_host(aleo_mi355x_found** out, const char* text, const uint64_t* offsets, size_t n, const void* view_keys32, const void* address_xs32, size_t n_keys);
int32_t aleo_mi355x_records_serial_numbers(void* sn_out, uint8_t* flags, const void* commitments32, size_t n, const void* sk_sig32);
int32_t aleo_mi355x_records_serial_numbers_host(void* sn_out, uint8_t* flags, const void* commitments32, size_t n, const void* sk_sig32);
size_t aleo_mi355x_min_serials(void);
int32_t aleo_mi355x_found_serial_numbers(const aleo_mi355x_found* found, const void* commitments32, size_t n, const void* sk_sig32, void* sn_out, uint8_t* flags);
int32_t aleo_mi355x_record_commitment(void* out32, const char* record1, const void* plain_fields, size_t n_fields, const char* program_id, const char* record_name);
int32_t aleo_mi355x_record_checksum(void* out32, const char* record1);
int32_t aleo_mi355x_account_from_private_key(const char* private_key, void* sk_sig32, void* view_key32, void* address_x32);

const char* aleo_mi355x_strerror(int32_t status);
const char* aleo_mi355x_last_error(void);
const char* aleo_mi355x_version(void);

#ifdef __cplusplus
}
#endif
#endif
```

Before: 372.8 million.

## Overlap chunked scalar upload with per-piece count passes and whole-bucket slicing

In the multi-context chunked MSM, each chunk's scalars are now split into three pieces. Each piece is uploaded on a side stream and signalled with an event, so the partition-count kernel for a piece can start while later pieces are still copying. This hides host-to-device transfer behind sorting work. To allow this, the sort phase is split into begin/count/rest stages, and count launches take a segment range. Non-final chunks also set a whole-buckets flag that forces maximum slice sizes in the slicing rule; this changes load balance for those chunks, and the extra launches add overhead.

```diff
diff --git a/aleo_amd/_lib.py b/aleo_amd/_lib.py
--- a/aleo_amd/_lib.py
+++ b/aleo_amd/_lib.py
@@ -11,7 +11,7 @@
     'aleo_mi355x_ntt_fr_device', 'aleo_mi355x_ntt_fr_batch_device', 'aleo_mi355x_ntt_fr_from_device', 'aleo_mi355x_fr_grid_scale_device', 'aleo_mi355x_kzg_commit', 'aleo_mi355x_kzg_commit_device', 'aleo_mi355x_kzg_commit_hiding',
     'aleo_mi355x_msm_g1_batch_device', 'aleo_mi355x_kzg_commit_batch_device', 'aleo_mi355x_kzg_commit_batch', 'aleo_mi355x_kzg_commit_segments', 'aleo_mi355x_kzg_commit_segments_device',
     'aleo_mi355x_fr_vec_op_device', 'aleo_mi355x_fr_batch_inverse_device', 'aleo_mi355x_fr_spmv_device', 'aleo_mi355x_fr_divide_by_linear_device', 'aleo_mi355x_kzg_open_device', 'aleo_mi355x_fq_mul',
-    'aleo_mi355x_fr_mul', 'aleo_mi355x_selftest_madd28', 'aleo_mi355x_selftest_addquad', 'aleo_mi355x_selftest_f28_rows', 'aleo_mi355x_selftest_g2pair', 'aleo_mi355x_selftest_slice_order', 'aleo_mi355x_last_msm_timing', 'aleo_mi355x_strerror', 'aleo_mi355x_last_error',
+    'aleo_mi355x_fr_mul', 'aleo_mi355x_selftest_madd28', 'aleo_mi355x_selftest_addquad', 'aleo_mi355x_selftest_f28_rows', 'aleo_mi355x_selftest_g2pair', 'aleo_mi355x_selftest_slice_order', 'aleo_mi355x_selftest_slice_order_whole', 'aleo_mi355x_msm_host_cuts', 'aleo_mi355x_last_msm_timing', 'aleo_mi355x_strerror', 'aleo_mi355x_last_error',
     'aleo_mi355x_version',
     'aleo_mi355x_g1_compress', 'aleo_mi355x_g1_decompress', 'aleo_mi355x_fr_to_bytes', 'aleo_mi355x_fr_from_bytes',
     'aleo_mi355x_bech32m_encode', 'aleo_mi355x_bech32m_decode', 'aleo_mi355x_proof_to_bytes',
@@ -153,6 +153,8 @@
         'aleo_mi355x_selftest_f28_rows': ([vp, vp, u32, vp, vp, vp, vp, u32, vp, vp], i32),
         'aleo_mi355x_selftest_g2pair': ([vp, u32, u32, ctypes.POINTER(u32)], i32),
         'aleo_mi355x_selftest_slice_order': ([vp, u32, u32, i32, ctypes.POINTER(u32)], i32),
+        'aleo_mi355x_selftest_slice_order_whole': ([vp, u32, u32, i32, ctypes.POINTER(u32)], i32),
+        'aleo_mi355x_msm_host_cuts': ([u64, vp, ctypes.POINTER(u32)], i32),
         'aleo_mi355x_last_msm_timing': ([ctypes.POINTER(ctypes.c_double), i32], i32),
         'aleo_mi355x_strerror': ([i32], ctypes.c_char_p),
         'aleo_mi355x_last_error': ([], ctypes.c_char_p),
diff --git a/aleo_amd/csrc/api.hip b/aleo_amd/csrc/api.hip
--- a/aleo_amd/csrc/api.hip
+++ b/aleo_amd/csrc/api.hip
@@ -613,6 +613,12 @@
 int32_t aleo_mi355x_selftest_slice_order(const uint32_t* hist, uint32_t n_buckets, uint32_t total_pairs, int32_t fused, uint32_t* violations) {
   return guarded([&] { if (!hist || !violations) return ALEO_MI355X_ERR_BAD_ARG; Slot sl; if (sl.rc) return sl.rc; return selftest_slice_order(sl.c, hist, n_buckets, total_pairs, fused != 0, violations); });
 }
+int32_t aleo_mi355x_selftest_slice_order_whole(const uint32_t* hist, uint32_t n_buckets, uint32_t total_pairs, int32_t fused, uint32_t* violations) {
+  return guarded([&] { if (!hist || !violations) return ALEO_MI355X_ERR_BAD_ARG; Slot sl; if (sl.rc) return sl.rc; return selftest_slice_order(sl.c, hist, n_buckets, total_pairs, fused != 0, violations, true); });
+}
+int32_t aleo_mi355x_msm_host_cuts(uint64_t n_points, uint64_t* cuts, uint32_t* n_cuts) {
+  return guarded([&] { if (!cuts || !n_cuts || n_points >= (1ull << 31)) return ALEO_MI355X_ERR_BAD_ARG; *n_cuts = msm_host_cuts((size_t)n_points, cuts, *n_cuts); return ALEO_MI355X_OK; });
+}
 int32_t aleo_mi355x_selftest_g2pair(const void* affine192, uint32_t n_points, uint32_t n_pairs, uint32_t* failures2) {
   return guarded([&] { if (!affine192 || !failures2 || n_points < 3 || !n_pairs || n_pairs > (1u << 20)) return ALEO_MI355X_ERR_BAD_ARG; Slot sl; if (sl.rc) return sl.rc; return selftest_g2pair(sl.c, affine192, n_points, n_pairs, failures2); });
 }
diff --git a/aleo_amd/csrc/ctx.h b/aleo_amd/csrc/ctx.h
--- a/aleo_amd/csrc/ctx.h
+++ b/aleo_amd/csrc/ctx.h
@@ -159,19 +159,20 @@
 int32_t ensure_host_pinned(Ctx* c, size_t bytes);
 
 struct MsmSeg { const void* d_ptr = nullptr; size_t len = 0, off = 0; uint32_t out = 0; };
-struct MsmJob { const MsmSeg* segs = nullptr; uint32_t nseg = 0, k = 0; bool mont = false; bool sparse = false; bool fire_tail = false; size_t tier_n = 0; bool lean = false; };
+struct MsmJob { const MsmSeg* segs = nullptr; uint32_t nseg = 0, k = 0; bool mont = false; bool sparse = false; bool fire_tail = false; size_t tier_n = 0; bool lean = false; bool whole_buckets = false; };
 int32_t msm_run(Ctx* c, uint64_t* out_jac18, const PinnedBases& pb, const MsmJob& job, hipStream_t s);
 inline int32_t msm_run1(Ctx* c, uint64_t* out_jac18, const PinnedBases& pb, const void* d_scalars, size_t n, bool mont, hipStream_t s, bool sparse = false) {
   MsmSeg g; g.d_ptr = d_scalars; g.len = n;
   MsmJob j; j.segs = &g; j.nseg = 1; j.k = 1; j.mont = mont; j.sparse = sparse; return msm_run(c, out_jac18, pb, j, s);
 }
 int32_t msm_batch(Ctx* c, uint64_t* out_jac18, const PinnedBases& pb, const MsmJob& job, hipStream_t s);
+uint32_t msm_host_cuts(size_t n, uint64_t* cuts, uint32_t cap);
 int32_t msm_run1_split(Ctx* c, uint64_t* out_jac18, const PinnedBases& pb, const void* d_scalars, size_t n, bool mont, hipStream_t s, bool sparse, const void* host_src, bool may_merge = true);
 int32_t selftest_madd28(Ctx* c, uint32_t lanes, uint32_t steps, uint64_t seed, uint32_t* failures);
 int32_t selftest_addquad(Ctx* c, uint32_t ops, uint64_t seed, uint32_t* failures);
 int32_t selftest_f28_rows(Ctx* c, const void* a224, const void* b224, uint32_t n_add, void* out_pair224, void* out_quad224,
                           const void* acc224, const void* pt112, uint32_t n_madd, void* out_acc224, uint8_t* ok_u8);
-int32_t selftest_slice_order(Ctx* c, const uint32_t* h_hist, uint32_t M, uint32_t pairs, bool fused, uint32_t* violations);
+int32_t selftest_slice_order(Ctx* c, const uint32_t* h_hist, uint32_t M, uint32_t pairs, bool fused, uint32_t* violations, bool whole_buckets = false);
 int32_t generate_multiples(Ctx* c, const void* base104, uint64_t first, size_t n, PinnedBases* out);
 int32_t generate_from_scalars(Ctx* c, const void* base104, const void* scalars32, size_t n, PinnedBases* out);
 int32_t msm_precompute(Ctx* c, PinnedBases* pb);
diff --git a/aleo_amd/csrc/msm.hip b/aleo_amd/csrc/msm.hip
--- a/aleo_amd/csrc/msm.hip
+++ b/aleo_amd/csrc/msm.hip
@@ -351,6 +351,15 @@
 }
 
 int32_t msm_front_sort(Ctx* c, const PinnedBases& pb, const MsmJob& job, hipStream_t s, Front& f) {
+  int32_t rc;
+  if ((rc = msm_front_begin(c, pb, job, s, f)) || f.empty) return rc;
+  if ((rc = msm_front_count(f, 0, f.sp.sa.segs.nseg, s))) return rc;
+  return msm_front_rest(c, s, f);
+}
+int32_t msm_front_count(Front& f, uint32_t seg0, uint32_t nsegs, hipStream_t s) { return msm_sort_count(f.sp, seg0, nsegs, s); }
+int32_t msm_front_rest(Ctx* c, hipStream_t s, Front& f) { return msm_sort_rest(c, f.sp, s); }
+
+int32_t msm_front_begin(Ctx* c, const PinnedBases& pb, const MsmJob& job, hipStream_t s, Front& f) {
   const uint32_t K = f.K = job.k;
   size_t n = 0, pts = 0; SegArgs segs{};
   if (K > MAX_SETS || job.nseg > MAX_SEGS) { g_last_error = "msm: too many sets / segments in one call"; return ALEO_MI355X_ERR_BAD_ARG; }
@@ -393,7 +402,7 @@
   f.vpoints = masked ? (size_t)K * setw + nchunks + (nseg + 1) + (size_t)nseg * (tseg / 2 + tseg / 4 + 2) + 3 * (size_t)nchunks + 64 : (size_t)nchunks + P.W;
   if ((rc = ensure_host_pinned(c, 64 + (size_t)(masked ? nseg : P.W) * 224 + ASIDE_MAX * 228))) return rc;
   SortPhase& sp = f.sp;
-  if ((rc = msm_sort_phase(c, segs, pts, job.mont, d_inf, (uint32_t)(pre ? T->cover : pb.n), P, pre, s, &sp, f.lean))) return rc;
+  if ((rc = msm_sort_begin(c, segs, pts, job.mont, d_inf, (uint32_t)(pre ? T->cover : pb.n), P, pre, s, &sp, f.lean, job.whole_buckets))) return rc;
   const uint32_t M = sp.M;
   if ((rc = c->partial.reserve(sp.slices_max * (pre ? 224 : 192)))) return rc;
   if ((rc = c->vbuf.reserve(f.vpoints * 224))) return rc;
diff --git a/aleo_amd/csrc/msm_chain.h b/aleo_amd/csrc/msm_chain.h
--- a/aleo_amd/csrc/msm_chain.h
+++ b/aleo_amd/csrc/msm_chain.h
@@ -18,6 +18,9 @@
   void dismiss() { armed = false; }
 };
 int32_t msm_front_sort(Ctx* c, const PinnedBases& pb, const MsmJob& job, hipStream_t s, Front& f);
+int32_t msm_front_begin(Ctx* c, const PinnedBases& pb, const MsmJob& job, hipStream_t s, Front& f);
+int32_t msm_front_count(Front& f, uint32_t seg0, uint32_t nsegs, hipStream_t s);
+int32_t msm_front_rest(Ctx* c, hipStream_t s, Front& f);
 int32_t msm_front_accum(Ctx* c, hipStream_t s, Front& f, const FrontChain* seed, hipEvent_t after);
 int32_t msm_front_finish(Ctx* c, hipStream_t s, Front& f, bool allow_aside);
 int32_t msm_reduce_queue(Ctx* c, Front& f, hipStream_t s, const FrontChain& older);
diff --git a/aleo_amd/csrc/msm_common.h b/aleo_amd/csrc/msm_common.h
--- a/aleo_amd/csrc/msm_common.h
+++ b/aleo_amd/csrc/msm_common.h
@@ -9,6 +9,7 @@
 static constexpr uint32_t MAX_SEGS = 64;
 static constexpr uint32_t SUPER_CAP = 4096;
 static constexpr uint32_t MAX_SLICE = 512;
+static constexpr uint32_t WHOLE_BUCKETS = 1u << 31;
 
 struct MsmPlan { uint32_t c, W, B, M, S; };
 __host__ __device__ constexpr int win_count(int c) { return ((int)SCALAR_BITS + c - 1) / c; }
@@ -23,7 +24,8 @@
 
 struct SliceRule { uint32_t single, split; };
 __host__ __device__ __forceinline__ SliceRule pick_rule(const uint32_t* total_pairs, uint32_t M) {
-  const uint32_t pairs = total_pairs[0], mean = pairs / M, fill_shift = total_pairs[1];
+  const uint32_t pairs = total_pairs[0], mean = pairs / M, aux = total_pairs[1], fill_shift = aux & 31u;
+  if (aux & WHOLE_BUCKETS) return SliceRule{MAX_SLICE, MAX_SLICE};
   const uint32_t fill_min = pairs < (1u << 18) ? 4u : 8u;
   uint32_t by_mean = 32u; while (by_mean < 2u * mean && by_mean < 512u) by_mean <<= 1;
   uint32_t fill = (pairs + (1u << fill_shift) - 1) >> fill_shift;
@@ -40,16 +42,23 @@
   return (uint32_t)(((uint64_t)(k + 1) * cnt) / m) - (uint32_t)(((uint64_t)k * cnt) / m);
 }
 
+struct SortArgs { SegArgs segs; const uint8_t* inf; uint32_t nblk_x, row_stride; uint32_t* cnt; uint32_t* off_local; uint32_t* off_blk; uint2* items; };
 struct SortPhase {
   MsmPlan P; uint32_t M = 0, digitsW = 0, slice_blocks = 0; size_t slices_max = 0, pairs_max = 0;
   uint32_t *hist = nullptr, *heavy = nullptr, *meta = nullptr; uint2 *scan_local = nullptr, *scan_blk = nullptr;
   uint32_t *sorted = nullptr, *task_g = nullptr, *order = nullptr; const uint32_t* total_pairs = nullptr; const uint32_t* super_list = nullptr;
   uint32_t meta_seq = 0;
   size_t zero_bytes = 0;
+  SortArgs sa{}; bool mont = false, pre = false, lean = false; uint32_t nblk = 0, ncb = 0, LB = 0, cnt_len = 0, cnt_tiles = 0, aux = 0;
+  uint32_t *cnt_tile_tot = nullptr, *part_start = nullptr, *bin_cursor = nullptr; uint2* tile_tot = nullptr;
 };
 struct SliceMeta { uint32_t NT = 0, max_m = 0, n_heavy = 0, n_super = 0, max_common = 0; bool super_overflow = false; };
 int32_t msm_sort_phase(Ctx* c, SegArgs& segs, size_t pts, bool mont, const uint8_t* d_inf, uint32_t row_stride,
                        const MsmPlan& P, bool pre, hipStream_t s, SortPhase* out, bool lean = false);
+int32_t msm_sort_begin(Ctx* c, SegArgs& segs, size_t pts, bool mont, const uint8_t* d_inf, uint32_t row_stride,
+                       const MsmPlan& P, bool pre, hipStream_t s, SortPhase* out, bool lean = false, bool whole_buckets = false);
+int32_t msm_sort_count(const SortPhase& sp, uint32_t seg0, uint32_t nsegs, hipStream_t s);
+int32_t msm_sort_rest(Ctx* c, SortPhase& sp, hipStream_t s);
 int32_t msm_wait_meta(Ctx* c, const SortPhase& sp, hipStream_t s, SliceMeta* m);
 
 }
diff --git a/aleo_amd/csrc/msm_request.hip b/aleo_amd/csrc/msm_request.hip
--- a/aleo_amd/csrc/msm_request.hip
+++ b/aleo_amd/csrc/msm_request.hip
@@ -20,25 +20,48 @@
   return msm_back(c, out_jac18, f, s, job.fire_tail, FrontChain{});
 }
 
+namespace {
+constexpr uint32_t PIECES = 3;
+struct ChunkCuts { uint32_t Q = 1; size_t lo[4] = {0, 0, 0, 0}; size_t cut[3][PIECES + 1] = {}; };
+ChunkCuts chunk_cuts(size_t n, uint32_t Q) {
+  static const uint32_t share[4][3] = {{100, 0, 0}, {100, 0, 0}, {37, 63, 0}, {18, 30, 52}};
+  static const uint32_t piece_share[2][PIECES] = {{45, 35, 20}, {45, 35, 20}};
+  ChunkCuts cc; cc.Q = Q;
+  for (uint32_t k = 0, acc = 0; k < Q; ++k) { acc += share[Q][k]; cc.lo[k + 1] = k + 1 == Q ? n : (((size_t)((double)n * acc / 100.0)) + 255) & ~(size_t)255; if (cc.lo[k + 1] > n) cc.lo[k + 1] = n; }
+  for (uint32_t k = 0; k < Q; ++k) {
+    const size_t len = cc.lo[k + 1] - cc.lo[k];
+    for (uint32_t p = 0, acc = 0; p < PIECES; acc += piece_share[k ? 1 : 0][p], ++p) cc.cut[k][p] = cc.lo[k] + (size_t)((double)len * acc / 100.0);
+    cc.cut[k][PIECES] = cc.lo[k + 1];
+  }
+  return cc;
+}
+}
 static int32_t msm_run_chunked(Ctx* c, HelperSet& hs, uint64_t* out_jac18, const PinnedBases& pb, size_t n, bool mont, hipStream_t s, const void* host_src) {
   const uint32_t Q = 1 + (uint32_t)hs.ctx.size();
-  static const uint32_t share[4][3] = {{0, 0, 0}, {0, 0, 0}, {37, 63, 0}, {18, 30, 52}};
+  const ChunkCuts cc = chunk_cuts(n, Q); const size_t* lo = cc.lo;
   Ctx* cx[3] = {c, Q > 1 ? hs.ctx[0] : nullptr, Q > 2 ? hs.ctx[1] : nullptr}; hipStream_t st[3] = {s, Q > 1 ? hs.ctx[0]->hi : nullptr, Q > 2 ? hs.ctx[1]->hi : nullptr};
   StreamDrainGuard guard; for (uint32_t k = 0; k < Q; ++k) { guard.add(st[k]); guard.add(cx[k]->side); }
-  size_t lo[4] = {0, 0, 0, 0};
-  for (uint32_t k = 0, acc = 0; k < Q; ++k) { acc += share[Q][k]; lo[k + 1] = k + 1 == Q ? n : (((size_t)((double)n * acc / 100.0)) + 255) & ~(size_t)255; if (lo[k + 1] > n) lo[k + 1] = n; }
-  Front f[3]; MsmSeg seg[3]; int32_t rc;
+  Front f[3]; MsmSeg seg[3][PIECES]; int32_t rc;
   auto view = [&](uint32_t k) { return FrontView{cx[k]->partial.as<char>(), f[k].sp.hist, f[k].sp.scan_local, f[k].sp.scan_blk}; };
   auto chain_before = [&](uint32_t k) { FrontChain ch; for (uint32_t i = k; i-- > 0;) ch.v[ch.n++] = view(i); return ch; };
   for (uint32_t k = 0; k < Q; ++k) {
-    MsmJob j; j.mont = mont; j.tier_n = n; j.k = 1;
+    MsmJob j; j.mont = mont; j.tier_n = n; j.k = 1; j.whole_buckets = k + 1 < Q;
     const size_t len = lo[k + 1] - lo[k];
     if ((rc = cx[k]->scalars_stage.reserve((len ? len : 1) * 32))) return rc;
-    if (hipMemcpyAsync(cx[k]->scalars_stage.p, (const char*)host_src + lo[k] * 32, len * 32, hipMemcpyHostToDevice, st[k]) != hipSuccess) { g_last_error = "msm: upload of a chunk failed"; return ALEO_MI355X_ERR_HIP; }
-    seg[k].d_ptr = cx[k]->scalars_stage.p; seg[k].len = len; seg[k].off = lo[k];
-    j.segs = &seg[k]; j.nseg = 1;
-    if ((rc = msm_front_sort(cx[k], pb, j, st[k], f[k]))) return rc;
+    for (uint32_t p = 0; p < PIECES; ++p) { seg[k][p].d_ptr = (const char*)cx[k]->scalars_stage.p + (cc.cut[k][p] - lo[k]) * 32; seg[k][p].len = cc.cut[k][p + 1] - cc.cut[k][p]; seg[k][p].off = cc.cut[k][p]; }
+    j.segs = seg[k]; j.nseg = PIECES;
+    if ((rc = msm_front_begin(cx[k], pb, j, st[k], f[k]))) return rc;
     if (f[k].empty || !f[k].masked || f[k].P.c != f[0].P.c || f[k].sp.M != f[0].sp.M) { g_last_error = "msm: internal: chunks without a shared table window"; return ALEO_MI355X_ERR_HIP; }
+    static_assert(PIECES == 3, "one event per piece");
+    hipEvent_t landed[PIECES] = {cx[k]->ev[4], cx[k]->ev[7], cx[k]->ev_hop};
+    for (uint32_t p = 0, sg = 0; p < PIECES; ++p) {
+      if (!seg[k][p].len) continue;
+      if (hipMemcpyAsync(const_cast<void*>(seg[k][p].d_ptr), (const char*)host_src + seg[k][p].off * 32, seg[k][p].len * 32, hipMemcpyHostToDevice, cx[k]->side) != hipSuccess) { g_last_error = "msm: upload of a chunk failed"; return ALEO_MI355X_ERR_HIP; }
+      HIPCHK(hipEventRecord(landed[p], cx[k]->side));
+      HIPCHK(hipStreamWaitEvent(st[k], landed[p], 0));
+      if ((rc = msm_front_count(f[k], sg++, 1, st[k]))) return rc;
+    }
+    if ((rc = msm_front_rest(cx[k], st[k], f[k]))) return rc;
     if (k) { if ((rc = msm_front_finish(cx[k - 1], st[k - 1], f[k - 1], false))) return rc; }
     const FrontChain seed = chain_before(k);
     if ((rc = msm_front_accum(cx[k], st[k], f[k], &seed, k ? cx[k - 1]->ev[2] : nullptr))) return rc;
@@ -161,6 +184,13 @@
 }
 
 static constexpr uint32_t MERGE_MIN_LG = 19, CHUNKS3_MIN_LG = 21;
+uint32_t msm_host_cuts(size_t n, uint64_t* cuts, uint32_t cap) {
+  const uint32_t Q = n >= ((size_t)1 << CHUNKS3_MIN_LG) ? 3 : (n >= ((size_t)1 << MERGE_MIN_LG) ? 2 : 1);
+  const ChunkCuts cc = chunk_cuts(n, Q); uint32_t m = 0;
+  for (uint32_t k = 0; k < Q; ++k) for (uint32_t p = 0; p < (Q > 1 ? PIECES : 1u); ++p, ++m) if (m < cap) cuts[m] = cc.cut[k][p];
+  if (m < cap) cuts[m] = n;
+  return m + 1;
+}
 int32_t msm_run1_split(Ctx* c, uint64_t* out_jac18, const PinnedBases& pb, const void* d_scalars, size_t n, bool mont, hipStream_t s, bool sparse, const void* host_src, bool may_merge) {
   const bool tiered = msm_tier(pb, n) != nullptr;
   HelperSet hs;
diff --git a/aleo_amd/csrc/msm_sort.hip b/aleo_amd/csrc/msm_sort.hip
--- a/aleo_amd/csrc/msm_sort.hip
+++ b/aleo_amd/csrc/msm_sort.hip
@@ -68,16 +68,16 @@
 __device__ __forceinline__ uint32_t xcd_tile(uint32_t b, uint32_t g) { return (g & 7u) ? b : (b & 7u) * (g >> 3) + (b >> 3); }
 #endif
 template <int C, bool MONT, bool PRE>
-__global__ void __launch_bounds__(256) k_part_count(SegArgs segs, const uint8_t* inf, uint32_t* __restrict__ cnt) {
+__global__ void __launch_bounds__(256) k_part_count(SegArgs segs, uint32_t seg0, const uint8_t* inf, uint32_t* __restrict__ cnt) {
   using Gm = SortGeom<C, PRE>;
   __shared__ uint32_t h[MAX_COARSE];
-  const uint32_t bx = xcd_tile(blockIdx.x, gridDim.x);
-  const uint32_t n = segs.n[blockIdx.y], base = bx * segs.tile;
+  const uint32_t bx = xcd_tile(blockIdx.x, gridDim.x), sg = seg0 + blockIdx.y;
+  const uint32_t n = segs.n[sg], base = bx * segs.tile;
   if (base >= n) return;
   for (uint32_t i = threadIdx.x; i < Gm::NCB; i += 256) h[i] = 0;
   __syncthreads();
-  const char* scalars = segs.ptr[blockIdx.y]; const uint32_t off = segs.off[blockIdx.y], nblk = segs.ncol;
-  cnt += (size_t)segs.set[blockIdx.y] * Gm::NCB * nblk + segs.col0[blockIdx.y];
+  const char* scalars = segs.ptr[sg]; const uint32_t off = segs.off[sg], nblk = segs.ncol;
+  cnt += (size_t)segs.set[sg] * Gm::NCB * nblk + segs.col0[sg];
   for (uint32_t q = 0; q < segs.tile / 256; ++q) {
     uint32_t i = base + q * 256 + threadIdx.x;
     if (i < n && !(inf && inf[off + i])) {
@@ -496,13 +496,14 @@
   for (int k = 0; k < 8; ++k) if (s0 + tid * 8 + k <= s1) order[base[len[k]] + rank[k]] = s0 + tid * 8 + k;
 }
 
-struct SortArgs { SegArgs segs; const uint8_t* inf; uint32_t nblk_x, row_stride; uint32_t* cnt; uint32_t* off_local; uint32_t* off_blk; uint2* items; };
-template <int C, bool MONT, bool PRE> static void launch_sort_c(const SortArgs& a, int phase, hipStream_t s) {
-  if (phase == 0) hipLaunchKernelGGL((k_part_count<C, MONT, PRE>), dim3(a.nblk_x, a.segs.nseg), dim3(256), 0, s, a.segs, a.inf, a.cnt);
-  else hipLaunchKernelGGL((k_part_scatter<C, MONT, PRE>), dim3(a.nblk_x, a.segs.nseg), dim3(256), 0, s, a.segs, a.inf, a.row_stride, a.off_local, a.off_blk, a.items);
-}
-template <bool MONT> static void launch_sort(int c, bool pre, const SortArgs& a, int phase, hipStream_t s) {
-#define CASE(C, PRE) case C: launch_sort_c<C, MONT, PRE>(a, phase, s); break;
+template <int C, bool MONT, bool PRE> static void launch_sort_c(const SortArgs& a, int phase, uint32_t seg0, uint32_t nsegs, hipStream_t s) {
+  if (phase == 0) {
+    uint32_t nb = 1; for (uint32_t q = seg0; q < seg0 + nsegs; ++q) { const uint32_t b = (a.segs.n[q] + a.segs.tile - 1) / a.segs.tile; nb = b > nb ? b : nb; }
+    hipLaunchKernelGGL((k_part_count<C, MONT, PRE>), dim3(nb, nsegs), dim3(256), 0, s, a.segs, seg0, a.inf, a.cnt);
+  } else hipLaunchKernelGGL((k_part_scatter<C, MONT, PRE>), dim3(a.nblk_x, a.segs.nseg), dim3(256), 0, s, a.segs, a.inf, a.row_stride, a.off_local, a.off_blk, a.items);
+}
+template <bool MONT> static void launch_sort(int c, bool pre, const SortArgs& a, int phase, uint32_t seg0, uint32_t nsegs, hipStream_t s) {
+#define CASE(C, PRE) case C: launch_sort_c<C, MONT, PRE>(a, phase, seg0, nsegs, s); break;
   if (pre) switch (c) { CASE(13, true) CASE(16, true) CASE(17, true) CASE(20, true) }
   else switch (c) {
     CASE(2, false) CASE(3, false) CASE(4, false) CASE(5, false) CASE(6, false) CASE(7, false) CASE(8, false) CASE(9, false) CASE(10, false) CASE(11, false) CASE(12, false)
@@ -545,7 +546,15 @@
 
 int32_t msm_sort_phase(Ctx* c, SegArgs& segs, size_t pts, bool mont, const uint8_t* d_inf, uint32_t row_stride,
                        const MsmPlan& P, bool pre, hipStream_t s, SortPhase* out, bool lean) {
-  SortPhase& sp = *out; sp.P = P;
+  int32_t rc;
+  if ((rc = msm_sort_begin(c, segs, pts, mont, d_inf, row_stride, P, pre, s, out, lean, false))) return rc;
+  if ((rc = msm_sort_count(*out, 0, segs.nseg, s))) return rc;
+  return msm_sort_rest(c, *out, s);
+}
+
+int32_t msm_sort_begin(Ctx* c, SegArgs& segs, size_t pts, bool mont, const uint8_t* d_inf, uint32_t row_stride,
+                       const MsmPlan& P, bool pre, hipStream_t s, SortPhase* out, bool lean, bool whole_buckets) {
+  SortPhase& sp = *out; sp.P = P; sp.mont = mont; sp.pre = pre; sp.lean = lean; sp.aux = FILL_SHIFT | (whole_buckets ? WHOLE_BUCKETS : 0u);
   uint32_t width[MAX_SETS] = {}, nblk_x = 0;
   segs.tile = pts >= ((size_t)1 << 22) ? 8192u : (pts >= ((size_t)1 << 21) ? 4096u : PART_TILE);
   for (uint32_t q = 0; q < segs.nseg; ++q) {
@@ -574,12 +583,13 @@
   if ((rc = c->part_items.reserve(pairs_max * 8))) return rc;
   if ((rc = c->task_g.reserve(2 * slices_max * 4))) return rc;
   if ((rc = ensure_host_pinned(c, 64))) return rc;
+  sp.nblk = nblk; sp.ncb = ncb; sp.LB = LB; sp.cnt_len = (uint32_t)cnt_len; sp.cnt_tiles = cnt_tiles;
 
   uint32_t* hist = sp.hist = c->hist.as<uint32_t>(); uint32_t* heavy = sp.heavy = hist + M; uint32_t* meta = sp.meta = heavy + M;
   sp.super_list = heavy + M + 2048;
-  uint32_t* bin_cursor = hist + 2 * (size_t)M + 2048 + SUPER_CAP;
+  sp.bin_cursor = hist + 2 * (size_t)M + 2048 + SUPER_CAP;
   uint2* scan_local = sp.scan_local = c->scan_local.as<uint2>();
-  uint2* tile_tot = c->scan_blk.as<uint2>(); uint2* scan_blk = sp.scan_blk = tile_tot + ntiles;
+  uint2* tile_tot = sp.tile_tot = c->scan_blk.as<uint2>(); uint2* scan_blk = sp.scan_blk = tile_tot + ntiles;
   uint32_t* sorted = sp.sorted = c->sorted.as<uint32_t>(); uint32_t* task_g = sp.task_g = c->task_g.as<uint32_t>(); uint32_t* order = sp.order = task_g + slices_max;
 
   if (!lean) HIPCHK(hipEventRecord(c->ev[0], s));
@@ -587,22 +597,36 @@
   const bool cleared_ahead = c->hist_clean >= sp.zero_bytes && c->hist_clean_stream == s && c->hist_clean_ptr == (void*)hist;
   c->hist_clean = 0;
   if (!cleared_ahead) HIPCHK(hipMemsetAsync(hist, 0, sp.zero_bytes, s));
-  SortArgs sa;
+  SortArgs& sa = sp.sa;
   sa.segs = segs; sa.nblk_x = nblk_x ? nblk_x : 1;
   sa.inf = d_inf; sa.row_stride = row_stride;
   sa.cnt = hist + hist_words; sa.off_local = c->part_cnt.as<uint32_t>();
-  uint32_t* cnt_tile_tot = sa.off_local + cnt_len; sa.off_blk = cnt_tile_tot + cnt_tiles;
+  sp.cnt_tile_tot = sa.off_local + cnt_len; sa.off_blk = sp.cnt_tile_tot + cnt_tiles;
   sa.items = c->part_items.as<uint2>();
-  const uint32_t* total_pairs = sp.total_pairs = sa.off_blk + cnt_tiles;
-  uint32_t* part_start = sa.off_blk + cnt_tiles + 4;
-  const uint32_t nparts_max = ncb + (uint32_t)(pairs_max / BIN_PART) + 1;
-  if (mont) launch_sort<true>(P.c, pre, sa, 0, s); else launch_sort<false>(P.c, pre, sa, 0, s);
-  hipLaunchKernelGGL(k_scan32_tiles, dim3(cnt_tiles), dim3(256), 0, s, sa.cnt, (uint32_t)cnt_len, sa.off_local, cnt_tile_tot);
-  hipLaunchKernelGGL(k_scan32_top, dim3(1), dim3(256), 0, s, cnt_tile_tot, cnt_tiles, sa.off_blk, FILL_SHIFT);
-  if (mont) launch_sort<true>(P.c, pre, sa, 1, s); else launch_sort<false>(P.c, pre, sa, 1, s);
+  sp.total_pairs = sa.off_blk + cnt_tiles;
+  sp.part_start = sa.off_blk + cnt_tiles + 4;
+  return ALEO_MI355X_OK;
+}
+
+int32_t msm_sort_count(const SortPhase& sp, uint32_t seg0, uint32_t nsegs, hipStream_t s) {
+  if (!nsegs || seg0 + nsegs > sp.sa.segs.nseg) { g_last_error = "msm: internal: count pass over segments the sort does not have"; return ALEO_MI355X_ERR_BAD_ARG; }
+  if (sp.mont) launch_sort<true>(sp.P.c, sp.pre, sp.sa, 0, seg0, nsegs, s); else launch_sort<false>(sp.P.c, sp.pre, sp.sa, 0, seg0, nsegs, s);
+  HIPCHK(hipGetLastError());
+  return ALEO_MI355X_OK;
+}
+
+int32_t msm_sort_rest(Ctx* c, SortPhase& sp, hipStream_t s) {
+  const MsmPlan& P = sp.P; const SortArgs& sa = sp.sa; const bool pre = sp.pre, lean = sp.lean;
+  const uint32_t M = sp.M, ntiles = (M + SCAN_TILE - 1) / SCAN_TILE, nblk = sp.nblk, ncb = sp.ncb, LB = sp.LB, cnt_tiles = sp.cnt_tiles;
+  uint32_t* hist = sp.hist; uint32_t* part_start = sp.part_start; uint2* tile_tot = sp.tile_tot; const uint32_t* total_pairs = sp.total_pairs;
+  const uint32_t nparts_max = ncb + (uint32_t)(sp.pairs_max / BIN_PART) + 1;
+  int32_t rc;
+  hipLaunchKernelGGL(k_scan32_tiles, dim3(cnt_tiles), dim3(256), 0, s, sa.cnt, sp.cnt_len, sa.off_local, sp.cnt_tile_tot);
+  hipLaunchKernelGGL(k_scan32_top, dim3(1), dim3(256), 0, s, sp.cnt_tile_tot, cnt_tiles, sa.off_blk, sp.aux);
+  if (sp.mont) launch_sort<true>(P.c, pre, sa, 1, 0, sa.segs.nseg, s); else launch_sort<false>(P.c, pre, sa, 1, 0, sa.segs.nseg, s);
   hipLaunchKernelGGL(k_bin_parts, dim3(1), dim3(256), 0, s, sa.off_local, sa.off_blk, nblk, ncb, cnt_tiles, part_start);
   hipLaunchKernelGGL(k_bin_hist, dim3(nparts_max), dim3(256), 0, s, sa.items, sa.off_local, sa.off_blk, nblk, ncb, cnt_tiles, LB, part_start, hist);
-  hipLaunchKernelGGL(k_bin_scatter, dim3(nparts_max), dim3(256), 0, s, sa.items, sa.off_local, sa.off_blk, nblk, ncb, cnt_tiles, LB, part_start, hist, bin_cursor, sorted);
+  hipLaunchKernelGGL(k_bin_scatter, dim3(nparts_max), dim3(256), 0, s, sa.items, sa.off_local, sa.off_blk, nblk, ncb, cnt_tiles, LB, part_start, hist, sp.bin_cursor, sp.sorted);
   uint32_t* host_meta = nullptr;
   HIPCHK(hipHostGetDevicePointer((void**)&host_meta, c->h_pinned, 0));
   sp.meta_seq = ++c->meta_seq;
@@ -635,7 +659,7 @@
   return ALEO_MI355X_OK;
 }
 
-int32_t selftest_slice_order(Ctx* c, const uint32_t* h_hist, uint32_t M, uint32_t pairs, bool fused, uint32_t* violations) {
+int32_t selftest_slice_order(Ctx* c, const uint32_t* h_hist, uint32_t M, uint32_t pairs, bool fused, uint32_t* violations, bool whole_buckets) {
   const uint32_t ntiles = (M + SCAN_TILE - 1) / SCAN_TILE;
   uint64_t sum = 0; for (uint32_t g = 0; g < M; ++g) sum += h_hist[g];
   if (!M || M > (1u << 20) || sum >= (1ull << 31) || (fused && ntiles > FUSED_TILES)) { g_last_error = "selftest_slice_order: bad argument"; return ALEO_MI355X_ERR_BAD_ARG; }
@@ -648,7 +672,7 @@
   if ((rc = c->task_g.reserve(2 * sp.slices_max * 4))) return rc;
   if ((rc = c->part_cnt.reserve(16))) return rc;
   if ((rc = ensure_host_pinned(c, 64))) return rc;
-  const uint32_t tp[2] = {pairs, FILL_SHIFT};
+  const uint32_t tp[2] = {pairs, FILL_SHIFT | (whole_buckets ? WHOLE_BUCKETS : 0u)};
   const SliceRule rule = pick_rule(tp, M);
   std::vector<uint32_t> first(M + 1), len_want(MAX_SLICE + 1, 0);
   uint32_t NT = 0, max_m = 0, max_common = 0, n_common = 0, n_super = 0;
diff --git a/include/aleo_mi355x.h b/include/aleo_mi355x.h
--- a/include/aleo_mi355x.h
+++ b/include/aleo_mi355x.h
@@ -173,6 +173,8 @@
                                       const void* acc224, const void* pt112, uint32_t n_madd, void* out_acc224, uint8_t* ok_u8);
 
 int32_t aleo_mi355x_selftest_slice_order(const uint32_t* hist, uint32_t n_buckets, uint32_t total_pairs, int32_t fused, uint32_t* violations);
+int32_t aleo_mi355x_selftest_slice_order_whole(const uint32_t* hist, uint32_t n_buckets, uint32_t total_pairs, int32_t fused, uint32_t* violations);
+int32_t aleo_mi355x_msm_host_cuts(uint64_t n_points, uint64_t* cuts, uint32_t* n_cuts);
 
 int32_t aleo_mi355x_selftest_g2pair(const void* affine192, uint32_t n_points, uint32_t n_pairs, uint32_t* failures2);
 
```

After: 361.6 million. 0.97x the previous value.
